# IRVLUTD/handnet-pipeline

Measured on AMD Instinct MI355X. Metric: end-to-end frames/sec (FCOS+A2J, 640x480), higher is better.
Workload: dtype f16x3 (fp32 values split into fp16 hi+lo, 3 MFMAs, fp32 accumulate; fp32 I/O); 1 GPU; Full HandNet pipeline (FCOS -> crop -> A2J), 640x480 RGB-D (BASELINE config 4); batch_per_gpu=32, global_batch=32, frame=640x480 RGB-D, parallelism=frames sharded over 1 GPU(s), one all-gather of per-frame records per step, rccl_ranks=1, ipc_mode=HSA_ENABLE_IPC_MODE_LEGACY=0, hipgraph=False

## Files before the change

### handnet-pipeline_amd/csrc/conv_igemm_f16x3.hip

```cpp
#define HN_IGEMM_MAIN_TU 1
#include "conv_igemm_f16x3_plan.h"

namespace {

constexpr const char* kCarryRefused =
    "the carried apply pass rides on the plain row-shared 128x128 grouped launch only (this shape takes another form): run the "
    "separate pass";

template <int BM, int BN, int WM, int WN, int NBUF, bool BUF, int TERMS = 3>
int launch16_impl(const ConvParams16& p0, hipStream_t st, const hn::CarryHook* carry = nullptr) {
  ConvParams16 p = p0;
  p.tiles_m = hn::cdiv(p.M, BM);
  p.tiles_n = hn::cdiv(p.Cout, BN);
  p.nblocks = p.tiles_m * p.tiles_n;
  plan_splits(p, BM, BN);
  int taken = 0;
  assign_tickets(p, BM, BN, WM * WN, p.split_ws, taken);
  int grid_x = p.nblocks;
  if (p.groups > 1) {
    grid_x = 0;
    for (int g = 0; g < p.groups; ++g) {
      p.gnblocks[g] = hn::cdiv(p.gM[g], BM) * p.tiles_n;
      grid_x = grid_x > p.gnblocks[g] ? grid_x : p.gnblocks[g];
    }
  }
  bool rs = false;
  constexpr int RS_LDS_BYTES = NBUF * (BM + WM * WN * 8 + BN) * ROWH * 2;
  if constexpr (BUF && NBUF == 2 && (WM * WN == 4 || WM * WN == 8) && RS_LDS_BYTES <= (WM * WN == 4 ? 80 : 160) * 1024 - 2048) {
    rs = rs_will_run(p, BM, BN, WM * WN, NBUF, BUF);
    if constexpr (BM == 128 && BN == 128 && WM == 2 && WN == 2 && TERMS == 3) {
      const int mask = rs ? mixed_small_mask(p, p.tiles_n) : 0;
      if (mask && carry) return hn::fail(HN_ERR_ARG, "%s", kCarryRefused);
      if (mask) {
        p.small_mask = mask;
        grid_x = 0;
        for (int g = 0; g < p.groups; ++g) {
          p.gnblocks[g] = hn::cdiv(p.gM[g], (mask >> g) & 1 ? 64 : 128) * p.tiles_n;
          grid_x = grid_x > p.gnblocks[g] ? grid_x : p.gnblocks[g];
        }
        constexpr int LDS_MIXED = RS_LDS_BYTES > 3 * (64 + 128) * ROWH * 2 ? RS_LDS_BYTES : 3 * (64 + 128) * ROWH * 2;
        static bool mixed_attr[64] = {};
        int dev = 0;
        HN_CHECK_HIP(hipGetDevice(&dev));
        if (dev < 0 || dev >= 64 || !mixed_attr[dev]) {
          HN_CHECK_HIP(hipFuncSetAttribute((const void*)conv_igemm_f16x3_mixed_kernel, hipFuncAttributeMaxDynamicSharedMemorySize,
                                           LDS_MIXED));
          if (dev >= 0 && dev < 64) mixed_attr[dev] = true;
        }
        hipLaunchKernelGGL(conv_igemm_f16x3_mixed_kernel, dim3(grid_x, 1, p.groups), dim3(256), LDS_MIXED, st, p);
        HN_CHECK_LAUNCH("conv_igemm_f16x3_mixed_kernel");
        return HN_OK;
      }
    }
    if (carry) {
      if constexpr (BM == 128 && BN == 128 && WM == 2 && WN == 2) {
        if (!rs || p.groups <= 1 || p.splits != 1) return hn::fail(HN_ERR_ARG, "%s", kCarryRefused);
        if (carry->dry) return HN_OK;
        return hn::launch_conv_carry(&p, sizeof(p), grid_x, p.groups, TERMS, RS_LDS_BYTES, carry->job, st);
      } else {
        return hn::fail(HN_ERR_ARG, "%s", kCarryRefused);
      }
    }
    if (rs) {
      constexpr int LDS_BYTES = RS_LDS_BYTES;
      static bool attr_set[64] = {};
      int dev = 0;
      HN_CHECK_HIP(hipGetDevice(&dev));
      if (dev < 0 || dev >= 64 || !attr_set[dev]) {
        HN_CHECK_HIP(hipFuncSetAttribute((const void*)conv_igemm_f16x3_kernel<BM, BN, WM, WN, NBUF, true, true, TERMS>,
                                         hipFuncAttributeMaxDynamicSharedMemorySize, LDS_BYTES));
        if (dev >= 0 && dev < 64) attr_set[dev] = true;
      }
      hipLaunchKernelGGL((conv_igemm_f16x3_kernel<BM, BN, WM, WN, NBUF, true, true, TERMS>),
                         dim3(grid_x, 1, p.groups > 1 ? p.groups : 1), dim3(WM * WN * 64), LDS_BYTES, st, p);
    }
  }
  if (carry) return hn::fail(HN_ERR_ARG, "%s", kCarryRefused);
  if (!rs)
    hipLaunchKernelGGL((conv_igemm_f16x3_kernel<BM, BN, WM, WN, NBUF, BUF, false, TERMS>),
                       dim3(grid_x, p.splits, p.groups > 1 ? p.groups : 1), dim3(WM * WN * 64), 0, st, p);
  HN_CHECK_LAUNCH("conv_igemm_f16x3_kernel");
  if (p.splits > 1 && p.ticket_base < 0) {
    const long total = (long)p.M * (p.Cout >> 3);
    const int grid = (int)((total + 255) / 256 < 4096 ? (total + 255) / 256 : 4096);
    hipLaunchKernelGGL(splitk_reduce_kernel, dim3(grid), dim3(256), 0, st, p);
    HN_CHECK_LAUNCH("splitk_reduce_kernel");
  }
  return HN_OK;
}

template <int BM, int BN, int WM, int WN, int NST, int KK>
int launch16_deepk(const ConvParams16& p0, hipStream_t st) {
  ConvParams16 p = p0;
  p.tiles_m = hn::cdiv(p.M, BM);
  p.tiles_n = hn::cdiv(p.Cout, BN);
  p.nblocks = p.tiles_m * p.tiles_n;
  plan_splits(p, BM, BN, KK);
  int taken = 0;
  assign_tickets(p, BM, BN, WM * WN, p.split_ws, taken);
  int grid_x = p.nblocks;
  if (p.groups > 1) {
    grid_x = 0;
    for (int g = 0; g < p.groups; ++g) {
      p.gnblocks[g] = hn::cdiv(p.gM[g], BM) * p.tiles_n;
      grid_x = grid_x > p.gnblocks[g] ? grid_x : p.gnblocks[g];
    }
  }
  constexpr int LDS_BYTES = NST * KK * (BM + BN) * ROWH * 2;
  static_assert(LDS_BYTES <= 160 * 1024, "deep-k ring exceeds the LDS");
  static bool attr_set[64] = {};
  int dev = 0;
  HN_CHECK_HIP(hipGetDevice(&dev));
  if (dev < 0 || dev >= 64 || !attr_set[dev]) {
    HN_CHECK_HIP(hipFuncSetAttribute((const void*)conv_igemm_f16x3_deepk_kernel<BM, BN, WM, WN, NST, KK>,
                                     hipFuncAttributeMaxDynamicSharedMemorySize, LDS_BYTES));
    if (dev >= 0 && dev < 64) attr_set[dev] = true;
  }
  hipLaunchKernelGGL((conv_igemm_f16x3_deepk_kernel<BM, BN, WM, WN, NST, KK>), dim3(grid_x, p.splits, p.groups > 1 ? p.groups : 1),
                     dim3(WM * WN * 64), LDS_BYTES, st, p);
  HN_CHECK_LAUNCH("conv_igemm_f16x3_deepk_kernel");
  if (p.splits > 1 && p.ticket_base < 0) {
    const long total = (long)p.M * (p.Cout >> 3);
    const int grid = (int)((total + 255) / 256 < 4096 ? (total + 255) / 256 : 4096);
    hipLaunchKernelGGL(splitk_reduce_kernel, dim3(grid), dim3(256), 0, st, p);
    HN_CHECK_LAUNCH("splitk_reduce_kernel");
  }
  return HN_OK;
}

template <int BM, int BN, int WM, int WN, int NBUF, bool ALLOW_F16X1 = true>
int launch16(const ConvParams16& p0, hipStream_t st, const hn::CarryHook* carry = nullptr) {
  ConvParams16 p = p0;
  const bool ok = finish_params16(p);
  if (p.terms == 1) {
    if constexpr (ALLOW_F16X1) {
      if (ok) return launch16_impl<BM, BN, WM, WN, NBUF, true, 1>(p, st, carry);
    }
    return hn::fail(HN_ERR_ARG, "the f16x1 mode exists for the descriptor-form kernels of the engine tiles only");
  }
  if (ok) return launch16_impl<BM, BN, WM, WN, NBUF, true>(p, st, carry);
  return launch16_impl<128, 128, 2, 2, 2, false>(p, st, carry);
}

}

static int deepk_of(const hn_conv_desc* d, int tile);
static int pick_tile_base(const hn_conv_desc* d);
extern "C" int hn_conv2d_f16x3_pick_tile(const hn_conv_desc* d) {
  if (!d) return HN_TILE_64x64;
  if (d->tile != HN_TILE_AUTO) return d->tile;
  return deepk_of(d, pick_tile_base(d));
}

static int pick_tile_base(const hn_conv_desc* d) {
  if (d->cout <= 32) return nblocks16(d, 128, 32) < 64 ? HN_TILE_32x64 : HN_TILE_128x32;
  const int64_t want = 256;
  if (d->cout > 64 && nblocks16(d, 128, 128) >= want) return HN_TILE_128x128;
  if (d->cout > 64 && d->r * d->s * d->cin / 32 >= 288 && nblocks16(d, 128, 128) >= 224) return HN_TILE_128x128;
  if (d->cout <= 64 && nblocks16(d, 256, 64) >= 2 * want) return HN_TILE_256x64;
  if (d->cout >= 128 && nblocks16(d, 64, 128) >= 192) return HN_TILE_64x128;
  if (nblocks16(d, 128, 64) >= want) return HN_TILE_128x64;
  if (nblocks16(d, 64, 64) < 128) return HN_TILE_32x64;
  return HN_TILE_64x64;
}

static int deepk_of(const hn_conv_desc* d, int tile) {
  if (hn::env_flags().no_deepk || d->terms == 1) return tile;
  const int ktiles = d->r * d->s * d->cin / 32;
  if (ktiles < 8) return tile;
  if (tile == HN_TILE_64x64 && nblocks16(d, 64, 64) <= 256) return HN_TILE_64x64_K2;
  return tile;
}

extern "C" int hn_conv2d_f16x3_uses_halo(const hn_conv_desc* d, int has_residual) {
  return d && hn::conv3x3_halo_applies(d, false, false, has_residual ? (const void*)d : nullptr) ? 1 : 0;
}

extern "C" int hn_conv2d_f16x3_uses_stream(const hn_conv_desc* d) {
  return d && hn::conv1x1_stream_applies(d, false, false) ? 1 : 0;
}

extern "C" int hn_conv2d_f16x3_uses_rs(const hn_conv_desc* d) {
  if (!d || d->w <= 0 || d->cin <= 0) return 0;
  if (hn::conv3x3_halo_applies(d, false, false, d->res_mode ? (const void*)d : nullptr)) return 0;
  const int tile = hn_conv2d_f16x3_pick_tile(d);
  ConvParams16 p;
  p.R = d->r; p.S = d->s; p.stride = d->stride; p.dil = d->dil; p.pad = d->pad;
  p.H = d->h; p.W = d->w; p.pitch = d->w;
  p.OH = (d->h + 2 * d->pad - d->dil * (d->r - 1) - 1) / d->stride + 1;
  p.OW = (d->w + 2 * d->pad - d->dil * (d->s - 1) - 1) / d->stride + 1;
  p.Cout = d->cout;
  p.M = d->n * d->oh * d->ow;
  p.ktiles = d->r * d->s * d->cin / BK;
  p.groups = 1;
  p.rs_ok = 1;
  p.gn_partial = nullptr;
  p.vec_epi = d->cout % 8 == 0;
  p.splitk_mode = d->splitk;
  p.split_ws = d->splitk >= 0 ? reinterpret_cast<float*>(16) : nullptr;
  p.split_ws_bytes = (int64_t)32 << 20;
  TileForm f = tile_form(tile, tile == HN_TILE_128x32 && rs32_preferred(d));
  if (f.bm == 0) return 0;
  p.nblocks = hn::cdiv(p.M, f.bm) * hn::cdiv(p.Cout, f.bn);
  plan_splits(p, f.bm, f.bn, f.kk);
  if (tile == HN_TILE_128x32 && f.nbuf == 2 && !rs_will_run(p, f.bm, f.bn, f.waves, 2, true)) return 0;
  return rs_will_run(p, f.bm, f.bn, f.waves, f.nbuf, true) ? 1 : 0;
}


extern "C" int hn_conv2d_nhwc_f16x3(const hn_conv_desc* d, const void* x16, const void* w16, const float* bias,
                                    const void* residual, void* y, void* stream) {
  return hn_igemm_conv16_run(d, x16, w16, bias, residual, y, nullptr, nullptr, 0, stream);
}

extern "C" int hn_conv2d_nhwc_f16x3_ws(const hn_conv_desc* d, const void* x16, const void* w16, const float* bias,
                                       const void* residual, void* y, void* workspace, int64_t workspace_bytes,
                                       void* stream) {
  HN_CHECK_ARG(workspace == nullptr || ((uintptr_t)workspace % 16 == 0 && workspace_bytes >= 0), "bad workspace");
  return hn_igemm_conv16_run(d, x16, w16, bias, residual, y, nullptr, workspace, workspace_bytes, stream);
}

extern "C" int hn_conv2d_nhwc_f16x3_gn(const hn_conv_desc* d, const void* x16, const void* w16, const float* bias,
                                       void* y, float* gn_partial, void* stream) {
  HN_CHECK_ARG(gn_partial, "hn_conv2d_nhwc_f16x3_gn: null gn_partial");
  HN_CHECK_ARG(d && d->cout % 8 == 0, "GroupNorm statistics need cout %% 8 == 0");
  return hn_igemm_conv16_run(d, x16, w16, bias, nullptr, y, gn_partial, nullptr, 0, stream);
}

extern "C" int hn_conv2d_nhwc_f16x3_grouped(const hn_conv_desc* d, const hn_conv_group* group, void* stream) {
  return hn::conv_grouped_run(d, group, stream, nullptr);
}

int hn::conv_grouped_run(const hn_conv_desc* d, const hn_conv_group* group, void* stream, const hn::CarryHook* carry) {
  HN_CHECK_ARG(d && group, "hn_conv2d_nhwc_f16x3_grouped: null pointer");
  HN_CHECK_ARG(group->count >= 1 && group->count <= HN_CONV_MAX_GROUP, "group count must be 1..%d", HN_CONV_MAX_GROUP);
  HN_CHECK_ARG(d->res_mode == 0, "grouped convolutions take no residual");
  bool any_gn = false, all_gn = true;
  for (int g = 0; g < group->count; ++g) {
    HN_CHECK_ARG(group->x16[g] && group->w16[g] && group->y[g], "group member %d has a null tensor", g);
    any_gn = any_gn || group->gn_partial[g];
    all_gn = all_gn && group->gn_partial[g];
  }
  HN_CHECK_ARG(any_gn == all_gn, "gn_partial must be given for every group member or for none");
  HN_CHECK_ARG(group->gn_units == 0 || group->gn_units >= d->cout / 8, "gn_units smaller than cout/8");
  return hn_igemm_conv16_run(d, group->x16[0], group->w16[0], group->bias[0], nullptr, group->y[0], nullptr, nullptr, 0, stream,
                    group, carry);
}

int hn_igemm_conv16_run(const hn_conv_desc* d, const void* x16, const void* w16, const float* bias, const void* residual, void* y,
                        float* gn_partial, void* workspace, int64_t workspace_bytes, void* stream, const hn_conv_group* group,
                        const hn::CarryHook* carry) {
  ConvParams16 p;
  HN_TRY16(fill_params16(d, x16, w16, bias, residual, y, gn_partial, workspace, workspace_bytes, p));
  if (d->terms != 1 && hn::conv3x3_halo_applies(d, gn_partial != nullptr, group != nullptr, residual) &&
      hn::conv3x3_halo_operands_ok(d, x16, w16, bias, residual, y))
    return hn::conv3x3_halo(d, x16, w16, bias, residual, y, (hipStream_t)stream);
  if (hn::conv1x1_stream_applies(d, gn_partial != nullptr, group != nullptr) &&
      hn::conv1x1_stream_operands_ok(d, x16, w16, bias, residual, y))
    return hn::conv1x1_stream(d, x16, w16, bias, residual, y, (hipStream_t)stream);

  hn_conv_desc tile_desc = *d;
  if (group) {
    p.groups = group->count;
    if (group->gn_units > 0) p.gn_units = group->gn_units;
    int64_t total_m = 0;
    for (int g = 0; g < group->count; ++g) {
      const int gh = group->h[g] > 0 ? group->h[g] : d->h, gw = group->w[g] > 0 ? group->w[g] : d->w;
      p.gH[g] = gh; p.gW[g] = gw;
      p.gOH[g] = (gh + 2 * d->pad - d->dil * (d->r - 1) - 1) / d->stride + 1;
      p.gOW[g] = (gw + 2 * d->pad - d->dil * (d->s - 1) - 1) / d->stride + 1;
      HN_CHECK_ARG(p.gOH[g] > 0 && p.gOW[g] > 0, "group member %d has an empty output", g);
      HN_CHECK_ARG((int64_t)d->n * p.gOH[g] * p.gOW[g] < (int64_t)1 << 31, "too many output pixels");
      p.gM[g] = d->n * p.gOH[g] * p.gOW[g];
      total_m += p.gM[g];
      if (gn_of_group_needs_32(group, g)) HN_CHECK_ARG(p.gOH[g] * p.gOW[g] >= 32, "GroupNorm statistics need OH*OW >= 32");
      p.gx[g] = (const _Float16*)group->x16[g]; p.gw[g] = (const _Float16*)group->w16[g];
      p.gbias[g] = group->bias[g]; p.gy[g] = group->y[g]; p.ggn[g] = group->gn_partial[g];
      p.vec_epi = p.vec_epi && ((uintptr_t)group->y[g] % 16 == 0) &&
                  (group->bias[g] == nullptr || (uintptr_t)group->bias[g] % 16 == 0);
    }
    p.gn_partial = group->gn_partial[0];
    p.split_ws = nullptr;
    if (group->gn_partial[0])
      HN_CHECK_ARG(p.vec_epi && !d->out_split && d->relu_cols == 0,
                   "GroupNorm statistics need the vector epilogue, fp32 output and no ReLU");
    tile_desc.n = 1;
    tile_desc.oh = (int)(total_m < ((int64_t)1 << 30) ? total_m : ((int64_t)1 << 30));
    tile_desc.ow = 1;
  }
  p.splits = 1;
  p.kt_per = p.ktiles;
  if (gn_partial) {
    HN_CHECK_ARG(p.vec_epi && !d->out_split && d->res_mode == 0 && d->relu_cols == 0,
                 "GroupNorm statistics need the vector epilogue, fp32 output, no residual and no ReLU");
    HN_CHECK_ARG(d->oh * d->ow >= 32, "GroupNorm statistics in the epilogue need OH*OW >= 32");
  }
  hipStream_t st = (hipStream_t)stream;
  int picked = hn_conv2d_f16x3_pick_tile(&tile_desc);
  if (carry && (picked != HN_TILE_128x128 || !group)) return hn::fail(HN_ERR_ARG, "%s", kCarryRefused);
  switch (picked) {
    case HN_TILE_128x128: return launch16<128, 128, 2, 2, 2>(p, st, carry);
    case HN_TILE_128x64: return launch16<128, 64, 2, 2, 2>(p, st);
    case HN_TILE_64x64: return launch16<64, 64, 2, 2, 3>(p, st);
    case HN_TILE_128x32: {
      bool rs2 = rs32_preferred(d);
      if (rs2) {
        ConvParams16 q = p;
        q.nblocks = hn::cdiv(q.M, 128) * hn::cdiv(q.Cout, 32);
        if (group) {
          q.nblocks = 0;
          for (int g = 0; g < q.groups; ++g) q.nblocks += hn::cdiv(q.gM[g], 128) * hn::cdiv(q.Cout, 32);
        }
        plan_splits(q, 128, 32);
        rs2 = rs_will_run(q, 128, 32, 4, 2, true);
      }
      if (rs2) return launch16<128, 32, 4, 1, 2>(p, st);
      return launch16<128, 32, 4, 1, 3>(p, st);
    }
    case HN_TILE_64x128: return launch16<64, 128, 2, 2, 3>(p, st);
    case HN_TILE_32x64: return launch16<32, 64, 1, 2, 4>(p, st);
    case HN_TILE_64x64_K2: {
      ConvParams16 q = p;
      if (p.terms == 3 && finish_params16(q)) return launch16_deepk<64, 64, 2, 2, 3, 2>(q, st);
      return launch16<64, 64, 2, 2, 3>(p, st);
    }
    case HN_TILE_256x64: return launch16<256, 64, 4, 1, 2>(p, st);
    default: return hn::fail(HN_ERR_ARG, "unknown or retired tile id %d", d->tile);
  }
}

static int stem16_run(const void* x16, int n, int ph, int pw, int pad, int r, int stride, int cout, const void* w16,
                      const float* bias, int relu, void* y, int out_split, bool pool, void* stream, int terms = 3) {
  HN_CHECK_ARG(x16 && w16 && y, "hn_conv_stem_f16x3: null pointer");
  HN_CHECK_ARG(n > 0 && ph > 0 && pw > 0 && cout > 0 && stride > 0, "bad dims");
  HN_CHECK_ARG(r >= 1 && r <= 8 && pad == r / 2, "stem filter must be R x R with R <= 8 and pad = R/2");
  HN_CHECK_ARG(!out_split || cout % 32 == 0, "S32 output needs cout %% 32 == 0 (got %d)", cout);
  const int hb = ph + 2 * pad, wb = pw + 2 * pad;
  const int oh = (hb - r) / stride + 1, ow = (wb - r) / stride + 1;
  HN_CHECK_ARG((ow - 1) * stride + 8 <= wb, "the 8-pixel k run of the last output column leaves the bordered row");
  HN_CHECK_ARG((int64_t)n * oh * ow < (int64_t)1 << 31, "too many output pixels");
  HN_CHECK_ARG((uintptr_t)x16 % 16 == 0 && (stride * 4 * 2) % 16 == 0 && (wb * 4 * 2) % 16 == 0,
               "LDS-DMA needs 16-byte aligned rows (stride and bordered width must be even)");
  ConvParams16 p;
  p.x = (const _Float16*)x16; p.w = (const _Float16*)w16; p.bias = bias; p.res = nullptr; p.y = y;
  p.N = n; p.H = hb; p.W = wb; p.Cin = 32; p.Cout = cout; p.R = r; p.S = 1;
  p.stride = stride; p.pad = 0; p.dil = 1; p.OH = oh; p.OW = ow;
  p.M = n * oh * ow;
  p.Ktot = r * 32;
  p.ktiles = r;
  p.relu_cols = relu ? cout : 0; p.res_mode = 0; p.res_h = p.res_w = 0;
  p.out_split = out_split; p.res_split = 0;
  p.xs = 4; p.pitch = wb; p.lo_off = (long)n * hb * wb * 4;
  p.gn_partial = nullptr;
  p.split_ws = nullptr; p.split_ws_bytes = 0; p.splits = 1; p.kt_per = p.ktiles; p.splitk_mode = -1; p.groups = 1; p.gn_units = cout >> 3;
  p.ys = (out_split ? 2 : 1) * cout;
  p.rs = 0;
  p.vec_epi = (cout % 8 == 0) && ((uintptr_t)y % 16 == 0) && (bias == nullptr || (uintptr_t)bias % 16 == 0);
  p.tiles_m = p.tiles_n = p.nblocks = 0;
  p.small_mask = 0;
  p.rs_ok = 0;
  p.terms = terms == 1 ? 1 : 3;
  p.range_flag = hn::range_flag_ptr();
  hipStream_t st = (hipStream_t)stream;
  if (pool) {
    HN_CHECK_ARG(cout == 64 && relu && out_split && bias, "the fused stem + max-pool kernel needs cout = 64, bias, ReLU and an S32 output");
    HN_CHECK_ARG((uintptr_t)y % 16 == 0 && (uintptr_t)bias % 16 == 0, "unaligned output / bias");
    HN_CHECK_ARG(r == 7 && stride == 2 && pad == 3 && (uintptr_t)w16 % 16 == 0,
                 "the fused stem + max-pool kernel is written for the 7x7 / stride-2 / pad-3 ResNet stem");
    return hn::stem_pool_direct(x16, n, ph, pw, w16, bias, y, terms == 1 ? 1 : 3, st);
  }
  if (cout <= 32) return launch16<128, 32, 4, 1, 3>(p, st);
  if (cout <= 64) return launch16<128, 64, 2, 2, 2>(p, st);
  return launch16<128, 128, 2, 2, 2>(p, st);
}

extern "C" int hn_conv_stem_f16x3(const void* x16, int n, int ph, int pw, int pad, int r, int stride, int cout,
                                  const void* w16, const float* bias, int relu, void* y, int out_split, void* stream) {
  return stem16_run(x16, n, ph, pw, pad, r, stride, cout, w16, bias, relu, y, out_split, false, stream);
}

extern "C" int hn_conv_stem_pool_f16x3(const void* x16, int n, int ph, int pw, int pad, int r, int stride, int cout,
                                       const void* w16, const float* bias, void* y, void* stream) {
  return stem16_run(x16, n, ph, pw, pad, r, stride, cout, w16, bias, 1, y, 1, true, stream);
}

extern "C" int hn_conv_stem_pool_f16x3_terms(const void* x16, int n, int ph, int pw, int pad, int r, int stride, int cout,
                                             const void* w16, const float* bias, void* y, int terms, void* stream) {
  HN_CHECK_ARG(terms == 0 || terms == 1 || terms == 3, "terms must be 0 / 3 or 1");
  return stem16_run(x16, n, ph, pw, pad, r, stride, cout, w16, bias, 1, y, 1, true, stream, terms);
}

int hn::tickets_nonzero_main(int64_t* count) { return tickets_nonzero_here(count); }
```

### handnet-pipeline_amd/csrc/conv_igemm_f16x3_kernel.h

```cpp
#pragma once
#include "hn_common.h"

#include <type_traits>

namespace {

typedef float f32x4 __attribute__((ext_vector_type(4)));
typedef _Float16 f16x8 __attribute__((ext_vector_type(8)));
typedef unsigned int u32x4 __attribute__((ext_vector_type(4)));
typedef __attribute__((address_space(3))) void lds_void;
typedef __attribute__((address_space(1))) const void gbl_void;

__device__ __attribute__((aligned(256))) _Float16 g_zero_page16[128];

constexpr int kTicketSlots = 128, kTicketsPerSlot = 4096;
constexpr bool fused_reduce_form(int bm, int bn) { return bm <= 64 && bn <= 128; }
__device__ int g_split_tickets[kTicketSlots * kTicketsPerSlot];

struct ConvParams16 {
  const _Float16* x;
  const _Float16* w;
  const float* bias;
  const void* res;
  void* y;
  int N, H, W, Cin, Cout, R, S, stride, pad, dil, OH, OW;
  int M, Ktot, ktiles;
  int relu_cols, res_mode, res_h, res_w;
  int xs;
  int pitch;
  long lo_off;
  int ys;
  int rs;
  int out_split, res_split;
  int vec_epi;
  float* gn_partial;
  int groups;
  const _Float16* gx[HN_CONV_MAX_GROUP];
  const _Float16* gw[HN_CONV_MAX_GROUP];
  const float* gbias[HN_CONV_MAX_GROUP];
  void* gy[HN_CONV_MAX_GROUP];
  float* ggn[HN_CONV_MAX_GROUP];
  int gH[HN_CONV_MAX_GROUP], gW[HN_CONV_MAX_GROUP], gOH[HN_CONV_MAX_GROUP], gOW[HN_CONV_MAX_GROUP];
  int gM[HN_CONV_MAX_GROUP], gnblocks[HN_CONV_MAX_GROUP];
  int gn_units;
  int splits, kt_per, splitk_mode;
  int ticket_base;
  float* split_ws;
  int64_t split_ws_bytes;
  int tiles_m, tiles_n, nblocks;
  int small_mask;
  int* range_flag;
  unsigned mg_ohow, sh_ohow, mg_ow, sh_ow;
  unsigned gmg_ohow[HN_CONV_MAX_GROUP], gsh_ohow[HN_CONV_MAX_GROUP], gmg_ow[HN_CONV_MAX_GROUP], gsh_ow[HN_CONV_MAX_GROUP];
  unsigned mg_w1, sh_w1, mg_h, sh_h;
  unsigned gmg_w1[HN_CONV_MAX_GROUP], gsh_w1[HN_CONV_MAX_GROUP], gmg_h[HN_CONV_MAX_GROUP], gsh_h[HN_CONV_MAX_GROUP];
  int terms;
  int rs_ok;
  unsigned a_records;
  unsigned b_records;
  unsigned ga_records[HN_CONV_MAX_GROUP];
};

#define HN_TRY16(expr)          \
  do {                          \
    const int st_ = (expr);     \
    if (st_ != HN_OK) return st_; \
  } while (0)

constexpr int BK = 32;
constexpr int ROWH = 64;

__device__ __forceinline__ int swz(int row) { return (row >> 1) & 7; }

__device__ __forceinline__ int fastdiv(int n, unsigned mg, unsigned sh) {
  return mg ? (int)(__umulhi((unsigned)n, mg) >> sh) : n;
}

__device__ __forceinline__ void mfma_pinned(f32x4& c, const f16x8& a, const f16x8& b) {
  asm volatile("v_mfma_f32_16x16x32_f16 %0, %2, %1, %0" : "+a"(c) : "v"(a), "v"(b) : "memory");
}

template <int OFF>
__device__ __forceinline__ void lds_read_pinned(f16x8& dst, unsigned addr) {
  static_assert(OFF >= 0 && OFF < 65536, "ds_read offset field is 16 bits");
  asm volatile("ds_read_b128 %0, %1 offset:%2" : "=v"(dst) : "v"(addr), "n"(OFF) : "memory");
}
template <int N>
__device__ __forceinline__ void lgkm_wait() {
  static_assert(N >= 0 && N <= 15, "lgkmcnt is a 4-bit counter");
  asm volatile("s_waitcnt lgkmcnt(%0)" ::"n"(N) : "memory");
}
__device__ __forceinline__ unsigned lds_addr(const _Float16* p) { return (unsigned)(size_t)(lds_void*)p; }

template <int B, int E, class F>
__device__ __forceinline__ void static_for(F&& f) {
  if constexpr (B < E) {
    f(std::integral_constant<int, B>{});
    static_for<B + 1, E>(f);
  }
}

__device__ __forceinline__ void epi_finish8(const ConvParams16& p, int m, int n, float (&v)[8], int ohow,
                                            const f16x8* pre_hi = nullptr, const f16x8* pre_lo = nullptr) {
  if (pre_hi) {
#pragma unroll
    for (int e = 0; e < 8; ++e) v[e] += (float)(*pre_hi)[e] + (float)(*pre_lo)[e];
  } else if (p.res_mode) {
    long rpix = m;
    if (p.res_mode == 2) {
      const int img = m / ohow;
      const int rem = m - img * ohow;
      const int oh = rem / p.OW, ow = rem - oh * p.OW;
      const int sh_ = (int)(((long)oh * p.res_h) / p.OH), sw_ = (int)(((long)ow * p.res_w) / p.OW);
      rpix = ((long)img * p.res_h + sh_) * p.res_w + sw_;
    }
    if (p.res_split) {
      const _Float16* q16 = reinterpret_cast<const _Float16*>(p.res) + rpix * p.rs + (n >> 5) * 64 + (n & 31);
      const f16x8 rh = *reinterpret_cast<const f16x8*>(q16), rl = *reinterpret_cast<const f16x8*>(q16 + 32);
#pragma unroll
      for (int e = 0; e < 8; ++e) v[e] += (float)rh[e] + (float)rl[e];
    } else {
      const float* q32 = reinterpret_cast<const float*>(p.res) + rpix * p.rs + n;
      const f32x4 r0 = *reinterpret_cast<const f32x4*>(q32), r1 = *reinterpret_cast<const f32x4*>(q32 + 4);
#pragma unroll
      for (int e = 0; e < 4; ++e) {
        v[e] += r0[e];
        v[4 + e] += r1[e];
      }
    }
  }
  if (p.relu_cols >= p.Cout) {
#pragma unroll
    for (int e = 0; e < 8; ++e) v[e] = hn::relu(v[e]);
  } else if (p.relu_cols > 0) {
#pragma unroll
    for (int e = 0; e < 8; ++e)
      if (n + e < p.relu_cols) v[e] = hn::relu(v[e]);
  }
  if (p.out_split) {
    if (p.range_flag) hn::range_note_n<8>(p.range_flag, v);
    f16x8 hi, lo;
#pragma unroll
    for (int e = 0; e < 8; ++e) {
      const _Float16 h = (_Float16)v[e];
      hi[e] = h;
      lo[e] = (_Float16)(v[e] - (float)h);
    }
    _Float16* q16 = reinterpret_cast<_Float16*>(p.y) + (long)m * p.ys + (n >> 5) * 64 + (n & 31);
    *reinterpret_cast<f16x8*>(q16) = hi;
    *reinterpret_cast<f16x8*>(q16 + 32) = lo;
  } else {
    float* q32 = reinterpret_cast<float*>(p.y) + (long)m * p.ys + n;
    f32x4 o0, o1;
#pragma unroll
    for (int e = 0; e < 4; ++e) {
      o0[e] = v[e];
      o1[e] = v[4 + e];
    }
    *reinterpret_cast<f32x4*>(q32) = o0;
    *reinterpret_cast<f32x4*>(q32 + 4) = o1;
  }
}

__device__ __forceinline__ void splitk_reduce_body(const ConvParams16& p) {
  const int units = p.Cout >> 3;
  const long total = (long)p.M * units;
  const int ohow = p.OH * p.OW;
  const long plane = (long)p.M * p.Cout;
  for (long i = (long)blockIdx.x * blockDim.x + threadIdx.x; i < total; i += (long)gridDim.x * blockDim.x) {
    const int m = (int)(i / units), n = (int)(i - (long)m * units) * 8;
    float v[8] = {0.f, 0.f, 0.f, 0.f, 0.f, 0.f, 0.f, 0.f};
    const float* src = p.split_ws + (long)m * p.Cout + n;
    for (int z = 0; z < p.splits; ++z) {
      const f32x4 a = *reinterpret_cast<const f32x4*>(src + z * plane), b = *reinterpret_cast<const f32x4*>(src + z * plane + 4);
#pragma unroll
      for (int e = 0; e < 4; ++e) {
        v[e] += a[e];
        v[4 + e] += b[e];
      }
    }
    if (p.bias) {
      const f32x4 b0 = *reinterpret_cast<const f32x4*>(p.bias + n), b1 = *reinterpret_cast<const f32x4*>(p.bias + n + 4);
#pragma unroll
      for (int e = 0; e < 4; ++e) {
        v[e] += b0[e];
        v[4 + e] += b1[e];
      }
    }
    epi_finish8(p, m, n, v, ohow);
  }
}

#ifdef HN_IGEMM_MAIN_TU
__global__ __launch_bounds__(256) void splitk_reduce_kernel(const ConvParams16 p) { splitk_reduce_body(p); }
#endif

template <int TM, int TH, int DPT, int TERMS = 3>
struct HalfSched {
  static constexpr int NM = 3 * TM * TH;
  static constexpr int NB = (TERMS == 3 ? 2 : 1) * TH;
  static constexpr int NAL = TERMS == 3 ? TM : 0;
  static constexpr int NMEM = DPT + NB + NAL + TM;
  static constexpr int earliest(int q) {
    return q < DPT + NB ? 0
           : q < DPT + NB + NAL ? (q - DPT - NB + 1) * TH
                                : 2 * TM * TH + (q - DPT - NB - NAL + 1) * TH;
  }
  static constexpr int slot(int q) {
    const int spread = (q * NM) / NMEM;
    return earliest(q) > spread ? earliest(q) : spread;
  }
};

template <int BM, int BN, int WM, int WN, int NBUF, bool BUF, bool RS = false, int TERMS = 3, bool DYN = false, int KK = 1>
__device__ __forceinline__ void conv_igemm_f16x3_body(const ConvParams16& p, const int blk_x, const int blk_y, const int blk_z,
                                                      const unsigned karg_off = 0 ) {
  static_assert(TERMS == 3 || TERMS == 1, "three terms (fp32-grade) or the hi*hi term alone");
  static_assert(NBUF >= 2 && NBUF <= 6, "2..6 LDS stages");
  static_assert(!RS || (BUF && NBUF == 2), "row-shared A needs the descriptor form and the 2-stage pipeline");
  static_assert(KK == 1 || (BUF && !RS && DYN && TERMS == 3), "the deep-k loop: descriptor form, per-tap, dynamic LDS, three terms");
  constexpr int NSLOT = NBUF * KK;
  struct {
    const _Float16 *x, *w;
    const float* bias;
    void* y;
    float* gn_partial;
    int H, W, pitch, OH, OW, M, nblocks;
    unsigned a_records, mg_ohow, sh_ohow, mg_ow, sh_ow, mg_w1, sh_w1, mg_h, sh_h;
  } o = {p.x, p.w, p.bias, p.y, p.gn_partial, p.H, p.W, p.pitch, p.OH, p.OW, p.M, p.nblocks, p.a_records,
         p.mg_ohow, p.sh_ohow, p.mg_ow, p.sh_ow, p.mg_w1, p.sh_w1, p.mg_h, p.sh_h};
  if (p.groups > 1) {
    typedef __attribute__((address_space(4))) const ConvParams16 KArgs;
    KArgs* kp = (KArgs*)__builtin_amdgcn_kernarg_segment_ptr();
    const int gz = blk_z;
    static_assert(HN_CONV_MAX_GROUP == 6, "member tables hold six entries");
    o.nblocks = kp->gnblocks[gz];
    if (blk_x >= o.nblocks) return;
    o.x = kp->gx[gz];
    o.w = kp->gw[gz];
    o.bias = kp->gbias[gz];
    o.y = kp->gy[gz];
    o.gn_partial = kp->ggn[gz];
    o.H = kp->gH[gz];
    o.W = kp->gW[gz];
    o.pitch = o.W;
    o.OH = kp->gOH[gz];
    o.OW = kp->gOW[gz];
    o.M = kp->gM[gz];
    o.a_records = kp->ga_records[gz];
    o.mg_ohow = kp->gmg_ohow[gz];
    o.sh_ohow = kp->gsh_ohow[gz];
    o.mg_ow = kp->gmg_ow[gz];
    o.sh_ow = kp->gsh_ow[gz];
    if constexpr (RS) {
      o.mg_w1 = kp->gmg_w1[gz];
      o.sh_w1 = kp->gsh_w1[gz];
      o.mg_h = kp->gmg_h[gz];
      o.sh_h = kp->gsh_h[gz];
    }
  }
  constexpr int NT = WM * WN * 64;
  constexpr int TM = BM / WM / 16, TN = BN / WN / 16;
  static_assert(TM >= 2 && TM % 2 == 0 && TN >= 2 && TN % 2 == 0, "wave tile must be a multiple of 32x32");
  constexpr int TH = TN / 2;
  constexpr int ROWS_PASS = NT / 8;
  static_assert(BM % ROWS_PASS == 0 && BN % ROWS_PASS == 0, "tile rows must be a multiple of NT/8");
  constexpr int A_ROWS = RS ? BM + ROWS_PASS : BM;
  constexpr int A_IT = A_ROWS / ROWS_PASS, B_IT = BN / ROWS_PASS;
  constexpr int A_BUF = A_ROWS * ROWH, B_BUF = BN * ROWH;
  extern __shared__ __attribute__((aligned(1024))) _Float16 smem_dyn[];
  __shared__ __attribute__((aligned(1024))) _Float16 smem_static[(RS || DYN) ? 8 : NSLOT * (A_BUF + B_BUF)];
  _Float16* smem = (RS || DYN) ? smem_dyn : smem_static;
  _Float16* As = smem;
  _Float16* Bs = smem + NSLOT * A_BUF;

  int lid;
  {
    const int bid = blk_x, nb = o.nblocks;
    const int q = nb >> 3, rr = nb & 7, xcd = bid & 7, loc = bid >> 3;
    lid = (xcd < rr ? xcd * (q + 1) : rr * (q + 1) + (xcd - rr) * q) + loc;
  }
  const int tile_m = lid / p.tiles_n, tile_n = lid - tile_m * p.tiles_n;
  const int m0 = tile_m * BM, n0 = tile_n * BN;
  const int tid = threadIdx.x, lane = tid & 63, wave = tid >> 6;
  const int wm = wave / WN, wn = wave - wm * WN;
  const int ohow = o.OH * o.OW;


  const int drow = tid >> 3, dpos = tid & 7;
  int a_ih0[A_IT], a_iw0[A_IT], a_cc[A_IT];
  const _Float16* a_row[A_IT];
  const _Float16* b_ptr[B_IT];
  unsigned a_off[A_IT], a_inv[A_IT], b_off[B_IT];
  int rs_u0 = 0;
  if constexpr (RS) {
    const int mw = fastdiv(m0, o.mg_ow, o.sh_ow);
    rs_u0 = mw * (o.W + 1) + (m0 - mw * o.W) - 1;
  }
#pragma unroll
  for (int it = 0; it < A_IT; ++it) {
    const int row = drow + it * ROWS_PASS;
    if constexpr (RS) {
      const int u = rs_u0 + row;
      const int uc = u < 0 ? 0 : u;
      const int rowi = fastdiv(uc, o.mg_w1, o.sh_w1);
      const int owp = uc - rowi * (o.W + 1);
      const int img = fastdiv(rowi, o.mg_h, o.sh_h);
      const int oh = rowi - img * o.H;
      const bool pix_ok = u >= 0 && owp < o.W && rowi < p.N * o.H;
      const int chunk = dpos ^ swz(row);
      a_off[it] = pix_ok ? (((unsigned)rowi * (unsigned)o.pitch + (unsigned)owp) * (unsigned)p.xs + (unsigned)((chunk & 3) * 8) +
                            (unsigned)(chunk >> 2) * (unsigned)p.lo_off) * 2u
                         : 0u;
      a_inv[it] = !pix_ok ? 7u : (oh == 0 ? 1u : 0u) | (oh == o.H - 1 ? 4u : 0u);
      continue;
    }
    int m = m0 + row;
    m = m < o.M ? m : o.M - 1;
    const int img = fastdiv(m, o.mg_ohow, o.sh_ohow);
    const int rem = m - img * ohow;
    const int oh = fastdiv(rem, o.mg_ow, o.sh_ow), ow = rem - oh * o.OW;
    const int ih0 = oh * p.stride - p.pad, iw0 = ow * p.stride - p.pad;
    const int chunk = dpos ^ swz(row);
    if constexpr (BUF) {
      a_off[it] = (((unsigned)(img * o.H + oh * p.stride) * (unsigned)o.pitch + (unsigned)(ow * p.stride)) * (unsigned)p.xs +
                   (unsigned)((chunk & 3) * 8) + (unsigned)(chunk >> 2) * (unsigned)p.lo_off) * 2u;
      unsigned inv = 0;
      if (p.pad > 0) {
        if (p.R == 3 && p.S == 3) {
          const unsigned uw = (unsigned)o.W, uh = (unsigned)o.H;
          const unsigned col_bits = ((unsigned)iw0 >= uw ? 1u : 0u) | ((unsigned)(iw0 + p.dil) >= uw ? 2u : 0u) |
                                    ((unsigned)(iw0 + 2 * p.dil) >= uw ? 4u : 0u);
          inv = ((unsigned)ih0 >= uh ? 7u : col_bits) | (((unsigned)(ih0 + p.dil) >= uh ? 7u : col_bits) << 3) |
                (((unsigned)(ih0 + 2 * p.dil) >= uh ? 7u : col_bits) << 6);
        } else {
          unsigned col_bits = 0;
          for (int sx = 0; sx < p.S; ++sx) col_bits |= ((unsigned)(iw0 + sx * p.dil) >= (unsigned)o.W ? 1u : 0u) << sx;
          const unsigned row_full = (1u << p.S) - 1u;
          for (int r = 0; r < p.R; ++r) {
            const unsigned bits = (unsigned)(ih0 + r * p.dil) >= (unsigned)o.H ? row_full : col_bits;
            inv |= bits << (r * p.S);
          }
        }
      }
      a_inv[it] = inv;
    } else {
      a_ih0[it] = ih0;
      a_iw0[it] = iw0;
      a_cc[it] = chunk * 8;
      a_row[it] = o.x + (((long)img * o.H + ih0) * o.pitch + iw0) * p.xs + (chunk & 3) * 8 + (chunk >> 2) * p.lo_off;
    }
  }
#pragma unroll
  for (int it = 0; it < B_IT; ++it) {
    const int row = drow + it * ROWS_PASS;
    int n = n0 + row;
    n = n < p.Cout ? n : p.Cout - 1;
    if constexpr (BUF)
      b_off[it] = ((unsigned)n * (unsigned)p.Ktot * 2u + (unsigned)((dpos ^ swz(row)) * 8)) * 2u;
    else
      b_ptr[it] = o.w + (long)n * p.Ktot * 2 + (dpos ^ swz(row)) * 8;
  }
  const long a_shift = RS ? (long)o.pitch * p.xs * 2 : BUF ? ((long)p.pad * o.pitch + p.pad) * p.xs * 2 : 0;
  const __amdgpu_buffer_rsrc_t rsrc_a = __builtin_amdgcn_make_buffer_rsrc(
      (void*)(reinterpret_cast<const char*>(o.x) - a_shift), 0, (int)o.a_records, 0x00020000);
  const __amdgpu_buffer_rsrc_t rsrc_b = __builtin_amdgcn_make_buffer_rsrc((void*)o.w, 0, (int)p.b_records, 0x00020000);
  const int grp_row = __builtin_amdgcn_readfirstlane(wave) * 8;
// ... 238 lines not shown
    if constexpr (PH == 2) rs_a_offsets(uoff_a, sh_a);
    _Float16* Ad = As + aq * A_BUF;
    _Float16* Bd = Bs + cs * B_BUF;
    const int an = PH == 2 ? aq ^ 1 : aq;
    unsigned anx[TM][2];
#pragma unroll
    for (int i = 0; i < TM; ++i)
#pragma unroll
      for (int pl = 0; pl < 2; ++pl) anx[i][pl] = rs_addr(i, NPH - 1, pl, an);
    const unsigned bnx_hi = b_rd_hi + ns * (B_BUF * 2), bnx_lo = b_rd_lo + ns * (B_BUF * 2);
    static_for<0, S3::NM + 1>([&](auto K) {
      constexpr int k = decltype(K)::value;
      static_for<0, S3::NMEM>([&](auto Q) {
        constexpr int q = decltype(Q)::value;
        if constexpr (S3::slot(q) == k) {
          if constexpr (q < B_IT) {
            dma_b_piece(q, Bd, boff);
          } else if constexpr (q < DPT_PH) {
            dma_a_piece(q - B_IT, Ad, 0, 0, uoff_a, sh_a);
          } else if constexpr (q < DPT_PH + S3::NB) {
            if constexpr (TERMS == 3) {
              constexpr int jj = (q - DPT_PH) >> 1;
              if constexpr ((q - DPT_PH) & 1)
                lds_read_pinned<jj * TILE_OFF>(b0.l[jj], bnx_lo);
              else
                lds_read_pinned<jj * TILE_OFF>(b0.h[jj], bnx_hi);
            } else {
              lds_read_pinned<(q - DPT_PH) * TILE_OFF>(b0.h[q - DPT_PH], bnx_hi);
            }
          } else if constexpr (q < DPT_PH + S3::NB + S3::NAL) {
            constexpr int i = q - DPT_PH - S3::NB;
            lds_read_pinned<0>(af.l[i], anx[i][1]);
          } else {
            constexpr int i = q - DPT_PH - S3::NB - S3::NAL;
            lds_read_pinned<0>(af.h[i], anx[i][0]);
          }
        }
      });
      if constexpr (k < S3::NM) {
        constexpr int term = k / (TM * TH), i = (k / TH) % TM, jj = k % TH;
        if constexpr (TERMS == 3 || term == 2) mfma_pinned(acc[i][TH + jj], term == 0 ? af.l[i] : af.h[i], term == 1 ? b1.l[jj] : b1.h[jj]);
      }
    });
    advance_tile();
    if constexpr (PH == 2) rs_a_advance();
  };
  if constexpr (RS) {
    rs_dma_a_tile(0);
    dma_tile(0);
    drain_and_barrier();
    dma_tile(1);
    rs_dma_a_tile(1);
    static_for<0, TH>([&](auto JJ) {
      constexpr int jj = decltype(JJ)::value;
      lds_read_pinned<jj * TILE_OFF>(b0.h[jj], b_rd_hi);
      if constexpr (TERMS == 3) lds_read_pinned<jj * TILE_OFF>(b0.l[jj], b_rd_lo);
    });
    if constexpr (TERMS == 3)
      static_for<0, TM>([&](auto I) { lds_read_pinned<0>(af.l[decltype(I)::value], rs_addr(decltype(I)::value, -1, 1, 0)); });
    static_for<0, TM>([&](auto I) { lds_read_pinned<0>(af.h[decltype(I)::value], rs_addr(decltype(I)::value, -1, 0, 0)); });
    __builtin_amdgcn_s_waitcnt(0xC07F);
    int aq = 0, cs = 0;
    for (int q3 = 0; q3 < a_qn; ++q3) {
      step_rs(std::integral_constant<int, 0>{}, cs, cs ^ 1, aq);
      step_rs(std::integral_constant<int, 1>{}, cs ^ 1, cs, aq);
      step_rs(std::integral_constant<int, 2>{}, cs, cs ^ 1, aq);
      cs ^= 1;
      aq ^= 1;
    }
  } else if constexpr (KK > 1) {
    static_assert((NBUF - 2) * KK * (A_IT + B_IT) <= 63, "vmcnt is a 6-bit counter");
    for (int s0 = 0; s0 < (NBUF - 1) * KK; ++s0) dma_tile(s0);
    const int nstages = (T + KK - 1) / KK;
    int grp = 0;
    static_assert(KK == 2, "the stage schedule below is written for two tiles per stage");
    auto read_frags = [&](int slot, f16x8 (&fah)[TM], f16x8 (&fal)[TM], f16x8 (&fbh)[TN], f16x8 (&fbl)[TN]) {
      const _Float16* Ab = As + slot * A_BUF;
      const _Float16* Bb = Bs + slot * B_BUF;
#pragma unroll
      for (int i = 0; i < TM; ++i) {
        fah[i] = *reinterpret_cast<const f16x8*>(Ab + a_rd[i][0]);
        fal[i] = *reinterpret_cast<const f16x8*>(Ab + a_rd[i][1]);
      }
#pragma unroll
      for (int j = 0; j < TN; ++j) {
        fbh[j] = *reinterpret_cast<const f16x8*>(Bb + b_rd[j][0]);
        fbl[j] = *reinterpret_cast<const f16x8*>(Bb + b_rd[j][1]);
      }
    };
    auto mfma_tile = [&](const f16x8 (&fah)[TM], const f16x8 (&fal)[TM], const f16x8 (&fbh)[TN], const f16x8 (&fbl)[TN]) {
#pragma unroll
      for (int i = 0; i < TM; ++i)
#pragma unroll
        for (int j = 0; j < TN; ++j) acc[i][j] = __builtin_amdgcn_mfma_f32_16x16x32_f16(fbh[j], fal[i], acc[i][j], 0, 0, 0);
#pragma unroll
      for (int i = 0; i < TM; ++i)
#pragma unroll
        for (int j = 0; j < TN; ++j) acc[i][j] = __builtin_amdgcn_mfma_f32_16x16x32_f16(fbl[j], fah[i], acc[i][j], 0, 0, 0);
#pragma unroll
      for (int i = 0; i < TM; ++i)
#pragma unroll
        for (int j = 0; j < TN; ++j) acc[i][j] = __builtin_amdgcn_mfma_f32_16x16x32_f16(fbh[j], fah[i], acc[i][j], 0, 0, 0);
    };
    (void)nstages;
    const int full = T / KK;
    for (int st = 0; st < full; ++st) {
      asm volatile("s_waitcnt vmcnt(%0) lgkmcnt(0)" ::"n"((NBUF - 2) * KK * DPT) : "memory");
      __builtin_amdgcn_s_barrier();
      asm volatile("" ::: "memory");
      f16x8 a0h[TM], a0l[TM], b0h[TN], b0l[TN], a1h[TM], a1l[TM], b1h[TN], b1l[TN];
      read_frags(grp * KK, a0h, a0l, b0h, b0l);
      const int refill = grp == 0 ? NBUF - 1 : grp - 1;
#pragma unroll
      for (int kk = 0; kk < KK; ++kk) dma_tile(refill * KK + kk);
      read_frags(grp * KK + 1, a1h, a1l, b1h, b1l);
      mfma_tile(a0h, a0l, b0h, b0l);
      mfma_tile(a1h, a1l, b1h, b1l);
      grp = grp + 1 == NBUF ? 0 : grp + 1;
    }
    if (T & 1) {
      asm volatile("s_waitcnt vmcnt(%0)" ::"n"((NBUF - 2) * KK * DPT) : "memory");
      __builtin_amdgcn_s_barrier();
      asm volatile("" ::: "memory");
      f16x8 a0h[TM], a0l[TM], b0h[TN], b0l[TN];
      read_frags(grp * KK, a0h, a0l, b0h, b0l);
      mfma_tile(a0h, a0l, b0h, b0l);
    }
  } else {
  dma_tile(0);
  drain_and_barrier();
  for (int i = 1; i < NBUF; ++i) dma_tile(i);
  static_for<0, TH>([&](auto JJ) {
    constexpr int jj = decltype(JJ)::value;
    lds_read_pinned<jj * TILE_OFF>(b0.h[jj], b_rd_hi);
    if constexpr (TERMS == 3) lds_read_pinned<jj * TILE_OFF>(b0.l[jj], b_rd_lo);
  });
  if constexpr (TERMS == 3)
    static_for<0, TM>([&](auto I) { lds_read_pinned<decltype(I)::value * TILE_OFF>(af.l[decltype(I)::value], a_rd_lo); });
  static_for<0, TM>([&](auto I) { lds_read_pinned<decltype(I)::value * TILE_OFF>(af.h[decltype(I)::value], a_rd_hi); });
  __builtin_amdgcn_s_waitcnt(0xC07F);
  int cs = 0, ns = 1;
  for (int t = 0; t < T; ++t) {
    step_main(cs, ns);
    cs = ns;
    ns = ns + 1 == NBUF ? 0 : ns + 1;
  }
  }
  asm volatile("s_waitcnt lgkmcnt(0)\n\ts_nop 15\n\ts_nop 15" ::: "memory");
  asm volatile("s_waitcnt vmcnt(0)" ::: "memory");

  ConvParams16 q = p;
  q.x = o.x; q.w = o.w; q.bias = o.bias; q.y = o.y; q.gn_partial = o.gn_partial;
  q.H = o.H; q.W = o.W; q.pitch = o.pitch; q.OH = o.OH; q.OW = o.OW; q.M = o.M;
  if (p.splits > 1) {
    q.y = p.split_ws + (long)blk_y * o.M * p.Cout;
    q.ys = p.Cout;
    q.bias = nullptr;
    q.res_mode = 0;
    q.relu_cols = 0;
    q.out_split = 0;
    q.gn_partial = nullptr;
  }
  const float* res32 = reinterpret_cast<const float*>(q.res);
  const _Float16* res16 = reinterpret_cast<const _Float16*>(q.res);
  float* y32 = reinterpret_cast<float*>(q.y);
  _Float16* y16 = reinterpret_cast<_Float16*>(q.y);
  const int px = lane & 15;
  const int nsub = (lg & 1) * 16 + (lg >> 1) * 8;
  const int n_wave = n0 + wn * (BN / WN);
  auto swap8 = [&](f32x4& x, f32x4& y) {
#pragma unroll
    for (int r = 0; r < 4; ++r) {
      const auto s = __builtin_amdgcn_permlane16_swap(__float_as_uint(x[r]), __float_as_uint(y[r]), false, false);
      x[r] = __uint_as_float(s[0]);
      y[r] = __uint_as_float(s[1]);
    }
  };
  constexpr bool FUSED_REDUCE = !RS && TERMS == 3 && fused_reduce_form(BM, BN);
  const bool tickets = FUSED_REDUCE && p.splits > 1 && p.ticket_base >= 0;
  __amdgpu_buffer_rsrc_t rsrc_ws = __builtin_amdgcn_make_buffer_rsrc((void*)p.split_ws, 0, 0, 0x00020000);
  int plane_off = 0;
  if constexpr (FUSED_REDUCE) {
    if (tickets) {
      const int plane_bytes = o.M * p.Cout * 4;
      rsrc_ws = __builtin_amdgcn_make_buffer_rsrc((void*)p.split_ws, 0, plane_bytes * p.splits, 0x00020000);
      plane_off = blk_y * plane_bytes;
    }
  }
  if (p.vec_epi) {
    constexpr int NP = TN / 2;
    f32x4 bias0[NP], bias1[NP];
#pragma unroll
    for (int jp = 0; jp < NP; ++jp) {
      const int n = n_wave + jp * 32 + nsub;
      bias0[jp] = f32x4{0.f, 0.f, 0.f, 0.f};
      bias1[jp] = bias0[jp];
      if (q.bias && n < p.Cout) {
        bias0[jp] = *reinterpret_cast<const f32x4*>(q.bias + n);
        bias1[jp] = *reinterpret_cast<const f32x4*>(q.bias + n + 4);
      }
    }
    constexpr bool PREF = TM * NP <= 8;
    f16x8 rpre_h[PREF ? TM * NP : 1], rpre_l[PREF ? TM * NP : 1];
    const bool use_pre = PREF && q.res_mode == 1 && q.res_split;
    if constexpr (PREF) {
      if (use_pre) {
#pragma unroll
        for (int i = 0; i < TM; ++i)
#pragma unroll
          for (int jp = 0; jp < NP; ++jp) {
            int m = m0 + wm * (BM / WM) + i * 16 + px;
            m = m < o.M ? m : o.M - 1;
            int n = n_wave + jp * 32 + nsub;
            n = n < p.Cout ? n : 0;
            const _Float16* q16 = res16 + (long)m * q.rs + (n >> 5) * 64 + (n & 31);
            rpre_h[i * NP + jp] = *reinterpret_cast<const f16x8*>(q16);
            rpre_l[i * NP + jp] = *reinterpret_cast<const f16x8*>(q16 + 32);
          }
      }
    }
    __builtin_amdgcn_s_waitcnt(0x0F70);
#pragma unroll
    for (int i = 0; i < TM; i += 2) {
      float gsum[NP][4];
#pragma unroll
      for (int jp = 0; jp < NP; ++jp)
#pragma unroll
        for (int e = 0; e < 4; ++e) gsum[jp][e] = 0.f;
      const int m_grp = m0 + wm * (BM / WM) + i * 16;
      const int m_split = (fastdiv(m_grp < o.M ? m_grp : o.M - 1, o.mg_ohow, o.sh_ohow) + 1) * ohow;
#pragma unroll
      for (int ii = 0; ii < 2; ++ii) {
        const int m = m_grp + ii * 16 + px;
#pragma unroll
        for (int jp = 0; jp < NP; ++jp) {
          f32x4 x = acc[i + ii][2 * jp], y = acc[i + ii][2 * jp + 1];
          swap8(x, y);
          const int n = n_wave + jp * 32 + nsub;
          if (m >= o.M || n >= p.Cout) continue;
          float v[8];
#pragma unroll
          for (int e = 0; e < 4; ++e) {
            v[e] = x[e] + bias0[jp][e];
            v[4 + e] = y[e] + bias1[jp][e];
          }
          if (q.gn_partial) {
            float s1 = 0.f, s2 = 0.f;
#pragma unroll
            for (int e = 0; e < 8; ++e) {
              s1 += v[e];
              s2 += v[e] * v[e];
            }
            const bool second = m >= m_split;
            gsum[jp][0] += second ? 0.f : s1;
            gsum[jp][1] += second ? 0.f : s2;
            gsum[jp][2] += second ? s1 : 0.f;
            gsum[jp][3] += second ? s2 : 0.f;
          }
          if constexpr (FUSED_REDUCE) {
            if (tickets) {
              const u32x4 d0 = {__float_as_uint(v[0]), __float_as_uint(v[1]), __float_as_uint(v[2]), __float_as_uint(v[3])};
              const u32x4 d1 = {__float_as_uint(v[4]), __float_as_uint(v[5]), __float_as_uint(v[6]), __float_as_uint(v[7])};
              const int voff = (m * p.Cout + n) * 4;
              __builtin_amdgcn_raw_buffer_store_b128(d0, rsrc_ws, voff, plane_off, 16 );
              __builtin_amdgcn_raw_buffer_store_b128(d1, rsrc_ws, voff + 16, plane_off, 16);
              continue;
            }
          }
          if constexpr (PREF) {
            if (use_pre) epi_finish8(q, m, n, v, ohow, &rpre_h[(i + ii) * NP + jp], &rpre_l[(i + ii) * NP + jp]);
            else epi_finish8(q, m, n, v, ohow);
          } else {
            epi_finish8(q, m, n, v, ohow);
          }
        }
      }
      if (q.gn_partial) {
#pragma unroll
        for (int jp = 0; jp < NP; ++jp) {
#pragma unroll
          for (int ofs = 1; ofs < 16; ofs <<= 1)
#pragma unroll
            for (int e = 0; e < 4; ++e) gsum[jp][e] += __shfl_xor(gsum[jp][e], ofs);
          const int n = n_wave + jp * 32 + nsub;
          if (px == 0 && n < p.Cout && m_grp < o.M) {
            f32x4 o4 = {gsum[jp][0], gsum[jp][1], gsum[jp][2], gsum[jp][3]};
            *reinterpret_cast<f32x4*>(q.gn_partial + ((long)(m_grp >> 5) * p.gn_units + (n >> 3)) * 4) = o4;
          }
        }
      }
    }
    if constexpr (FUSED_REDUCE) {
      if (tickets) {
        typedef __attribute__((address_space(4))) const unsigned KW;
        KW* kw = (KW*)((__attribute__((address_space(4))) const char*)__builtin_amdgcn_kernarg_segment_ptr() + karg_off);
        asm volatile("" : "+s"(kw));
        ConvParams16 f;
        {
          unsigned* dst = reinterpret_cast<unsigned*>(&f);
#pragma unroll
          for (int w = 0; w < (int)(sizeof(ConvParams16) / 4); ++w) dst[w] = kw[w];
        }
        int* ticket = g_split_tickets + p.ticket_base + lid * (WM * WN) + __builtin_amdgcn_readfirstlane(wave);
        __builtin_amdgcn_s_waitcnt(0x0F70);
        int drawn = 0;
        if (lane == 0) drawn = __hip_atomic_fetch_add(ticket, 1, __ATOMIC_RELAXED, __HIP_MEMORY_SCOPE_AGENT);
        drawn = __builtin_amdgcn_readfirstlane(drawn);
        if (drawn != f.splits - 1) return;
        if (lane == 0) __hip_atomic_store(ticket, 0, __ATOMIC_RELAXED, __HIP_MEMORY_SCOPE_AGENT);
        const int plane_bytes = f.M * f.Cout * 4;
        const int f_ohow = f.OH * f.OW;
        constexpr int NU = TM * NP, ZC = NU <= 2 ? 4 : 2;
        float v[NU][8];
        int voff[NU];
        bool live[NU];
#pragma unroll
        for (int u = 0; u < NU; ++u) {
          const int m = m0 + wm * (BM / WM) + (u / NP) * 16 + px, n = n_wave + (u % NP) * 32 + nsub;
          live[u] = m < f.M && n < f.Cout;
          voff[u] = live[u] ? (m * f.Cout + n) * 4 : 0;
#pragma unroll
          for (int e = 0; e < 8; ++e) v[u][e] = 0.f;
        }
        for (int z0 = 0; z0 < f.splits; z0 += ZC) {
          u32x4 ld[ZC][NU][2];
#pragma unroll
          for (int zz = 0; zz < ZC; ++zz) {
            const int z = z0 + zz < f.splits ? z0 + zz : f.splits - 1;
#pragma unroll
            for (int u = 0; u < NU; ++u) {
              ld[zz][u][0] = __builtin_amdgcn_raw_buffer_load_b128(rsrc_ws, voff[u], z * plane_bytes, 16 );
              ld[zz][u][1] = __builtin_amdgcn_raw_buffer_load_b128(rsrc_ws, voff[u] + 16, z * plane_bytes, 16);
            }
          }
#pragma unroll
          for (int zz = 0; zz < ZC; ++zz) {
            if (z0 + zz < f.splits) {
#pragma unroll
              for (int u = 0; u < NU; ++u)
#pragma unroll
                for (int e = 0; e < 4; ++e) {
                  v[u][e] += __uint_as_float(ld[zz][u][0][e]);
                  v[u][4 + e] += __uint_as_float(ld[zz][u][1][e]);
                }
            }
          }
        }
#pragma unroll
        for (int u = 0; u < NU; ++u) {
          if (!live[u]) continue;
          const int m = m0 + wm * (BM / WM) + (u / NP) * 16 + px, n = n_wave + (u % NP) * 32 + nsub;
          if (f.bias) {
            const f32x4 b0 = *reinterpret_cast<const f32x4*>(f.bias + n), b1 = *reinterpret_cast<const f32x4*>(f.bias + n + 4);
#pragma unroll
            for (int e = 0; e < 4; ++e) {
              v[u][e] += b0[e];
              v[u][4 + e] += b1[e];
            }
          }
          epi_finish8(f, m, n, v[u], f_ohow);
        }
      }
    }
    return;
  }
#pragma unroll
  for (int i = 0; i < TM; ++i) {
    const int m = m0 + wm * (BM / WM) + i * 16 + px;
    if (m >= o.M) continue;
    long rpix = 0;
    if (p.res_mode == 1) {
      rpix = (long)m;
    } else if (p.res_mode == 2) {
      const int img = m / ohow;
      const int rem = m - img * ohow;
      const int oh = rem / o.OW, ow = rem - oh * o.OW;
      const int sh_ = (int)(((long)oh * p.res_h) / o.OH), sw_ = (int)(((long)ow * p.res_w) / o.OW);
      rpix = ((long)img * p.res_h + sh_) * p.res_w + sw_;
    }
#pragma unroll
    for (int j = 0; j < TN; ++j) {
#pragma unroll
      for (int r = 0; r < 4; ++r) {
        const int n = n_wave + j * 16 + lg * 4 + r;
        if (n >= p.Cout) continue;
        float v = acc[i][j][r];
        if (q.bias) v += q.bias[n];
        if (p.res_mode) {
          if (p.res_split) {
            const _Float16* q = res16 + rpix * p.rs + (n >> 5) * 64 + (n & 31);
            v += (float)q[0] + (float)q[32];
          } else {
            v += res32[rpix * p.rs + n];
          }
        }
        if (n < p.relu_cols) v = hn::relu(v);
        if (p.out_split) {
          if (p.range_flag) hn::range_note(p.range_flag, v);
          _Float16* q = y16 + (long)m * p.ys + (n >> 5) * 64 + (n & 31);
          const _Float16 h = (_Float16)v;
          q[0] = h;
          q[32] = (_Float16)(v - (float)h);
        } else {
          y32[(long)m * p.ys + n] = v;
        }
      }
    }
  }
}

template <int BM, int BN, int WM, int WN, int NBUF, bool BUF, bool RS = false, int TERMS = 3>
__global__ __launch_bounds__(WM* WN * 64, (BM * BN / (WM * WN) > 64 * 64 ? 1 : 2))
void conv_igemm_f16x3_kernel(const ConvParams16 p) {
  conv_igemm_f16x3_body<BM, BN, WM, WN, NBUF, BUF, RS, TERMS>(p, (int)blockIdx.x, (int)blockIdx.y, (int)blockIdx.z);
}

template <int BM, int BN, int WM, int WN, int NST, int KK>
__global__ __launch_bounds__(WM* WN * 64, 2)
void conv_igemm_f16x3_deepk_kernel(const ConvParams16 p) {
  conv_igemm_f16x3_body<BM, BN, WM, WN, NST, true, false, 3, true, KK>(p, (int)blockIdx.x, (int)blockIdx.y, (int)blockIdx.z);
}

#ifdef HN_IGEMM_MAIN_TU
__global__ __launch_bounds__(256, 2) void conv_igemm_f16x3_mixed_kernel(const ConvParams16 p) {
  typedef __attribute__((address_space(4))) const ConvParams16 KArgs;
  KArgs* kp = (KArgs*)__builtin_amdgcn_kernarg_segment_ptr();
  if ((kp->small_mask >> blockIdx.z) & 1)
    conv_igemm_f16x3_body<64, 128, 2, 2, 3, true, false, 3, true>(p, (int)blockIdx.x, (int)blockIdx.y, (int)blockIdx.z);
  else
    conv_igemm_f16x3_body<128, 128, 2, 2, 2, true, true, 3>(p, (int)blockIdx.x, (int)blockIdx.y, (int)blockIdx.z);
}

#endif

constexpr int kMultiMax = HN_CONV_MULTI_MAX;
struct MultiParams16 {
  int count;
  int start[kMultiMax + 1];
  ConvParams16 m[kMultiMax];
};

__device__ __forceinline__ void load_member16(const MultiParams16& unused_by_value_copy, int g, ConvParams16& p) {
  (void)unused_by_value_copy;
  typedef __attribute__((address_space(4))) const unsigned KW;
  typedef __attribute__((address_space(4))) const char KB;
  KB* base = (KB*)__builtin_amdgcn_kernarg_segment_ptr();
  KW* src = (KW*)(base + offsetof(MultiParams16, m) + (size_t)g * sizeof(ConvParams16));
  unsigned* dst = reinterpret_cast<unsigned*>(&p);
  static_assert(sizeof(ConvParams16) % 4 == 0, "parameter block is copied word by word");
#pragma unroll
  for (int i = 0; i < (int)(sizeof(ConvParams16) / 4); ++i) dst[i] = src[i];
}

#ifdef HN_IGEMM_MULTI_TU
template <int BM, int BN, int WM, int WN, int NBUF, int KK = 1>
__global__ __launch_bounds__(WM* WN * 64, (BM * BN / (WM * WN) > 64 * 64 ? 1 : 2))
void conv_igemm_f16x3_multi_kernel(const MultiParams16 mp) {
  typedef __attribute__((address_space(4))) const MultiParams16 KM;
  KM* km = (KM*)__builtin_amdgcn_kernarg_segment_ptr();
  const int bid = (int)blockIdx.x;
  int g = 0;
#pragma unroll
  for (int i = 1; i < kMultiMax; ++i) g = (i < km->count && bid >= km->start[i]) ? i : g;
  int local = bid - km->start[g];
  ConvParams16 p;
  load_member16(mp, g, p);
  int by = 0;
  while (local >= p.nblocks) {
    local -= p.nblocks;
    ++by;
  }
  conv_igemm_f16x3_body<BM, BN, WM, WN, NBUF, true, false, 3, (KK > 1), KK>(
      p, local, by, 0, (unsigned)(offsetof(MultiParams16, m) + (size_t)g * sizeof(ConvParams16)));
}

__global__ __launch_bounds__(256) void splitk_reduce_multi_kernel(const MultiParams16 mp) {
  ConvParams16 p;
  load_member16(mp, (int)blockIdx.y, p);
  if (p.splits <= 1 || p.ticket_base >= 0) return;
  splitk_reduce_body(p);
}
#endif

}
```

### handnet-pipeline_amd/csrc/conv_igemm_f16x3_plan.h

```cpp
#pragma once
#include <mutex>
#include "conv_igemm_f16x3_kernel.h"

namespace {

struct SplitModel { int slots; double t_fix, t_k; };
static SplitModel split_model(int bm, int bn, int kk = 1) {
  const int cus = 256;
  if (kk > 1) return {1 * cus, 12.0, 0.10};
  if (bm == 32 && bn == 64) return {3 * cus, 3.0, 0.27};
  if (bm == 64 && bn == 64) return {3 * cus, 12.0, 0.12};
  if (bm == 64 && bn == 128) return {2 * cus, 16.0, 0.12};
  if (bm == 128 && bn == 64) return {2 * cus, 16.0, 0.20};
  if (bm == 128 && bn == 32) return {2 * cus, 12.0, 0.15};
  return {2 * cus, 20.0, 0.40};
}
static void plan_splits(ConvParams16& p, int bm, int bn, int kk = 1) {
  p.splits = 1;
  p.kt_per = p.ktiles;
  p.ticket_base = -1;
  if (p.groups > 1) return;
  if (!(p.split_ws && p.splitk_mode >= 0 && p.vec_epi && !p.gn_partial)) return;
  const int64_t plane_bytes = (int64_t)p.M * p.Cout * 4;
  int want = 1;
// ... 12 lines not shown
    SplitModel sm = split_model(bm, bn, kk);
    const hn::Tuning& tn = hn::tuning();
    sm.t_fix *= tn.splitk_fix;
    sm.t_k *= tn.splitk_tk;
    const double t_red0 = 4.5 * tn.splitk_red0, t_plane_min = 0.3 * tn.splitk_plane, bw = 3.0e6;
    double best = (double)hn::cdiv(p.nblocks, sm.slots) * (sm.t_fix + p.ktiles * sm.t_k);
    for (int s = 2; s <= 16 && p.ktiles / s >= min_per; ++s) {
      const int kt = hn::cdiv(p.ktiles, s), se = hn::cdiv(p.ktiles, kt);
      if (se != s) continue;
      const double per_plane = (double)plane_bytes / bw;
      const double t = (double)hn::cdiv((int64_t)p.nblocks * s, sm.slots) * (sm.t_fix + kt * sm.t_k) + t_red0 +
                       s * (per_plane > t_plane_min ? per_plane : t_plane_min);
      if (t < best) {
        best = t;
        want = s;
      }
    }
  }
  if ((int64_t)want * plane_bytes > p.split_ws_bytes) want = (int)(p.split_ws_bytes / plane_bytes);
  if (want > 1) {
    p.kt_per = hn::cdiv(p.ktiles, want);
    p.splits = hn::cdiv(p.ktiles, p.kt_per);
  }
}

static int split_ticket_slot(const void* workspace) {
  static std::mutex mu;
  static const void* keys[kTicketSlots];
  static int used = 0;
  std::lock_guard<std::mutex> lock(mu);
  for (int i = 0; i < used; ++i)
    if (keys[i] == workspace) return i;
  if (used == kTicketSlots) return -1;
  keys[used] = workspace;
  return used++;
}
static int tickets_nonzero_here(int64_t* count) {
  static int host[kTicketSlots * kTicketsPerSlot];
  HN_CHECK_HIP(hipDeviceSynchronize());
  HN_CHECK_HIP(hipMemcpyFromSymbol(host, HIP_SYMBOL(g_split_tickets), sizeof(host)));
  int64_t c = 0;
  for (int i = 0; i < kTicketSlots * kTicketsPerSlot; ++i) c += host[i] != 0;
  *count += c;
  return HN_OK;
}

static void assign_tickets(ConvParams16& p, int bm, int bn, int waves, const void* workspace, int& taken) {
  p.ticket_base = -1;
  if (p.splits <= 1 || !fused_reduce_form(bm, bn) || p.terms != 3 || !workspace || hn::env_flags().no_fused_reduce || taken + p.nblocks * waves > kTicketsPerSlot ||
      (int64_t)p.splits * p.M * p.Cout * 4 >= ((int64_t)1 << 31)) return;
  const int slot = split_ticket_slot(workspace);
  if (slot < 0) return;
  p.ticket_base = slot * kTicketsPerSlot + taken;
  taken += p.nblocks * waves;
}

static bool rs_tile_form(int bm, int bn, int waves, int nbuf, bool buf) {
  const int lds = nbuf * (bm + waves * 8 + bn) * ROWH * 2;
  return buf && nbuf == 2 && (waves == 4 || waves == 8) && lds <= (waves == 4 ? 80 : 160) * 1024 - 2048;
}
static bool rs_geometry(const ConvParams16& p) {
  return p.R == 3 && p.S == 3 && p.stride == 1 && p.dil == 1 && p.pad == 1 && p.pitch == p.W && p.OH == p.H && p.OW == p.W &&
         !hn::env_flags().no_rs;
}
static bool rs_will_run(const ConvParams16& p, int bm, int bn, int waves, int nbuf, bool buf) {
  if (!(p.rs_ok && rs_geometry(p) && rs_tile_form(bm, bn, waves, nbuf, buf)) || p.splits != 1) return false;
  const int spare = waves * 8 - 2;
  if ((bm + 1) / p.W + 1 > spare) return false;
  for (int g = 0; p.groups > 1 && g < p.groups; ++g)
    if ((bm + 1) / p.gW[g] + 1 > spare) return false;
  return true;
}

static int mixed_small_mask(const ConvParams16& p, int tiles_n) {
  if (p.groups <= 1 || p.terms != 3 || hn::env_flags().no_mixed) return 0;
  const int slots = 512;
  int64_t total = 0;
  int max_m = 0;
  for (int g = 0; g < p.groups; ++g) {
    total += (int64_t)hn::cdiv(p.gM[g], 128) * tiles_n;
    max_m = max_m > p.gM[g] ? max_m : p.gM[g];
  }
  const int64_t tail = total % slots;
  if (total <= slots || total > 3 * slots || tail == 0 || tail > slots / 4) return 0;
  int mask = 0;
  for (int g = 0; g < p.groups; ++g)
    if ((int64_t)p.gM[g] * 2 <= max_m) mask |= 1 << g;
  return mask;
}

static void magic_u31(unsigned d, unsigned& mg, unsigned& sh) {
  if (d <= 1) { mg = 0; sh = 0; return; }
  unsigned k = 0;
  while ((1ull << k) < d) ++k;
  const unsigned long long pw = 1ull << (31 + k);
  mg = (unsigned)((pw + d - 1) / d);
  sh = k - 1;
}

static bool finish_params16(ConvParams16& p) {
  magic_u31((unsigned)(p.OH * p.OW), p.mg_ohow, p.sh_ohow);
  magic_u31((unsigned)p.OW, p.mg_ow, p.sh_ow);
  magic_u31((unsigned)p.W + 1u, p.mg_w1, p.sh_w1);
  magic_u31((unsigned)p.H, p.mg_h, p.sh_h);
  for (int g = 0; g < HN_CONV_MAX_GROUP; ++g) {
    const bool on = p.groups > 1 && g < p.groups;
    magic_u31(on ? (unsigned)(p.gOH[g] * p.gOW[g]) : 1u, p.gmg_ohow[g], p.gsh_ohow[g]);
    magic_u31(on ? (unsigned)p.gOW[g] : 1u, p.gmg_ow[g], p.gsh_ow[g]);
    magic_u31(on ? (unsigned)p.gW[g] + 1u : 1u, p.gmg_w1[g], p.gsh_w1[g]);
    magic_u31(on ? (unsigned)p.gH[g] : 1u, p.gmg_h[g], p.gsh_h[g]);
  }
  p.rs_ok = p.rs_ok && rs_geometry(p);
  const int64_t lim = (int64_t)1 << 31;
  auto extent = [&](int h, int pitch) {
    return ((int64_t)p.N * h * pitch * p.xs + (p.lo_off > 32 ? p.lo_off : 0)) * 2 +
           ((int64_t)p.pad * pitch + p.pad) * p.xs * 2;
  };
  bool ok = p.R * p.S <= 32 && (int64_t)p.Cout * p.Ktot * 4 < lim;
  int64_t ea = extent(p.H, p.pitch);
  ok = ok && ea < lim;
  p.a_records = (unsigned)(ok ? ea : 0);
  p.b_records = (unsigned)(ok ? (int64_t)p.Cout * p.Ktot * 4 : 0);
  for (int g = 0; g < HN_CONV_MAX_GROUP; ++g) p.ga_records[g] = 0;
  if (p.groups > 1)
    for (int g = 0; g < p.groups; ++g) {
      ea = extent(p.gH[g], p.gW[g]);
      ok = ok && ea < lim;
      p.ga_records[g] = (unsigned)(ea < lim ? ea : 0);
    }
  return ok;
}

int64_t nblocks16(const hn_conv_desc* d, int bm, int bn) {
  const int64_t M = (int64_t)d->n * d->oh * d->ow;
  return (int64_t)hn::cdiv(M, bm) * hn::cdiv(d->cout, bn);
}

struct TileForm { int bm, bn, waves, nbuf, kk; };
static bool rs32_preferred(const hn_conv_desc* d) {
  return d->r == 3 && d->s == 3 && d->stride == 1 && d->dil == 1 && d->pad == 1 && !hn::env_flags().no_rs && !hn::env_flags().no_rs32;
}
static TileForm tile_form(int tile, bool rs32) {
  switch (tile) {
    case HN_TILE_128x128: return {128, 128, 4, 2, 1};
    case HN_TILE_128x64: return {128, 64, 4, 2, 1};
    case HN_TILE_64x64: return {64, 64, 4, 3, 1};
    case HN_TILE_128x32: return {128, 32, 4, rs32 ? 2 : 3, 1};
    case HN_TILE_64x128: return {64, 128, 4, 3, 1};
    case HN_TILE_32x64: return {32, 64, 2, 4, 1};
    case HN_TILE_256x64: return {256, 64, 4, 2, 1};
    case HN_TILE_64x64_K2: return {64, 64, 4, 3, 2};
    default: return {0, 0, 0, 0, 1};
  }
}

static inline bool gn_of_group_needs_32(const hn_conv_group* group, int g) { return group->gn_partial[g] != nullptr; }

static int fill_params16(const hn_conv_desc* d, const void* x16, const void* w16, const float* bias, const void* residual,
                         void* y, float* gn_partial, void* workspace, int64_t workspace_bytes, ConvParams16& p) {
  HN_CHECK_ARG(d && x16 && w16 && y, "hn_conv2d_nhwc_f16x3: null pointer");
  HN_CHECK_ARG(d->n > 0 && d->h > 0 && d->w > 0 && d->cin > 0 && d->cout > 0, "bad tensor dims");
  HN_CHECK_ARG(d->cin % 32 == 0, "f16x3 conv needs cin %% 32 == 0 (got %d); use hn_conv2d_nhwc_f32", d->cin);
  HN_CHECK_ARG(d->r > 0 && d->s > 0 && d->stride > 0 && d->dil > 0 && d->pad >= 0, "bad filter geometry");
  const int oh = (d->h + 2 * d->pad - d->dil * (d->r - 1) - 1) / d->stride + 1;
  const int ow = (d->w + 2 * d->pad - d->dil * (d->s - 1) - 1) / d->stride + 1;
  HN_CHECK_ARG(oh == d->oh && ow == d->ow, "output size mismatch: desc %dx%d, computed %dx%d", d->oh, d->ow, oh, ow);
  HN_CHECK_ARG(d->res_mode >= 0 && d->res_mode <= 2, "bad res_mode %d", d->res_mode);
  HN_CHECK_ARG(d->terms == 0 || d->terms == 1 || d->terms == 3, "terms must be 0 / 3 (f16x3) or 1 (f16x1), got %d", d->terms);
  HN_CHECK_ARG(d->res_mode == 0 || residual, "res_mode set but residual is null");
  HN_CHECK_ARG(d->res_mode != 2 || (d->res_h > 0 && d->res_w > 0), "res_mode 2 needs res_h/res_w");
  HN_CHECK_ARG(!d->in_affine, "f16x3 conv takes pre-split input; apply GroupNorm with hn_affine_split_f32 first");
  HN_CHECK_ARG(!d->out_split || d->cout % 32 == 0, "S32 output needs cout %% 32 == 0 (got %d)", d->cout);
  HN_CHECK_ARG(d->in_pix_stride == 0 || (d->in_pix_stride >= 2 * d->cin && d->in_pix_stride % 64 == 0), "bad in_pix_stride");
  HN_CHECK_ARG(d->out_pix_stride == 0 || d->out_pix_stride >= (d->out_split ? 2 : 1) * d->cout, "bad out_pix_stride");
  HN_CHECK_ARG((int64_t)d->n * d->oh * d->ow < (int64_t)1 << 31, "too many output pixels");
  p.x = (const _Float16*)x16; p.w = (const _Float16*)w16; p.bias = bias; p.res = residual; p.y = y;
  p.N = d->n; p.H = d->h; p.W = d->w; p.Cin = d->cin; p.Cout = d->cout; p.R = d->r; p.S = d->s;
  p.stride = d->stride; p.pad = d->pad; p.dil = d->dil; p.OH = d->oh; p.OW = d->ow;
  p.M = d->n * d->oh * d->ow;
  p.Ktot = d->r * d->s * d->cin;
  p.ktiles = p.Ktot / BK;
  p.relu_cols = d->relu_cols; p.res_mode = d->res_mode; p.res_h = d->res_h; p.res_w = d->res_w;
  p.out_split = d->out_split; p.res_split = d->res_split;
  p.xs = d->in_pix_stride ? d->in_pix_stride : 2 * d->cin;
  p.pitch = d->w;
  p.lo_off = 32;
  p.ys = d->out_pix_stride ? d->out_pix_stride : (d->out_split ? 2 : 1) * d->cout;
  p.rs = d->res_pix_stride ? d->res_pix_stride : (d->res_split ? 2 : 1) * d->cout;
  p.vec_epi = (d->cout % 8 == 0) && (p.out_split || p.ys % 4 == 0) &&
              (p.res_mode == 0 || p.res_split || p.rs % 4 == 0) &&
              ((uintptr_t)y % 16 == 0) && (bias == nullptr || (uintptr_t)bias % 16 == 0) &&
              (residual == nullptr || (uintptr_t)residual % 16 == 0);
  p.tiles_m = p.tiles_n = p.nblocks = 0;
  p.small_mask = 0;
  p.range_flag = hn::range_flag_ptr();
  p.gn_partial = gn_partial;
  p.split_ws = (float*)workspace;
  p.split_ws_bytes = workspace ? workspace_bytes : 0;
  p.splitk_mode = d->splitk;
  p.groups = 1;
  p.rs_ok = 1;
  p.terms = d->terms == 1 ? 1 : 3;
  p.gn_units = d->cout >> 3;
  return HN_OK;
}

}

int hn_igemm_conv16_run(const hn_conv_desc* d, const void* x16, const void* w16, const float* bias, const void* residual, void* y,
                        float* gn_partial, void* workspace, int64_t workspace_bytes, void* stream,
                        const hn_conv_group* group = nullptr, const hn::CarryHook* carry = nullptr);
```

### handnet-pipeline_amd/csrc/hn_common.h

```cpp
#pragma once
#include <hip/hip_runtime.h>
#include <stdarg.h>
#include <stdint.h>
#include <stdio.h>

#include "../../include/handnet_hip.h"

namespace hn {

char* err_buf();
int fail(int code, const char* fmt, ...);
int* range_flag_ptr();
struct EnvFlags {
  bool no_rs, no_rs32, split_generic, no_halo, no_thin, thin_tap, thin_flat, no_fuse_last_gn, pre_generic, no_multi,
      halo_stamps, splitk_fill512, no_stream, no_mixed, no_deepk, no_fused_reduce, thin_nogroup;
};
const EnvFlags& env_flags();
struct Tuning {
  double splitk_fix = 1.0, splitk_tk = 1.0, splitk_red0 = 1.0, splitk_plane = 1.0;
};
const Tuning& tuning();
bool conv3x3_halo_applies(const hn_conv_desc* d, bool has_gn, bool has_group, const void* residual);
bool conv3x3_halo_operands_ok(const hn_conv_desc* d, const void* x16, const void* w16, const float* bias, const void* residual,
                              const void* y);
int conv3x3_halo(const hn_conv_desc* d, const void* x16, const void* w16, const float* bias, const void* residual, void* y,
                 hipStream_t st);
int stem_pool_direct(const void* x16, int n, int ph, int pw, const void* w16, const float* bias, void* y, int terms, hipStream_t st);
bool conv1x1_stream_applies(const hn_conv_desc* d, bool has_gn, bool has_group);
bool conv1x1_stream_operands_ok(const hn_conv_desc* d, const void* x16, const void* w16, const float* bias, const void* residual,
                                const void* y);
int conv1x1_stream(const hn_conv_desc* d, const void* x16, const void* w16, const float* bias, const void* residual, void* y,
                   hipStream_t st);

struct CarryHook {
  const void* job;
  bool dry;
};
int launch_conv_carry(const void* conv_params, size_t conv_params_bytes, int grid_x, int groups, int terms, int lds_bytes,
                      const void* job, hipStream_t st);
int conv_grouped_run(const hn_conv_desc* d, const hn_conv_group* group, void* stream, const CarryHook* carry);

int tickets_nonzero_main(int64_t* count);
int tickets_nonzero_multi(int64_t* count);

#define HN_CHECK_ARG(cond, ...)                          \
  do {                                                   \
    if (!(cond)) return hn::fail(HN_ERR_ARG, __VA_ARGS__); \
  } while (0)

#define HN_CHECK_HIP(expr)                                                         \
  do {                                                                             \
    hipError_t e_ = (expr);                                                        \
    if (e_ != hipSuccess)                                                          \
      return hn::fail(HN_ERR_HIP, "%s failed: %s", #expr, hipGetErrorString(e_)); \
  } while (0)

#define HN_CHECK_LAUNCH(name)                                                          \
  do {                                                                                 \
    hipError_t e_ = hipGetLastError();                                                 \
    if (e_ != hipSuccess)                                                              \
      return hn::fail(HN_ERR_HIP, "launch of %s failed: %s", name, hipGetErrorString(e_)); \
  } while (0)

static inline int cdiv(int64_t a, int64_t b) { return (int)((a + b - 1) / b); }

__device__ __forceinline__ void range_note(int* flag, float v) {
  if (!(fabsf(v) <= 65504.f)) *flag = 1;
}
__device__ __forceinline__ float max_nan(float a, float b) { return __builtin_elementwise_maximum(a, b); }
__device__ __forceinline__ float relu(float v) { return max_nan(v, 0.f); }
__device__ __forceinline__ float range_mag(float a, float b) { return max_nan(fabsf(a), fabsf(b)); }
__device__ __forceinline__ bool range_bad(float v) { return !(fabsf(v) <= 65504.f); }
template <int N>
__device__ __forceinline__ void range_note_n(int* flag, const float (&v)[N]) {
  float m = fabsf(v[0]);
#pragma unroll
  for (int e = 1; e < N; ++e) m = max_nan(m, fabsf(v[e]));
  if (!(m <= 65504.f)) *flag = 1;
}
__device__ __forceinline__ void range_note_input(int* flag, float v) {
  if (!(fabsf(v) <= 65504.f)) flag[fabsf(v) <= 3.402823466e38f ? 1 : 2] = 1;
}

}
```

### handnet-pipeline_amd/csrc/hn_common.hip

```cpp
#include "hn_common.h"

#include <stdlib.h>

#include <string.h>

__device__ int g_range_flag[4];
static thread_local int g_range_check_on = 0;
static thread_local int* g_range_bound = nullptr;
struct RangeScope { int on; int* bound; };
static thread_local RangeScope g_range_stack[8];
static thread_local int g_range_depth = 0;

namespace hn {

int* range_flag_ptr() {
  if (!g_range_check_on) return nullptr;
  if (g_range_bound) return g_range_bound;
  static int* ptrs[64] = {nullptr};
  int dev = 0;
  if (hipGetDevice(&dev) != hipSuccess || dev < 0 || dev >= 64) return nullptr;
  if (!ptrs[dev]) {
    void* p = nullptr;
    if (hipGetSymbolAddress(&p, HIP_SYMBOL(g_range_flag)) != hipSuccess) return nullptr;
    ptrs[dev] = (int*)p;
  }
  return ptrs[dev];
}

char* err_buf() {
  static thread_local char buf[512] = {0};
  return buf;
}

int fail(int code, const char* fmt, ...) {
  va_list ap;
  va_start(ap, fmt);
  vsnprintf(err_buf(), 512, fmt, ap);
  va_end(ap);
  return code;
}

}

extern "C" int hn_abi_version(void) { return HN_ABI_VERSION; }

extern "C" int hn_debug_tickets_nonzero(int64_t* count) {
  HN_CHECK_ARG(count, "hn_debug_tickets_nonzero: null pointer");
  *count = 0;
  if (int rc = hn::tickets_nonzero_main(count)) return rc;
  return hn::tickets_nonzero_multi(count);
}

namespace hn {
static EnvFlags g_env = {};
const EnvFlags& env_flags() { return g_env; }
static Tuning g_tuning;
const Tuning& tuning() { return g_tuning; }
}

extern "C" int hn_set_tuning(const char* name, double value) {
  HN_CHECK_ARG(name && value > 0.0, "hn_set_tuning: null name or non-positive value");
  struct Entry { const char* name; double hn::Tuning::*field; };
  static const Entry table[] = {{"splitk_fix", &hn::Tuning::splitk_fix}, {"splitk_tk", &hn::Tuning::splitk_tk},
                                {"splitk_red0", &hn::Tuning::splitk_red0}, {"splitk_plane", &hn::Tuning::splitk_plane}};
  for (const Entry& e : table)
    if (strcmp(e.name, name) == 0) {
      hn::g_tuning.*(e.field) = value;
      return HN_OK;
    }
  return hn::fail(HN_ERR_ARG, "hn_set_tuning: unknown constant '%s'", name);
}

extern "C" int hn_set_form(const char* name, int value) {
  HN_CHECK_ARG(name, "hn_set_form: null name");
  struct Entry { const char* name; bool hn::EnvFlags::*field; };
  static const Entry table[] = {
      {"conv_no_rs", &hn::EnvFlags::no_rs},
      {"conv_no_rs32", &hn::EnvFlags::no_rs32},
      {"split_generic", &hn::EnvFlags::split_generic},
      {"conv_no_halo", &hn::EnvFlags::no_halo},
      {"preprocess_generic", &hn::EnvFlags::pre_generic},
      {"conv_no_multi", &hn::EnvFlags::no_multi},
      {"no_fuse_last_gn", &hn::EnvFlags::no_fuse_last_gn},
      {"no_thin_outputs", &hn::EnvFlags::no_thin},
      {"thin_form_tap", &hn::EnvFlags::thin_tap},
      {"thin_form_flat", &hn::EnvFlags::thin_flat},
      {"thin_no_group", &hn::EnvFlags::thin_nogroup},
      {"halo_stamps", &hn::EnvFlags::halo_stamps},
      {"splitk_fill512", &hn::EnvFlags::splitk_fill512},
      {"conv_no_stream", &hn::EnvFlags::no_stream},
      {"conv_no_mixed", &hn::EnvFlags::no_mixed},
      {"conv_no_deepk", &hn::EnvFlags::no_deepk},
      {"conv_no_fused_reduce", &hn::EnvFlags::no_fused_reduce},
  };
  for (const Entry& e : table)
    if (strcmp(e.name, name) == 0) {
      hn::g_env.*(e.field) = value != 0;
      return HN_OK;
    }
  return hn::fail(HN_ERR_ARG, "hn_set_form: unknown form '%s'", name);
}

extern "C" const char* hn_last_error(void) { return hn::err_buf(); }

extern "C" int hn_device_info(int* cu_count, int* clock_khz, char* arch_name, int arch_name_len) {
  int dev = 0;
  HN_CHECK_HIP(hipGetDevice(&dev));
  hipDeviceProp_t prop;
  HN_CHECK_HIP(hipGetDeviceProperties(&prop, dev));
  if (cu_count) *cu_count = prop.multiProcessorCount;
  if (clock_khz) *clock_khz = prop.clockRate;
  if (arch_name && arch_name_len > 0) {
    strncpy(arch_name, prop.gcnArchName, arch_name_len - 1);
    arch_name[arch_name_len - 1] = 0;
  }
  return HN_OK;
}

extern "C" int hn_device_pci_bus_id(char* out, int out_len) {
  HN_CHECK_ARG(out && out_len >= 16, "hn_device_pci_bus_id: buffer of at least 16 bytes");
  int dev = 0;
  HN_CHECK_HIP(hipGetDevice(&dev));
  HN_CHECK_HIP(hipDeviceGetPCIBusId(out, out_len, dev));
  return HN_OK;
}

extern "C" int hn_event_create(void** ev) {
  HN_CHECK_ARG(ev, "hn_event_create: null");
  hipEvent_t e;
  HN_CHECK_HIP(hipEventCreate(&e));
  *ev = (void*)e;
  return HN_OK;
}

extern "C" int hn_event_destroy(void* ev) {
  HN_CHECK_HIP(hipEventDestroy((hipEvent_t)ev));
  return HN_OK;
}

extern "C" int hn_event_record(void* ev, void* stream) {
  HN_CHECK_HIP(hipEventRecord((hipEvent_t)ev, (hipStream_t)stream));
  return HN_OK;
}

extern "C" int hn_event_elapsed_ms(void* start, void* stop, float* ms) {
  HN_CHECK_ARG(ms, "hn_event_elapsed_ms: null");
  HN_CHECK_HIP(hipEventSynchronize((hipEvent_t)stop));
  HN_CHECK_HIP(hipEventElapsedTime(ms, (hipEvent_t)start, (hipEvent_t)stop));
  return HN_OK;
}

extern "C" int hn_range_check_enable(int on) {
  g_range_check_on = on ? 1 : 0;
  return HN_OK;
}

extern "C" int hn_range_check_enabled(void) { return g_range_check_on; }

extern "C" int hn_range_check_bind(int32_t* block) {
  g_range_bound = block;
  return HN_OK;
}

extern "C" int hn_range_scope_begin(int32_t* block, int on) {
  HN_CHECK_ARG(g_range_depth < 8, "hn_range_scope_begin: more than 8 nested scopes on this thread");
  g_range_stack[g_range_depth++] = RangeScope{g_range_check_on, g_range_bound};
  g_range_check_on = on ? 1 : 0;
  g_range_bound = on ? block : nullptr;
  return HN_OK;
}

extern "C" int hn_range_scope_end(void) {
  HN_CHECK_ARG(g_range_depth > 0, "hn_range_scope_end: no open scope on this thread");
  const RangeScope s = g_range_stack[--g_range_depth];
  g_range_check_on = s.on;
  g_range_bound = s.bound;
  return HN_OK;
}

extern "C" int hn_range_check_fetch(int* flag, int reset, void* stream) {
  HN_CHECK_ARG(flag, "hn_range_check_fetch: null");
  void* p = nullptr;
  int words[4] = {0, 0, 0, 0};
  HN_CHECK_HIP(hipGetSymbolAddress(&p, HIP_SYMBOL(g_range_flag)));
  HN_CHECK_HIP(hipMemcpyAsync(words, p, sizeof(words), hipMemcpyDeviceToHost, (hipStream_t)stream));
  HN_CHECK_HIP(hipStreamSynchronize((hipStream_t)stream));
  *flag = (words[0] ? HN_RANGE_ACTIVATION : 0) | (words[1] ? HN_RANGE_INPUT : 0) | (words[2] ? HN_RANGE_INPUT_NONFINITE : 0);
  if (reset) {
    HN_CHECK_HIP(hipMemsetAsync(p, 0, sizeof(words), (hipStream_t)stream));
    HN_CHECK_HIP(hipStreamSynchronize((hipStream_t)stream));
  }
  return HN_OK;
}

namespace {
__global__ void range_collect_kernel(int* __restrict__ flags, int* __restrict__ dst) {
  const int t = threadIdx.x;
  if (t < 4) {
    dst[t] = flags[t];
    flags[t] = 0;
  }
}
}

extern "C" int hn_range_check_collect(int32_t* block, int32_t* dst, void* stream) {
  HN_CHECK_ARG(dst, "hn_range_check_collect: null");
  void* p = block;
  if (!p) HN_CHECK_HIP(hipGetSymbolAddress(&p, HIP_SYMBOL(g_range_flag)));
  hipLaunchKernelGGL(range_collect_kernel, dim3(1), dim3(64), 0, (hipStream_t)stream, (int*)p, dst);
  HN_CHECK_LAUNCH("range_collect_kernel");
  return HN_OK;
}

namespace {
__global__ __launch_bounds__(64) void clock_sample_kernel(unsigned long long ticks, float* mhz) {
  const unsigned long long r0 = __builtin_amdgcn_s_memrealtime();
  const unsigned long long c0 = __builtin_amdgcn_s_memtime();
  unsigned long long r1 = r0;
  for (long guard = 0; guard < (1L << 26) && r1 - r0 < ticks; ++guard) {
    __builtin_amdgcn_s_sleep(64);
    r1 = __builtin_amdgcn_s_memrealtime();
  }
  const unsigned long long c1 = __builtin_amdgcn_s_memtime();
  if (threadIdx.x == 0) mhz[0] = (float)((double)(c1 - c0) / ((double)(r1 - r0) * 0.01));
}
}

extern "C" int hn_clock_sample(int micros, float* mhz, void* stream) {
  HN_CHECK_ARG(mhz, "hn_clock_sample: null");
  HN_CHECK_ARG(micros > 0 && micros <= 2000000, "hn_clock_sample: micros must be in 1..2e6");
  hipLaunchKernelGGL(clock_sample_kernel, dim3(1), dim3(64), 0, (hipStream_t)stream, (unsigned long long)micros * 100ull, mhz);
  HN_CHECK_LAUNCH("clock_sample_kernel");
  return HN_OK;
}
```

### handnet-pipeline_amd/hn_amd/_lib.py

```python
from __future__ import annotations

import ctypes as C
import os
import threading
from pathlib import Path

from . import build as _build

ABI_VERSION = 36

TILE_AUTO, TILE_128x128, TILE_128x64, TILE_64x64, TILE_128x32, _TILE_RETIRED_5, TILE_64x128 = range(7)
HN_FCOS_MAX_LEVELS = 5

c_f32p = C.POINTER(C.c_float)
c_i32p = C.POINTER(C.c_int32)
c_i64p = C.POINTER(C.c_int64)


class ConvDesc(C.Structure):
    _fields_ = [(k, C.c_int32) for k in (
        "n", "h", "w", "cin", "cout", "r", "s", "stride", "pad", "dil", "oh", "ow",
        "relu_cols", "res_mode", "res_h", "res_w", "in_affine", "tile", "out_split", "res_split",
        "res_pix_stride", "in_pix_stride", "out_pix_stride", "in_affine_stride", "splitk", "terms")]


CONV_MAX_GROUP = 6


class ConvGroup(C.Structure):
    _fields_ = [("count", C.c_int32), ("x16", C.c_void_p * CONV_MAX_GROUP), ("w16", C.c_void_p * CONV_MAX_GROUP),
                ("bias", C.c_void_p * CONV_MAX_GROUP), ("y", C.c_void_p * CONV_MAX_GROUP),
                ("gn_partial", C.c_void_p * CONV_MAX_GROUP), ("h", C.c_int32 * CONV_MAX_GROUP),
                ("w", C.c_int32 * CONV_MAX_GROUP), ("gn_units", C.c_int32)]


CONV_MULTI_MAX = 4


class ConvMulti(C.Structure):
    _fields_ = [("count", C.c_int32), ("desc", ConvDesc * CONV_MULTI_MAX), ("x16", C.c_void_p * CONV_MULTI_MAX),
                ("w16", C.c_void_p * CONV_MULTI_MAX), ("bias", C.c_void_p * CONV_MULTI_MAX),
                ("residual", C.c_void_p * CONV_MULTI_MAX), ("y", C.c_void_p * CONV_MULTI_MAX)]


class GraphCsr(C.Structure):
    _fields_ = [("indptr", C.c_void_p), ("indices", C.c_void_p), ("values", C.c_void_p), ("v", C.c_int32)]


class ConvertOpts(C.Structure):
    _fields_ = [("clamp_keypoints", C.c_int32), ("clamp_box_h", C.c_int32), ("clamp_box_w", C.c_int32), ("reserved", C.c_int32),
                ("sample_box", C.c_void_p), ("sample_paras", C.c_void_p)]


class ModelConfig(C.Structure):
    _fields_ = [(k, C.c_int32) for k in ("parts", "num_classes", "num_joints", "rgbd", "min_size", "max_size", "ext", "f16_terms",
                                          "precision")] + [("image_mean", C.c_float * 3), ("image_std", C.c_float * 3)]


MODEL_FCOS, MODEL_A2J = 1, 2
PRECISION_SPLIT, PRECISION_F32 = 0, 1
RANGE_ACTIVATION, RANGE_INPUT, RANGE_INPUT_NONFINITE = 1, 2, 4
FRAME_F32_CHW, FRAME_U8_BGR_HWC = 0, 1


class FcosLevels(C.Structure):
    _fields_ = [("num_levels", C.c_int32),
                ("h", C.c_int32 * HN_FCOS_MAX_LEVELS),
                ("w", C.c_int32 * HN_FCOS_MAX_LEVELS),
                ("stride", C.c_int32 * HN_FCOS_MAX_LEVELS),
                ("cls_lr", C.c_void_p * HN_FCOS_MAX_LEVELS),
                ("reg_ctr", C.c_void_p * HN_FCOS_MAX_LEVELS)]


class GnLevels(C.Structure):
    _fields_ = [("count", C.c_int32), ("hw", C.c_int32 * HN_FCOS_MAX_LEVELS),
                ("partial", C.c_void_p * HN_FCOS_MAX_LEVELS), ("scale", C.c_void_p * HN_FCOS_MAX_LEVELS),
                ("shift", C.c_void_p * HN_FCOS_MAX_LEVELS)]


class SplitLevels(C.Structure):
    _fields_ = [("count", C.c_int32), ("hw", C.c_int32 * HN_FCOS_MAX_LEVELS),
                ("x", C.c_void_p * HN_FCOS_MAX_LEVELS), ("scale", C.c_void_p * HN_FCOS_MAX_LEVELS),
                ("shift", C.c_void_p * HN_FCOS_MAX_LEVELS), ("y16", C.c_void_p * HN_FCOS_MAX_LEVELS)]


class ThinLevels(C.Structure):
    _fields_ = [("count", C.c_int32), ("x16", C.c_void_p * HN_FCOS_MAX_LEVELS), ("y", C.c_void_p * HN_FCOS_MAX_LEVELS),
                ("h", C.c_int32 * HN_FCOS_MAX_LEVELS), ("w", C.c_int32 * HN_FCOS_MAX_LEVELS)]


class ThinMember(C.Structure):
    _fields_ = [("lv", ThinLevels), ("cout", C.c_int32), ("relu_cols", C.c_int32), ("w16", C.c_void_p), ("bias", C.c_void_p)]


class ThinAffine(C.Structure):
    _fields_ = [("x", C.c_void_p * HN_FCOS_MAX_LEVELS), ("scale", C.c_void_p * HN_FCOS_MAX_LEVELS),
                ("shift", C.c_void_p * HN_FCOS_MAX_LEVELS), ("in_pix_stride", C.c_int32), ("affine_stride", C.c_int32)]


VP = C.c_void_p
SIGNATURES = {
    "hn_abi_version": (C.c_int, []),
    "hn_last_error": (C.c_char_p, []),
    "hn_device_info": (C.c_int, [c_i32p, c_i32p, C.c_char_p, C.c_int]),
    "hn_event_create": (C.c_int, [C.POINTER(VP)]),
    "hn_event_destroy": (C.c_int, [VP]),
    "hn_event_record": (C.c_int, [VP, VP]),
    "hn_event_elapsed_ms": (C.c_int, [VP, VP, c_f32p]),
    "hn_clock_sample": (C.c_int, [C.c_int, VP, VP]),
    "hn_conv2d_nhwc_f16x3_multi": (C.c_int, [C.POINTER(ConvMulti), VP, C.c_int64, VP]),
    "hn_conv2d_f16x3_multi_fuses": (C.c_int, [C.POINTER(ConvMulti), C.c_int64]),
    "hn_device_pci_bus_id": (C.c_int, [C.c_char_p, C.c_int]),
    "hn_ingest_u8bgr_u16mm": (C.c_int, [VP, VP, C.c_int, VP, VP, VP, C.c_int, C.c_int, C.c_int, VP]),
    "hn_range_check_enable": (C.c_int, [C.c_int]),
    "hn_range_check_fetch": (C.c_int, [c_i32p, C.c_int, VP]),
    "hn_range_check_enabled": (C.c_int, []),
    "hn_range_check_bind": (C.c_int, [VP]),
    "hn_range_scope_begin": (C.c_int, [VP, C.c_int]),
    "hn_range_scope_end": (C.c_int, []),
    "hn_range_check_collect": (C.c_int, [VP, VP, VP]),
    "hn_set_form": (C.c_int, [C.c_char_p, C.c_int]),
    "hn_set_tuning": (C.c_int, [C.c_char_p, C.c_double]),
    "hn_conv2d_nhwc_f32": (C.c_int, [C.POINTER(ConvDesc), VP, VP, VP, VP, VP, VP, VP, VP]),
    "hn_conv2d_pick_tile": (C.c_int, [C.POINTER(ConvDesc)]),
    "hn_conv2d_nhwc_f16x3": (C.c_int, [C.POINTER(ConvDesc), VP, VP, VP, VP, VP, VP]),
    "hn_affine_split_f32": (C.c_int, [VP, VP, VP] + [C.c_int] * 6 + [VP, C.c_int, VP]),
    "hn_unsplit_f32": (C.c_int, [VP] + [C.c_int] * 4 + [VP, C.c_int, VP]),
    "hn_maxpool3x3s2_s32": (C.c_int, [VP, VP] + [C.c_int] * 6 + [VP]),
    "hn_conv2d_f16x3_pick_tile": (C.c_int, [C.POINTER(ConvDesc)]),
    "hn_conv2d_f16x3_uses_stream": (C.c_int, [C.POINTER(ConvDesc)]),
    "hn_conv2d_f16x3_uses_rs": (C.c_int, [C.POINTER(ConvDesc)]),
    "hn_conv2d_f16x3_uses_halo": (C.c_int, [C.POINTER(ConvDesc), C.c_int]),
    "hn_maxpool3x3s2_nhwc_f32": (C.c_int, [VP, VP] + [C.c_int] * 6 + [VP]),
    "hn_groupnorm_scratch_floats": (C.c_int64, [C.c_int] * 4),
    "hn_groupnorm_affine_f32": (C.c_int, [VP, VP, VP] + [C.c_int] * 4 + [C.c_float, VP, VP, VP, VP]),
    "hn_fcos_preprocess_f32": (C.c_int, [VP, VP] + [C.c_int] * 7 + [c_f32p, c_f32p, VP]),
    "hn_conv2d_nhwc_f16x3_ws": (C.c_int, [C.POINTER(ConvDesc)] + [VP] * 6 + [C.c_int64, VP]),
    "hn_conv2d_nhwc_f16x3_grouped": (C.c_int, [C.POINTER(ConvDesc), C.POINTER(ConvGroup), VP]),
    "hn_conv2d_nhwc_f16x3_gn": (C.c_int, [C.POINTER(ConvDesc)] + [VP] * 6),
    "hn_groupnorm_rows32_scratch_floats": (C.c_int64, [C.c_int64, C.c_int]),
    "hn_groupnorm_finalize_rows32": (C.c_int, [VP, VP, VP] + [C.c_int] * 4 + [C.c_float, VP, VP, VP]),
    "hn_spmm_csr_f32": (C.c_int, [VP, VP, VP, C.c_int, VP, VP, C.c_int, C.c_int, VP]),
    "hn_graph_conv_cheby3_f16x3": (C.c_int, [C.POINTER(GraphCsr), C.POINTER(GraphCsr), VP, C.c_int, C.c_int, VP, C.c_int, VP,
                                             C.c_int, C.c_int, VP, C.c_int, C.c_int, VP, C.c_int, VP]),
    "hn_linear_rows_f16x3": (C.c_int, [VP, C.c_int, C.c_int, C.c_int, VP, VP, VP, C.c_int, C.c_int, VP, VP, C.c_int, C.c_int, VP,
                                       C.c_int, VP]),
    "hn_mesh_finish_f32": (C.c_int, [VP, VP, VP, VP, C.c_int, C.c_int, C.c_int, C.c_int, VP, VP]),
    "hn_mesh_render_scratch_bytes": (C.c_int64, [C.c_int, C.c_int]),
    "hn_draw_labels_u8": (C.c_int, [VP, VP, VP, C.c_int, C.c_int, VP] + [C.c_int] * 4 + [VP, VP, VP]),
    "hn_mesh_render_u8": (C.c_int, [VP, VP, VP, VP] + [C.c_int] * 4 + [c_f32p, VP, C.c_int, C.c_int, C.c_int, VP, C.c_int64, VP, VP,
                                    VP]),
    "hn_pad_split_rows_f32": (C.c_int, [VP, C.c_int64, C.c_int, C.c_int, VP, VP]),
    "hn_lifter_combine_f32": (C.c_int, [VP, VP, C.c_int, C.c_int, C.c_int, C.c_int, VP, VP]),
    "hn_cheby3_basis_split": (C.c_int, [VP, VP, VP, C.c_int, VP, VP, VP, C.c_int, C.c_int, C.c_int, VP]),
    "hn_feat_interp_add_f32": (C.c_int, [VP, VP, VP, C.c_int64, C.c_int, C.c_int, C.c_int, VP]),
    "hn_fcos_preprocess_split": (C.c_int, [VP, VP] + [C.c_int] * 8 + [c_f32p, c_f32p, VP]),
    "hn_fcos_preprocess_list": (C.c_int, [VP, VP, VP] + [C.c_int] * 5 + [c_f32p, c_f32p, VP]),
    "hn_conv_stem_f16x3": (C.c_int, [VP] + [C.c_int] * 7 + [VP, VP, C.c_int, VP, C.c_int, VP]),
    "hn_conv_stem_pool_f16x3": (C.c_int, [VP] + [C.c_int] * 7 + [VP, VP, VP, VP]),
    "hn_conv_stem_pool_f16x3_terms": (C.c_int, [VP] + [C.c_int] * 7 + [VP, VP, VP, C.c_int, VP]),
    "hn_fcos_candidates": (C.c_int, [C.POINTER(FcosLevels), C.c_int, C.c_int, C.c_float,
                                     VP, VP, VP, VP, VP, VP, VP, C.c_int, VP]),
    "hn_fcos_candidates_ws_bytes": (C.c_int64, [C.c_int, C.c_int]),
    "hn_fcos_candidates_ws": (C.c_int, [C.POINTER(FcosLevels), C.c_int, C.c_int, C.c_float,
                                     VP, VP, VP, VP, VP, VP, VP, C.c_int, VP, C.c_int64, VP]),
    "hn_fcos_ext_gather": (C.c_int, [C.POINTER(FcosLevels), C.POINTER(VP), VP, VP, VP, C.c_int, C.c_int, VP, VP, VP]),
    "hn_fcos_nms_scratch_bytes": (C.c_int64, [C.c_int, C.c_int]),
    "hn_fcos_nms": (C.c_int, [VP] * 6 + [C.c_int, C.c_int, C.c_double, C.c_float, C.c_float] + [VP] * 9),
    "hn_fcos_nms_ratios": (C.c_int, [VP] * 6 + [C.c_int, C.c_int, C.c_double, VP] + [VP] * 9),
    "hn_nms": (C.c_int, [VP, VP, C.c_int, C.c_double, VP, VP, VP, VP]),
    "hn_crop_resize": (C.c_int, [VP, VP, VP, C.c_int, C.c_int, VP] + [C.c_int] * 7 + [VP, VP, VP, VP]),
    "hn_crop_resize_hands": (C.c_int, [VP, VP, VP, VP] + [C.c_int] * 3 + [VP] + [C.c_int] * 7 + [VP] * 6),
    "hn_stem_image_nhwc4": (C.c_int, [VP, C.c_int, C.c_int, C.c_int, C.c_int, VP, VP]),
    "hn_stem_image_nhwc4_valid": (C.c_int, [VP, C.c_int, C.c_int, C.c_int, C.c_int, VP, VP, VP]),
    "hn_pack_depth_nhwc": (C.c_int, [VP, VP, C.c_int, C.c_int, C.c_int, VP]),
    "hn_a2j_aggregate_f32": (C.c_int, [VP, VP, VP, VP] + [C.c_int] * 5 + [VP, VP]),
    "hn_create": (C.c_int, [C.POINTER(ModelConfig), C.POINTER(VP)]),
    "hn_load_weight": (C.c_int, [VP, C.c_char_p, VP, c_i64p, C.c_int]),
    "hn_finalize": (C.c_int, [VP]),
    "hn_fcos_capacity": (C.c_int64, [VP, C.c_int, C.c_int]),
    "hn_fcos_forward": (C.c_int, [VP, VP, C.c_int, C.c_int, C.c_int] + [VP] * 6 + [C.c_int, VP]),
    "hn_fcos_forward_ext": (C.c_int, [VP, VP, C.c_int, C.c_int, C.c_int] + [VP] * 8 + [C.c_int, VP]),
    "hn_fcos_capacity_list": (C.c_int64, [VP, C.POINTER(C.c_int32), C.POINTER(C.c_int32), C.c_int]),
    "hn_fcos_forward_list": (C.c_int, [VP, C.POINTER(C.c_void_p), C.POINTER(C.c_int32), C.POINTER(C.c_int32), C.c_int,
                                       VP, VP, VP, VP, VP, VP, C.c_int, VP]),
    "hn_a2j_forward": (C.c_int, [VP, VP, C.c_int, C.c_int, C.c_int, VP, VP, VP]),
    "hn_handnet_forward": (C.c_int, [VP, VP, VP, C.c_int, C.c_int, C.c_int, VP, VP, VP, VP]),
    "hn_handnet_forward_hands": (C.c_int, [VP, VP, VP] + [C.c_int] * 4 + [VP] * 5),
    "hn_destroy": (C.c_int, [VP]),
    "hn_groupnorm_finalize_rows32_levels": (C.c_int, [C.POINTER(GnLevels), VP, VP, C.c_int, C.c_int, C.c_int, C.c_float, VP]),
    "hn_affine_split_f32_levels": (C.c_int, [C.POINTER(SplitLevels)] + [C.c_int] * 6 + [VP]),
    "hn_affine_split_f32_levels_streams": (C.c_int, [C.POINTER(C.c_int32), C.c_int, C.c_int, C.c_int]),
    "hn_conv2d_nhwc_f16x3_grouped_carry": (C.c_int, [C.POINTER(ConvDesc), C.POINTER(ConvGroup), C.POINTER(SplitLevels)]
                                           + [C.c_int] * 6 + [VP]),
    "hn_conv2d_f16x3_grouped_carry_applies": (C.c_int, [C.POINTER(ConvDesc), C.POINTER(ConvGroup)]),
    "hn_pack_records": (C.c_int, [VP, VP, VP, C.c_int, C.c_int, C.c_int, C.c_int, VP, VP]),
    "hn_debug_tickets_nonzero": (C.c_int, [c_i64p]),
    "hn_pack_records_ex": (C.c_int, [VP, VP, VP, C.c_int, C.c_int, C.c_int, C.c_int, VP, VP, VP, VP]),
    "hn_unpack_records": (C.c_int, [VP, C.c_int, C.c_int, C.c_int, VP, VP, VP, VP, VP]),
    "hn_nonfinite_count_f32": (C.c_int, [VP, C.c_int64, VP, VP]),
    "hn_conv3x3_thin_f16x3_levels": (C.c_int, [C.POINTER(ThinLevels), C.c_int, C.c_int, C.c_int, VP, VP, C.c_int, C.c_int, VP]),
    "hn_conv3x3_thin_f16x3_levels_group": (C.c_int, [C.POINTER(ThinMember), C.c_int, C.c_int, C.c_int, C.c_int, VP]),
    "hn_conv3x3_thin_affine_applies": (C.c_int, [C.POINTER(ThinLevels), C.c_int, C.c_int, C.c_int]),
    "hn_conv3x3_thin_affine_f16x3_levels": (C.c_int, [C.POINTER(ThinLevels), C.POINTER(ThinAffine), C.c_int, C.c_int, C.c_int,
                                                      VP, VP, C.c_int, VP]),
    "hn_conv3x3_thin_uses_flat": (C.c_int, [C.POINTER(ThinLevels), C.c_int, C.c_int, C.c_int]),
    "hn_convert_joints_f32": (C.c_int, [VP, VP, VP, C.c_int, C.c_int, C.c_float, C.c_float, c_f32p, VP, VP]),
    "hn_convert_joints_samples_f32": (C.c_int, [VP, VP, VP, VP, C.c_int, C.c_int, C.c_float, C.c_float, VP, VP, VP]),
    "hn_a2j_aggregate_convert_f32": (C.c_int, [VP, VP, VP, VP] + [C.c_int] * 5 + [VP, C.c_float, C.c_float, c_f32p,
                                               C.POINTER(ConvertOpts), VP, VP, VP, VP]),
    "hn_a2j_aggregate_loss_f32": (C.c_int, [VP] * 5 + [C.c_int] * 5 + [C.c_float, C.c_float, VP, C.c_float, C.c_float, c_f32p,
                                            C.POINTER(ConvertOpts)] + [VP] * 7),
    "hn_joints2d_standardize_f32": (C.c_int, [VP, VP, C.c_int, C.c_int, VP, VP]),
    "hn_lifter_input_gated_f32": (C.c_int, [VP, VP, C.c_int, C.c_int, VP, VP, VP]),
    "hn_handnet_forward_xyz": (C.c_int, [VP, VP, VP, C.c_int, C.c_int, C.c_int, c_f32p, C.POINTER(ConvertOpts),
                                         VP, VP, VP, VP, VP, VP]),
    "hn_ingest_u8bgr_u16mm_flip": (C.c_int, [VP, VP, C.c_int, VP, VP, VP, C.c_int, C.c_int, C.c_int, C.c_int, VP]),
    "hn_flip_w_f32": (C.c_int, [VP, VP, C.c_int64, VP, VP, C.c_int64, C.c_int, VP]),
    "hn_crop_resize_hands_sided": (C.c_int, [VP] * 5 + [C.c_int] * 4 + [VP] + [C.c_int] * 7 + [VP] * 8),
    "hn_a2j_aggregate_convert_mirror_f32": (C.c_int, [VP] * 5 + [C.c_int] * 5 + [VP, C.c_float, C.c_float, c_f32p,
                                                      C.POINTER(ConvertOpts), VP, VP, VP, VP]),
    "hn_lifter_input_gated_mirror_f32": (C.c_int, [VP, VP, VP, C.c_int, C.c_int, VP, VP, VP]),
    "hn_mesh_finish_mirror_f32": (C.c_int, [VP] * 5 + [C.c_int] * 4 + [VP, VP]),
    "hn_crop_resize_hands_tracked": (C.c_int, [VP] * 5 + [C.c_int] * 4 + [VP] + [C.c_int] * 7 + [VP] * 8
                                     + [C.c_int, C.c_int, VP, VP, VP]),
    "hn_track_state_bytes": (C.c_int64, [C.c_int, C.c_int]),
    "hn_mesh_finish_smooth_f32": (C.c_int, [VP] * 9 + [C.c_int] * 4 + [C.c_float] * 4 + [VP] * 4),
    "hn_smooth_state_bytes": (C.c_int64, [C.c_int, C.c_int, C.c_int]),
    "hn_mesh_render_occluded_u8": (C.c_int, [VP, VP, VP, VP] + [C.c_int] * 4 + [c_f32p, VP, C.c_int, C.c_int, C.c_int, VP, C.c_int64,
                                             C.c_float, VP, C.c_int64, VP, VP, VP, VP, VP]),
    "hn_mesh_render_cams_u8": (C.c_int, [VP, VP, VP, VP] + [C.c_int] * 4 + [VP, VP, C.c_int, C.c_int, C.c_int, VP, C.c_int64, VP,
                                         VP, VP]),
    "hn_mesh_render_cams_occluded_u8": (C.c_int, [VP, VP, VP, VP] + [C.c_int] * 4 + [VP, VP, C.c_int, C.c_int, C.c_int, VP,
                                                  C.c_int64, C.c_float, VP, C.c_int64, VP, VP, VP, VP, VP]),
    "hn_rig_fuse_f32": (C.c_int, [VP] * 7 + [C.c_int] * 4 + [C.c_float] + [VP] * 9),
    "hn_hand_cloud_scratch_bytes": (C.c_int64, [C.c_int] * 3),
    "hn_hand_cloud_f32": (C.c_int, [VP] * 3 + [C.c_int64] + [VP] * 3 + [C.c_int] * 6 + [C.c_float, VP, C.c_int64] + [VP] * 4),
    "hn_mesh_fit_scratch_bytes": (C.c_int64, [C.c_int] * 3),
    "hn_mesh_fit_f32": (C.c_int, [VP] * 3 + [C.c_int64] + [VP] * 4 + [C.c_int] * 7 + [C.c_float, C.c_int] + [C.c_double] * 3
                        + [VP, C.c_int64] + [VP] * 6),
    "hn_mesh_geometry_f32": (C.c_int, [VP] * 4 + [C.c_int] * 4 + [c_f32p, VP, C.c_int, C.c_int, VP, C.c_int64, VP, VP, VP]),
    "hn_mesh_fit_iters_scratch_bytes": (C.c_int64, [C.c_int] * 8),
    "hn_mesh_fit_iters_f32": (C.c_int, [VP] * 3 + [C.c_int64] + [VP] * 7 + [C.c_int] * 9 + [C.c_float, C.c_int] + [C.c_double] * 3
                              + [VP, C.c_int64, VP, C.c_int64] + [VP] * 7),
    "hn_hpe_accumulate_f32": (C.c_int, [VP] * 3 + [C.c_int, C.c_int, VP, C.c_int] + [VP] * 6),
    "hn_det_ap_accumulate_f32": (C.c_int, [VP] * 8 + [C.c_int, C.c_int] + [VP] * 4 + [C.c_int] + [VP] * 3 + [C.c_int] * 4
                                 + [C.c_float, C.c_double] + [VP] * 4 + [C.c_int, VP]),
}

_lock = threading.Lock()
_lib = None


def lib_path() -> Path:
    override = os.environ.get("HN_LIB_PATH")
    return Path(override) if override else _build.LIB_PATH


def load(build_if_missing: bool = True) -> C.CDLL:
    global _lib
    with _lock:
        if _lib is not None:
            return _lib
        path = lib_path()
        if not path.exists():
            if not build_if_missing or path != _build.LIB_PATH:
                raise RuntimeError(f"{path} is missing; run `python __graft_entry__.py build`")
            _build.build_library()
        lib = C.CDLL(str(path))
        for name, (res, args) in SIGNATURES.items():
            try:
                fn = getattr(lib, name)
            except AttributeError as e:
                raise RuntimeError(f"{path} does not export {name}; rebuild it") from e
            fn.restype, fn.argtypes = res, args
        if lib.hn_abi_version() != ABI_VERSION:
            raise RuntimeError(f"{path}: ABI {lib.hn_abi_version()} != expected {ABI_VERSION}; rebuild it")
        _lib = lib
        return lib


def check(status: int, what: str) -> None:
    if status != 0:
        msg = load().hn_last_error()
        raise RuntimeError(f"{what} failed (status {status}): {msg.decode() if msg else '?'}")


def ptr(t) -> int | None:
    return None if t is None else t.data_ptr()
```

### handnet-pipeline_amd/hn_amd/forms.py

```python
from __future__ import annotations

import os

ENGINE_DEFAULTS = dict(
    head_streams=1,
    group_convs=True,
    fuse_stem_pool=True,
    fuse_last_gn=True,
    thin_outputs=True,
    conv_multi=True,
    conv_multi_fcos=True,
    tower_carry=True,
)
ACTIVE = dict(ENGINE_DEFAULTS)

_LIB_ENV = {
    "HN_CONV_NO_RS": ("conv_no_rs", None), "HN_CONV_NO_RS32": ("conv_no_rs32", None),
    "HN_SPLIT_GENERIC": ("split_generic", None),
    "HN_CONV_NO_HALO": ("conv_no_halo", None), "HN_PREPROCESS_GENERIC": ("preprocess_generic", None),
    "HN_CONV_NO_MULTI": ("conv_no_multi", None), "HN_HALO_STAMPS": ("halo_stamps", None),
    "HN_SPLITK_FILL512": ("splitk_fill512", None), "HN_CONV_NO_STREAM": ("conv_no_stream", None),
    "HN_CONV_NO_MIXED": ("conv_no_mixed", None), "HN_CONV_NO_DEEPK": ("conv_no_deepk", None),
    "HN_CONV_NO_FUSED_REDUCE": ("conv_no_fused_reduce", None), "HN_THIN_NO_GROUP": ("thin_no_group", None),
}


def engine_forms(overrides=None) -> dict:
    f = dict(ACTIVE)
    if overrides:
        unknown = set(overrides) - set(ENGINE_DEFAULTS)
        if unknown:
            raise KeyError(f"unknown engine forms: {sorted(unknown)}")
        f.update(overrides)
    return f


def apply_env(environ=None) -> dict:
    from . import ops
    env = os.environ if environ is None else environ
    done = {}
    for var, (form, _) in _LIB_ENV.items():
        if var in env:
            ops.set_form(form, True)
            done[var] = form
    if env.get("HN_FUSE_LAST_GN") == "0":
        ops.set_form("no_fuse_last_gn", True)
        ACTIVE["fuse_last_gn"] = False
        done["HN_FUSE_LAST_GN"] = "0"
    if env.get("HN_THIN_OUTPUTS") == "0":
        ops.set_form("no_thin_outputs", True)
        ACTIVE["thin_outputs"] = False
        done["HN_THIN_OUTPUTS"] = "0"
    if env.get("HN_THIN_FORM", "")[:1] in ("t", "f"):
        ops.set_form("thin_form_tap" if env["HN_THIN_FORM"][0] == "t" else "thin_form_flat", True)
        done["HN_THIN_FORM"] = env["HN_THIN_FORM"]
    for var, key in (("HN_GROUP_CONVS", "group_convs"), ("HN_FUSE_STEM_POOL", "fuse_stem_pool"), ("HN_CONV_MULTI", "conv_multi"),
                     ("HN_CONV_MULTI_FCOS", "conv_multi_fcos"), ("HN_TOWER_CARRY", "tower_carry")):
        if var in env:
            ACTIVE[key] = env[var] != "0"
            done[var] = env[var]
    if "HN_CONV_MULTI" in env and "HN_CONV_MULTI_FCOS" not in env:
        ACTIVE["conv_multi_fcos"] = ACTIVE["conv_multi"]
    if "HN_HEAD_STREAMS" in env:
        ACTIVE["head_streams"] = int(env["HN_HEAD_STREAMS"])
        done["HN_HEAD_STREAMS"] = env["HN_HEAD_STREAMS"]
    if "HN_SPLITK" in env:
        ops.SPLITK = env["HN_SPLITK"] != "0"
        done["HN_SPLITK"] = env["HN_SPLITK"]
    if "HN_SPLITK_EAGER" in env:
        ops.SPLITK_EAGER = env["HN_SPLITK_EAGER"] == "1"
        done["HN_SPLITK_EAGER"] = env["HN_SPLITK_EAGER"]
    for var in env:
        if var.startswith("HN_TUNE_"):
            from . import _lib
            ops.check(_lib.load().hn_set_tuning(var[8:].lower().encode(), float(env[var])), "hn_set_tuning")
            done[var] = env[var]
    if "HN_CANDIDATES_CHUNKED" in env:
        ops.CANDIDATES_CHUNKED = env["HN_CANDIDATES_CHUNKED"] != "0"
        done["HN_CANDIDATES_CHUNKED"] = env["HN_CANDIDATES_CHUNKED"]
    return done
```

### handnet-pipeline_amd/hn_amd/ops.py

```python
from __future__ import annotations

import collections
import contextlib
import ctypes as C
import math
import os
from dataclasses import dataclass

import numpy as np
import torch

from . import _lib
from ._lib import ConvDesc, ConvGroup, FcosLevels, check, ptr


_raw_stream = getattr(torch._C, "_cuda_getCurrentRawStream", None)
_cur_device = getattr(torch._C, "_cuda_getDevice", None)


def _stream() -> int:
    if _raw_stream is not None and _cur_device is not None:
        return _raw_stream(_cur_device())
    return torch.cuda.current_stream().cuda_stream

# ... 47 lines not shown


def conv_out_size(h, w, r, s, stride, pad, dil):
    return ((h + 2 * pad - dil * (r - 1) - 1) // stride + 1,
            (w + 2 * pad - dil * (s - 1) - 1) // stride + 1)


def is_split(t) -> bool:
    return t is not None and t.dtype == torch.float16 and t.dim() == 6 and t.shape[4] == 2 and t.shape[5] == 32


def channels(t) -> int:
    return t.shape[3] * 32 if is_split(t) else t.shape[3]


def _pixel_stride(t: torch.Tensor, name: str) -> int:
    if not t.is_cuda:
        raise RuntimeError(f"{name} must live on the GPU (no CPU fallback in handnet-pipeline_amd)")
    _check_device(t, name)
    n, h, w = t.shape[:3]
    ps = t.stride(2)
    if is_split(t):
        inner_ok = t.stride(5) == 1 and t.stride(4) == 32 and t.stride(3) == 64 and ps >= 64 * t.shape[3]
    elif t.dtype == torch.float32 and t.dim() == 4:
        inner_ok = t.stride(3) == 1 and ps >= t.shape[3]
    else:
        raise TypeError(f"{name}: expected fp32 [N,H,W,C] or fp16 S32 [N,H,W,C/32,2,32], got {t.dtype} {tuple(t.shape)}")
    if not inner_ok or t.stride(1) != w * ps or t.stride(0) != h * w * ps:
        raise ValueError(f"{name} must be NHWC-dense or a channel slice of an NHWC-dense tensor")
    return ps


_DESC_TEMPLATES = {}
_PLANS = {}


def _plan_get(*parts):
    key = (SPLITK, SPLITK_EAGER, F16_TERMS, parts)
    return key, _PLANS.get(key)


def _plan_put(key, struct, out_specs, use_ws):
    _PLANS[key] = (type(struct).from_buffer_copy(struct), out_specs, bool(use_ws))


def make_conv_desc(n, h, w, cin, cout, r, s, stride=1, pad=0, dil=1, relu_cols=0, res_mode=0,
                   res_h=0, res_w=0, in_affine=0, tile=0, in_pix_stride=0, out_pix_stride=0) -> ConvDesc:
    key = (n, h, w, cin, cout, r, s, stride, pad, dil, relu_cols, res_mode, res_h, res_w, in_affine, tile,
           in_pix_stride, out_pix_stride)
    tpl = _DESC_TEMPLATES.get(key)
    if tpl is None:
        oh, ow = conv_out_size(h, w, r, s, stride, pad, dil)
        tpl = _DESC_TEMPLATES[key] = ConvDesc(
            n=n, h=h, w=w, cin=cin, cout=cout, r=r, s=s, stride=stride, pad=pad, dil=dil, oh=oh, ow=ow,
            relu_cols=relu_cols, res_mode=res_mode, res_h=res_h, res_w=res_w, in_affine=in_affine, tile=tile,
            out_split=0, res_split=0, res_pix_stride=0, in_pix_stride=in_pix_stride, out_pix_stride=out_pix_stride,
            in_affine_stride=0, splitk=0)
    return ConvDesc.from_buffer_copy(tpl)


def _table_stride(scale, shift, n, c, stride=None, names="scale / shift", width="C"):
    if stride is None:
        stride = scale.stride(0)
    for t in (scale, shift):
        if not t.is_cuda or t.dtype != torch.float32 or tuple(t.shape) != (n, c) or t.stride(1) != 1 or t.stride(0) != stride:
            raise ValueError(f"{names} must be fp32 GPU [N, {width}] tables with equal row stride")
    return stride


def _s32_levels(xs, cin, what="levels"):
    n, xstride = xs[0].shape[0], _pixel_stride(xs[0], "x")
    for x in xs:
        if not is_split(x) or x.shape[0] != n or channels(x) != cin or _pixel_stride(x, "x") != xstride:
            raise ValueError(f"{what} must be S32 tensors of one batch size, channel count and pixel stride")
    return n, xstride


def _f32_levels(ts, c):
    n, xstride = ts[0].shape[0], _pixel_stride(ts[0], "x")
    for t in ts:
        if t.dtype != torch.float32 or is_split(t) or t.shape[0] != n or t.shape[3] != c or _pixel_stride(t, "x") != xstride:
            raise ValueError("levels must be fp32 NHWC tensors of one batch size, channel count and pixel stride")
    return n, xstride


def _rows(xs) -> int:
    return sum(x.shape[0] * x.shape[1] * x.shape[2] for x in xs)


def _alloc_out(n, oh, ow, cout, split, device):
    if split:
        if cout % 32:
            raise ValueError("out_split needs Cout % 32 == 0")
        return torch.empty((n, oh, ow, cout // 32, 2, 32), device=device, dtype=torch.float16)
    return torch.empty((n, oh, ow, cout), device=device, dtype=torch.float32)


def _relu_cols(cout, relu, relu_cols):
    return (cout if relu else 0) if relu_cols is None else relu_cols


def _stamp_out(d, out, cout, f16=True, splitk=None):
    ys = _pixel_stride(out, "out")
    d.out_split = 1 if is_split(out) else 0
    d.out_pix_stride = 0 if ys == (2 * cout if d.out_split else cout) else ys
    d.terms = 1 if (f16 and F16_TERMS == 1) else 0
    if splitk is not None:
        d.splitk = (1 if SPLITK_EAGER else 0) if splitk else -1
    return ys


def _stamp_residual(d, residual):
    d.res_split = 1 if is_split(residual) else 0
    d.res_pix_stride = _pixel_stride(residual, "residual")


def to_split(x, scale=None, shift=None, relu=False, out=None):
    lib = _lib.load()
    xs = _pixel_stride(x, "x")
    if is_split(x):
        raise TypeError("x is already split")
    n, h, w, c = x.shape
    if c % 32:
        raise ValueError("the S32 format needs C % 32 == 0")
    if out is None:
        out = torch.empty((n, h, w, c // 32, 2, 32), device=x.device, dtype=torch.float16)
    ys = _pixel_stride(out, "out")
    a_stride = 0 if scale is None else _table_stride(scale, shift, n, c)
    check(lib.hn_affine_split_f32(ptr(x), ptr(scale), ptr(shift), 1 if relu else 0, n, h * w, c, xs, a_stride,
                                  ptr(out), ys, _stream()), "hn_affine_split_f32")
    return out


def from_split(xs16, out=None):
    lib = _lib.load()
    ps = _pixel_stride(xs16, "x")
    if not is_split(xs16):
        raise TypeError("x is not an S32 tensor")
    n, h, w, nb = xs16.shape[:4]
    if out is None:
        out = torch.empty((n, h, w, nb * 32), device=xs16.device, dtype=torch.float32)
    check(lib.hn_unsplit_f32(ptr(xs16), n, h * w, nb * 32, ps, ptr(out), _pixel_stride(out, "out"), _stream()),
          "hn_unsplit_f32")
    return out


CONV_PROFILE = None
PROFILE_STAGE = None
TILE_NAMES = {1: "128x128", 2: "128x64", 3: "64x64", 4: "128x32", 6: "64x128", 7: "32x64", 8: "256x64", 12: "64x64k2"}
TILE_RS = 0x100
TILE_HALO = 0x200
TILE_MULTI = 0x400
TILE_STREAM = 0x800


def tile_name(tile) -> str:
    if isinstance(tile, int) and tile & TILE_HALO:
        return "halo16x16"
    if isinstance(tile, int) and tile & TILE_STREAM:
        return "stream1x1"
    base = TILE_NAMES.get(tile & 0xFF, str(tile & 0xFF)) if isinstance(tile, int) else str(tile)
    return base + ("+rs" if isinstance(tile, int) and tile & TILE_RS else "") + \
        ("+multi" if isinstance(tile, int) and tile & TILE_MULTI else "")


def _profile_start():
    if CONV_PROFILE is None:
        return None
    timer = HipTimer()
    timer.start()
    return timer


def _profile_stop(timer, describe):
    timer.stop()
    kind, macs, shape = describe()
    CONV_PROFILE.append((kind, macs, timer, shape, PROFILE_STAGE))


F16_TERMS = 3


class f16_terms:

    def __init__(self, terms):
        self.terms = terms

    def __enter__(self):
        global F16_TERMS
        self._old, F16_TERMS = F16_TERMS, self.terms

    def __exit__(self, *a):
        global F16_TERMS
        F16_TERMS = self._old


def clear_plan_caches():
    _PLANS.clear()
    _DESC_TEMPLATES.clear()


CONV_WORKSPACE_BYTES = 32 << 20
SPLITK = True
SPLITK_EAGER = True


class launch_cost_hidden:

    def __enter__(self):
        global SPLITK_EAGER
        self._old, SPLITK_EAGER = SPLITK_EAGER, True

    def __exit__(self, *a):
        global SPLITK_EAGER
        SPLITK_EAGER = self._old


def warm_up_on_side_stream(step, steps: int = 2):
    side = torch.cuda.Stream()
    side.wait_stream(torch.cuda.current_stream())
    with launch_cost_hidden(), torch.cuda.stream(side):
        for _ in range(steps):
            step()
    torch.cuda.current_stream().wait_stream(side)


def capture(step):
    g = torch.cuda.CUDAGraph()
    with launch_cost_hidden(), torch.cuda.graph(g, capture_error_mode="thread_local"):
        out = step()
    return g, out


def capture_step(step):
    warm_up_on_side_stream(step)
    return capture(step)


_WORKSPACES = {}


def _conv_workspace(device):
    key = (device.index, _stream())
    ws = _WORKSPACES.get(key)
    if ws is None:
        ws = _WORKSPACES[key] = torch.empty((CONV_WORKSPACE_BYTES // 4,), device=device, dtype=torch.float32)
    return ws


def conv2d_nhwc(x, w, bias=None, *, stride=1, pad=0, dil=1, relu=False, relu_cols=None,
                residual=None, res_upsample=False, in_scale=None, in_shift=None, out=None, tile=0,
                algo_cin=None, w16=None, out_split=False, gn_partial=None, splitk=True, force_splits=None):
    lib = _lib.load()
    plan_key = None
    if (out is None and in_scale is None and w16 is not None and gn_partial is None and CONV_PROFILE is None
            and x.dtype == torch.float16 and x.is_cuda):
        _check_device(x, "x")
        dev = x.device
        plan_key, plan = _plan_get(
            ConvDesc, dev.index, x.shape, x.stride(), w.data_ptr(), tuple(w.shape), w16.data_ptr(),
            None if bias is None else bias.data_ptr(), stride, pad, dil, relu, relu_cols, tile, out_split, res_upsample, splitk,
            None if residual is None else (residual.shape, residual.stride(), residual.dtype))
        if plan is not None:
            tpl, (out_shape, out_dtype), use_ws = plan
            d = ConvDesc.from_buffer_copy(tpl)
            out = torch.empty(out_shape, device=dev, dtype=out_dtype)
            ws = _conv_workspace(dev) if use_ws else None
            check(lib.hn_conv2d_nhwc_f16x3_ws(C.byref(d), ptr(x), ptr(w16), ptr(bias), ptr(residual), ptr(out),
                                              ptr(ws), ws.numel() * 4 if use_ws else 0, _stream()),
                  "hn_conv2d_nhwc_f16x3_ws")
            return out
    _req(w, name="w")
    cout, r, s, cin = w.shape
    use16 = w16 is not None
    if use16:
        if is_split(x):
            if in_scale is not None:
                raise ValueError("apply the affine with to_split() before an S32-input convolution")
        else:
            x = to_split(x, in_scale, in_shift, relu=in_scale is not None)
            in_scale = in_shift = None
    elif is_split(x):
        raise TypeError("the f32 kernel needs an fp32 input (use from_split)")
    xs = _pixel_stride(x, "x")
    n, h, wd = x.shape[:3]
    if channels(x) != cin:
        raise ValueError(f"weight Cin {cin} != input channels {channels(x)}")
    rc = _relu_cols(cout, relu, relu_cols)
    res_mode, rh, rw = 0, 0, 0
    if residual is not None:
        if channels(residual) != cout or residual.shape[0] != n:
            raise ValueError("residual shape mismatch")
        if is_split(residual) and not use16:
            raise TypeError("the f32 kernel takes fp32 residuals only")
        if res_upsample:
            res_mode, rh, rw = 2, residual.shape[1], residual.shape[2]
        else:
            res_mode = 1
    dense_in = xs == (2 * cin if is_split(x) else cin)
    d = make_conv_desc(n, h, wd, cin, cout, r, s, stride, pad, dil, rc, res_mode, rh, rw,
                       1 if in_scale is not None else 0, tile, in_pix_stride=0 if dense_in else xs)
    if out is None:
        out = _alloc_out(n, d.oh, d.ow, cout, out_split, x.device)
    if tuple(out.shape[:3]) != (n, d.oh, d.ow) or channels(out) != cout:
        raise ValueError("out has the wrong shape")
    splitk = bool(splitk and SPLITK) if use16 and gn_partial is None else None
    _stamp_out(d, out, cout, use16, splitk)
    if residual is not None:
        if res_mode == 1 and tuple(residual.shape[:3]) != (n, d.oh, d.ow):
            raise ValueError("residual shape mismatch")
        if use16:
            _stamp_residual(d, residual)
        elif _pixel_stride(residual, "residual") != cout:
            raise ValueError("the f32 kernel needs a dense residual")
    if bias is not None:
        _req(bias, name="bias")
    if in_scale is not None:
        a_stride = _table_stride(in_scale, in_shift, n, cin, names="in_scale / in_shift", width="Cin")
        d.in_affine_stride = 0 if a_stride == cin else a_stride
    timer = _profile_start()
    if use16:
        if (not w16.is_cuda or w16.dtype != torch.float16 or not w16.is_contiguous()
                or w16.numel() != 2 * w.numel()):
            raise ValueError("w16 must be the contiguous fp16 GPU tensor produced by weights.split_f16x3(w)")
        if gn_partial is not None:
            if residual is not None or rc or d.out_split:
                raise ValueError("gn_partial needs an fp32 output without residual / ReLU")
            need = lib.hn_groupnorm_rows32_scratch_floats(n * d.oh * d.ow, cout)
            if not gn_partial.is_cuda or gn_partial.dtype != torch.float32 or gn_partial.numel() < need:
                raise ValueError(f"gn_partial must be an fp32 GPU buffer of >= {need} floats")
            check(lib.hn_conv2d_nhwc_f16x3_gn(C.byref(d), ptr(x), ptr(w16), ptr(bias), ptr(out), ptr(gn_partial),
                                              _stream()), "hn_conv2d_nhwc_f16x3_gn")
        else:
            if force_splits is not None:
                d.splitk = int(force_splits) if force_splits >= 2 else -1
                plan_key = None
            ws = _conv_workspace(x.device) if splitk else None
            if plan_key is not None and (bias is None or bias.is_contiguous()):
                _plan_put(plan_key, d, (tuple(out.shape), out.dtype), splitk)
            check(lib.hn_conv2d_nhwc_f16x3_ws(C.byref(d), ptr(x), ptr(w16), ptr(bias), ptr(residual), ptr(out),
                                              ptr(ws), ws.numel() * 4 if splitk else 0, _stream()),
                  "hn_conv2d_nhwc_f16x3_ws")
    else:
        if gn_partial is not None:
            raise ValueError("gn_partial is an f16x3-kernel feature")
        check(lib.hn_conv2d_nhwc_f32(C.byref(d), ptr(x), ptr(w), ptr(bias), ptr(residual), ptr(in_scale),
                                     ptr(in_shift), ptr(out), _stream()), "hn_conv2d_nhwc_f32")
    if timer is not None:
        def describe():
            if use16:
                flags = TILE_HALO if lib.hn_conv2d_f16x3_uses_halo(C.byref(d), 1 if residual is not None else 0) else \
                    (TILE_STREAM if lib.hn_conv2d_f16x3_uses_stream(C.byref(d)) else
                     TILE_RS if lib.hn_conv2d_f16x3_uses_rs(C.byref(d)) else 0)
                kind = ("f16x3", lib.hn_conv2d_f16x3_pick_tile(C.byref(d)) | flags)
            else:
                kind = ("f32", lib.hn_conv2d_pick_tile(C.byref(d)))
            return kind, n * d.oh * d.ow * cout * r * s * (algo_cin or cin), (n, h, wd, cin, cout, r, stride, dil)
        _profile_stop(timer, describe)
    return out


def conv2d_nhwc_multi(items, fused=None):
    lib = _lib.load()
    k = len(items)
    if k == 0 or k > _lib.CONV_MULTI_MAX:
        raise ValueError(f"need 1..{_lib.CONV_MULTI_MAX} members")
    splitk = SPLITK
    key = [_lib.ConvMulti]
    for x, cw, opts in items:
        res = opts.get("residual")
        key.append((x.device.index, x.shape, x.stride(), x.dtype, cw.w16.data_ptr() if cw.w16 is not None else None,
                    None if cw.bias is None else cw.bias.data_ptr(), cw.stride, cw.pad, cw.dil, opts.get("relu", False),
                    opts.get("relu_cols"), opts.get("out_split", True),
                    None if res is None else (res.shape, res.stride(), res.dtype)))
    key, plan = _plan_get(*key)
    if plan is not None and CONV_PROFILE is None and fused is None:
        tpl, out_specs, use_ws = plan
        mm = _lib.ConvMulti.from_buffer_copy(tpl)
        outs = []
        for i, ((x, _cw, opts), (shape, dtype)) in enumerate(zip(items, out_specs)):
            _check_device(x, "x")
            y = torch.empty(shape, device=x.device, dtype=dtype)
            mm.x16[i], mm.residual[i], mm.y[i] = x.data_ptr(), ptr(opts.get("residual")), y.data_ptr()
            outs.append(y)
        ws = _conv_workspace(items[0][0].device) if use_ws else None
        check(lib.hn_conv2d_nhwc_f16x3_multi(C.byref(mm), ptr(ws), ws.numel() * 4 if use_ws else 0, _stream()),
              "hn_conv2d_nhwc_f16x3_multi")
        return outs
    mm = _lib.ConvMulti()
    mm.count = k
    outs = []
    macs, shapes = 0, []
    for i, (x, cw, opts) in enumerate(items):
        if not is_split(x) or cw.w16 is None:
            raise TypeError("multi launches take S32 inputs and split filter banks")
        if not x.is_cuda:
            raise RuntimeError("x must live on the GPU (no CPU fallback in handnet-pipeline_amd)")
        _check_device(x, "x")
        relu, relu_cols = opts.get("relu", False), opts.get("relu_cols")
        residual, out_split = opts.get("residual"), opts.get("out_split", True)
        cout, r, s_, cin = cw.w.shape
        n, h, wd = x.shape[:3]
        if channels(x) != cin:
            raise ValueError(f"member {i}: weight Cin {cin} != input channels {channels(x)}")
        xs = _pixel_stride(x, "x")
        d = make_conv_desc(n, h, wd, cin, cout, r, s_, cw.stride, cw.pad, cw.dil, _relu_cols(cout, relu, relu_cols),
                           1 if residual is not None else 0, 0, 0, 0, 0, in_pix_stride=0 if xs == 2 * cin else xs)
        y = _alloc_out(n, d.oh, d.ow, cout, out_split, x.device)
        _stamp_out(d, y, cout, splitk=bool(splitk))
        if residual is not None:
            if tuple(residual.shape[:3]) != (n, d.oh, d.ow) or channels(residual) != cout:
                raise ValueError(f"member {i}: residual shape mismatch")
            _stamp_residual(d, residual)
        if cw.bias is not None:
            _req(cw.bias, name="bias")
        mm.desc[i] = d
        mm.x16[i], mm.w16[i], mm.bias[i] = ptr(x), ptr(cw.w16), ptr(cw.bias)
        mm.residual[i], mm.y[i] = ptr(residual), ptr(y)
        outs.append(y)
        macs += n * d.oh * d.ow * cout * r * s_ * cin
        shapes.append((n, h, wd, cin, cout, r, cw.stride, cw.dil))
    ws = _conv_workspace(items[0][0].device) if splitk else None
    if fused is not None:
        fused.append(bool(lib.hn_conv2d_f16x3_multi_fuses(C.byref(mm), ws.numel() * 4 if splitk else 0)))
    timer = _profile_start()
    check(lib.hn_conv2d_nhwc_f16x3_multi(C.byref(mm), ptr(ws), ws.numel() * 4 if splitk else 0, _stream()),
          "hn_conv2d_nhwc_f16x3_multi")
    if timer is not None:
        def describe():
            big = max(range(k), key=lambda i: shapes[i][0] * shapes[i][1] * shapes[i][2] * shapes[i][3] * shapes[i][4] * shapes[i][5] ** 2)
            return ("f16x3", lib.hn_conv2d_f16x3_pick_tile(C.byref(mm.desc[big])) | TILE_MULTI), macs, shapes[big]
        _profile_stop(timer, describe)
    else:
        _plan_put(key, mm, [(tuple(y.shape), y.dtype) for y in outs], splitk)
    return outs


def conv2d_nhwc_grouped(xs, ws, *, pad=0, relu=False, relu_cols=None, out_split=False, tile=0, gn_partials=None,
                        outs=None, out_channel_offsets=None, gn=None, gn_units=0, carry=None, carry_query=False):
    k = len(xs)
    if k != len(ws) or k == 0 or k > _lib.CONV_MAX_GROUP:
        raise ValueError(f"need 1..{_lib.CONV_MAX_GROUP} inputs and as many weight sets")
    if k == 1 and outs is None and gn is None and carry is None and not carry_query:
        return [conv2d_nhwc(xs[0], ws[0].w, ws[0].bias, pad=pad, relu=relu, relu_cols=relu_cols, w16=ws[0].w16,
                            out_split=out_split, tile=tile, gn_partial=None if gn_partials is None else gn_partials[0])]
    lib = _lib.load()
    cout, r, s, cin = ws[0].w.shape
    x0 = xs[0]
    n, xstride = _s32_levels(xs, cin, "grouped inputs")
    for cw in ws:
        if tuple(cw.w.shape) != (cout, r, s, cin) or cw.w16 is None or (cw.bias is None) != (ws[0].bias is None):
            raise ValueError("grouped weights must share one shape (and all or none have a bias)")
    rc = _relu_cols(cout, relu, relu_cols)
    h0, w0 = x0.shape[1:3]
    d = make_conv_desc(n, h0, w0, cin, cout, r, s, 1, pad, 1, rc, 0, 0, 0, 0, tile,
                       in_pix_stride=0 if xstride == 2 * cin else xstride)
    if gn_partials is not None:
        if gn is not None or len(gn_partials) != k:
            raise ValueError("give gn_partials (one per member) or gn, not both")
        gn, gn_units = [(g, 0) for g in gn_partials], 0
    if gn is not None and (rc or out_split):
        raise ValueError("GroupNorm sums need fp32 outputs without ReLU")
    sizes = [conv_out_size(x.shape[1], x.shape[2], r, s, 1, pad, 1) for x in xs]
    if outs is None:
        outs = [_alloc_out(n, oh, ow, cout, out_split, x0.device) for oh, ow in sizes]
    offs = [0] * k if out_channel_offsets is None else list(out_channel_offsets)
    ystride = _stamp_out(d, outs[0], cout, splitk=False)
    grp = ConvGroup()
    grp.count = k
    grp.gn_units = int(gn_units)
    units = gn_units if gn_units else cout // 8
    for i, (x, cw, y, (oh, ow)) in enumerate(zip(xs, ws, outs, sizes)):
        if (tuple(y.shape[:3]) != (n, oh, ow) or is_split(y) != bool(d.out_split) or _pixel_stride(y, "out") != ystride
                or offs[i] % 32 or offs[i] + cout > channels(y)):
            raise ValueError("grouped outputs must match their member's size and share type / pixel stride")
        elt = 2 if d.out_split else 4
        grp.x16[i], grp.w16[i], grp.bias[i] = ptr(x), ptr(cw.w16), ptr(cw.bias)
        grp.y[i] = y.data_ptr() + elt * (2 * offs[i] if d.out_split else offs[i])
        grp.h[i], grp.w[i] = x.shape[1], x.shape[2]
        grp.gn_partial[i] = None
        if gn is not None:
            buf, uoff = gn[i]
            need = lib.hn_groupnorm_rows32_scratch_floats(n * oh * ow, units * 8)
            if buf.numel() < need or buf.dtype != torch.float32 or not buf.is_cuda or uoff * 8 + cout > units * 8:
                raise ValueError(f"member {i}: GroupNorm slab must be an fp32 GPU buffer of >= {need} floats")
            grp.gn_partial[i] = buf.data_ptr() + 16 * uoff
    if carry_query:
        return bool(lib.hn_conv2d_f16x3_grouped_carry_applies(C.byref(d), C.byref(grp)))
    timer = _profile_start()
    if carry is not None:
        cxs, caff, couts, crelu = carry
        lv, cn, cc, cxstride, ca_stride, cystride, _ = _split_levels_arg(cxs, caff, couts)
        check(lib.hn_conv2d_nhwc_f16x3_grouped_carry(C.byref(d), C.byref(grp), C.byref(lv), 1 if crelu else 0, cn, cc, cxstride,
                                                     ca_stride, cystride, _stream()), "hn_conv2d_nhwc_f16x3_grouped_carry")
    else:
        check(lib.hn_conv2d_nhwc_f16x3_grouped(C.byref(d), C.byref(grp), _stream()), "hn_conv2d_nhwc_f16x3_grouped")
    if timer is not None:
        def describe():
            rows = sum(n * oh * ow for oh, ow in sizes)
            tot = make_conv_desc(1, rows, 1, cin, cout, 1, 1)
            picked = lib.hn_conv2d_f16x3_pick_tile(C.byref(tot))
            q = ConvDesc.from_buffer_copy(d)
            q.tile, q.w = picked, min(ow for _, ow in sizes)
            return (("f16x3", picked | (TILE_RS if lib.hn_conv2d_f16x3_uses_rs(C.byref(q)) else 0)), rows * cout * r * s * cin,
                    (1, rows, 1, cin, cout, r, 1, 1))
        _profile_stop(timer, describe)
    return outs


def conv3x3_thin_levels(xs, cw, relu_cols=0):
    lib = _lib.load()
    cout, r, s, cin = cw.w.shape
    if (r, s) != (3, 3) or cout > 16 or cw.w16 is None or len(xs) > _lib.HN_FCOS_MAX_LEVELS:
        raise ValueError("conv3x3_thin_levels needs a 3x3 filter bank with <= 16 output channels and a split bank")
    n, xstride = _s32_levels(xs, cin)
    lv = _thin_levels_of(xs, inputs=True)
    outs = _thin_outs(lv, xs, cout)
    timer = _profile_start()
    check(lib.hn_conv3x3_thin_f16x3_levels(C.byref(lv), n, cin, cout, ptr(cw.w16), ptr(cw.bias), int(relu_cols),
                                           0 if xstride == 2 * cin else xstride, _stream()), "hn_conv3x3_thin_f16x3_levels")
    if timer is not None:
        def describe():
            rows = _rows(xs)
            form = "thin-P" if lib.hn_conv3x3_thin_uses_flat(C.byref(lv), n, cin, cout) else "thin16x16"
            return ("f16x3", form), rows * cout * 9 * cin, (1, rows, 1, cin, cout, 3, 1, 1)
        _profile_stop(timer, describe)
    return outs


def conv3x3_thin_levels_group(members):
    lib = _lib.load()
    if not 1 <= len(members) <= 3:
        raise ValueError("1..3 members")
    cin = members[0][1].w.shape[3]
    n, xstride = _s32_levels([x for xs, _, _ in members for x in xs], cin)
    arr = (_lib.ThinMember * len(members))()
    results = []
    for m, (xs, cw, relu_cols) in enumerate(members):
        cout, r, s_, c = cw.w.shape
        if (r, s_) != (3, 3) or cout > 16 or cw.w16 is None or len(xs) > _lib.HN_FCOS_MAX_LEVELS or c != cin:
            raise ValueError("members need 3x3 filter banks with <= 16 output channels, a split bank and one input channel count")
        mm = arr[m]
        mm.lv = _thin_levels_of(xs, inputs=True)
        results.append(_thin_outs(mm.lv, xs, cout))
        mm.cout, mm.relu_cols, mm.w16, mm.bias = cout, int(relu_cols), ptr(cw.w16), ptr(cw.bias)
    timer = _profile_start()
    check(lib.hn_conv3x3_thin_f16x3_levels_group(arr, len(members), n, cin, 0 if xstride == 2 * cin else xstride, _stream()),
          "hn_conv3x3_thin_f16x3_levels_group")
    if timer is not None:
        def describe():
            flat = any(lib.hn_conv3x3_thin_uses_flat(C.byref(arr[m].lv), n, cin, arr[m].cout) for m in range(len(members)))
            macs = sum(_rows(xs) * cw.w.shape[0] for xs, cw, _ in members) * 9 * cin
            couts = sum(cw.w.shape[0] for _, cw, _ in members)
            return ("f16x3", "thin-P" if flat else f"thin16x16x{len(members)}"), macs, (1, _rows(members[0][0]), 1, cin, couts, 3, 1, 1)
        _profile_stop(timer, describe)
    return results


def _thin_levels_of(ts, inputs=False):
    lv = _lib.ThinLevels()
    lv.count = len(ts)
    for i, t in enumerate(ts):
        lv.h[i], lv.w[i] = t.shape[1], t.shape[2]
        if inputs:
            lv.x16[i] = t.data_ptr()
    return lv


def _thin_outs(lv, ts, cout):
    outs = [torch.empty((t.shape[0], t.shape[1], t.shape[2], cout), device=t.device, dtype=torch.float32) for t in ts]
    for i, y in enumerate(outs):
        lv.y[i] = y.data_ptr()
    return outs


def thin_affine_applies(ts, cw) -> bool:
    cout, _, _, cin = cw.w.shape
    lv = _thin_levels_of(ts)
    return len(ts) <= _lib.HN_FCOS_MAX_LEVELS and bool(_lib.load().hn_conv3x3_thin_affine_applies(C.byref(lv), ts[0].shape[0], cin, cout))


def conv3x3_thin_affine_levels(ts, affines, ch0, cw, relu_cols=0):
    lib = _lib.load()
    cout, r, s, cin = cw.w.shape
    c = ts[0].shape[3]
    if (r, s) != (3, 3) or cw.w16 is None or ch0 % 32 or ch0 + cin > c:
        raise ValueError("conv3x3_thin_affine_levels needs a split 3x3 filter bank and a 32-aligned channel range")
    n, xstride = _f32_levels(ts, c)
    a_stride = affines[0][0].stride(0)
    lv, aff = _thin_levels_of(ts), _lib.ThinAffine()
    aff.in_pix_stride, aff.affine_stride = xstride, a_stride
    for i, (t, (scale, shift)) in enumerate(zip(ts, affines)):
        _table_stride(scale, shift, n, c, a_stride)
        aff.x[i], aff.scale[i], aff.shift[i] = t.data_ptr() + 4 * ch0, scale.data_ptr() + 4 * ch0, shift.data_ptr() + 4 * ch0
    outs = _thin_outs(lv, ts, cout)
    timer = _profile_start()
    check(lib.hn_conv3x3_thin_affine_f16x3_levels(C.byref(lv), C.byref(aff), n, cin, cout, ptr(cw.w16), ptr(cw.bias),
                                                  int(relu_cols), _stream()), "hn_conv3x3_thin_affine_f16x3_levels")
    if timer is not None:
        def describe():
            rows = _rows(ts)
            return ("f16x3", "thin-P+gn"), rows * cout * 9 * cin, (1, rows, 1, cin, cout, 3, 1, 1)
        _profile_stop(timer, describe)
    return outs


def thin_uses_flat(xs, cw) -> bool:
    cout, _, _, cin = cw.w.shape
    return bool(_lib.load().hn_conv3x3_thin_uses_flat(C.byref(_thin_levels_of(xs)), xs[0].shape[0], cin, cout))


def maxpool3x3s2_nhwc(x, out=None):
    lib = _lib.load()
    if is_split(x):
        if not x.is_contiguous():
            raise ValueError("x must be contiguous")
        n, h, w, nb = x.shape[:4]
        oh, ow = (h + 2 - 3) // 2 + 1, (w + 2 - 3) // 2 + 1
        if out is None:
            out = torch.empty((n, oh, ow, nb, 2, 32), device=x.device, dtype=torch.float16)
        check(lib.hn_maxpool3x3s2_s32(ptr(x), ptr(out), n, h, w, nb * 32, oh, ow, _stream()), "hn_maxpool3x3s2_s32")
        return out
    _req(x, name="x")
    n, h, w, c = x.shape
    oh, ow = (h + 2 - 3) // 2 + 1, (w + 2 - 3) // 2 + 1
    if out is None:
        out = torch.empty((n, oh, ow, c), device=x.device, dtype=torch.float32)
    check(lib.hn_maxpool3x3s2_nhwc_f32(ptr(x), ptr(out), n, h, w, c, oh, ow, _stream()), "hn_maxpool3x3s2_nhwc_f32")
    return out


def groupnorm_affine(x, gamma, beta, groups=32, eps=1e-5, scratch=None, scale=None, shift=None):
    lib = _lib.load()
    _req(x, name="x"); _req(gamma, name="gamma"); _req(beta, name="beta")
    n, h, w, c = x.shape
    need = lib.hn_groupnorm_scratch_floats(n, h * w, c, groups)
    if scratch is None or scratch.numel() < need:
        scratch = torch.empty((need,), device=x.device, dtype=torch.float32)
    if scale is None:
        scale = torch.empty((n, c), device=x.device, dtype=torch.float32)
    if shift is None:
        shift = torch.empty((n, c), device=x.device, dtype=torch.float32)
    check(lib.hn_groupnorm_affine_f32(ptr(x), ptr(gamma), ptr(beta), n, h * w, c, groups, eps, ptr(scratch),
# ... 749 lines not shown
        if other is not None and other.device != pred.device:
            raise ValueError(f"{name} lives on {other.device}, pred on {pred.device}")
    dist = torch.empty((s, 3, j), device=pred.device, dtype=torch.float64) if want_dist else None
    aligned = torch.empty((s, j, 3), device=pred.device, dtype=torch.float64) if want_aligned else None
    check(_lib.load().hn_hpe_accumulate_f32(ptr(pred), ptr(gt), ptr(valid), s, j, ptr(thresholds), t, ptr(state.hist), ptr(state.sum),
                                            ptr(state.n), ptr(dist), ptr(aligned), _stream()), "hn_hpe_accumulate_f32")
    return HPEBatch(state, dist, aligned)


def procrustes_align(gt, pred):
    _req(pred, name="pred")
    return hpe_accumulate(pred, gt, torch.zeros((1,), device=pred.device, dtype=torch.float64), want_aligned=True).aligned


DET_AP_MAX_GT = 64
DET_AP_MAX_RECORDS = 1 << 27
DET_AP_SCORE_BITS, DET_AP_TP_SHIFT, DET_AP_FP_SHIFT, DET_AP_VALID = 10, 10, 15, 1 << 20

DetAPTable = collections.namedtuple("DetAPTable", "hand_off hand_box hand_meta hand_obj obj_off obj_box obj_diff num_images "
                                                  "npos_hand npos_obj")
DetAPState = collections.namedtuple("DetAPState", "hand obj fed overflow flat")


def det_ap_table(hand_off, hand_box, hand_meta, hand_obj, obj_off, obj_box, obj_diff, device) -> DetAPTable:
    hand_off, obj_off = (np.asarray(x, np.int64).reshape(-1) for x in (hand_off, obj_off))
    hand_box, hand_meta, obj_box = (np.asarray(x, np.int64).reshape(-1, 4) for x in (hand_box, hand_meta, obj_box))
    hand_obj, obj_diff = np.asarray(hand_obj, np.float64).reshape(-1, 4), np.asarray(obj_diff, np.int64).reshape(-1)
    num_images = hand_off.shape[0] - 1
    if num_images < 1 or obj_off.shape[0] != num_images + 1:
        raise ValueError(f"hand_off and obj_off must hold images + 1 >= 2 offsets, got {hand_off.shape[0]} and {obj_off.shape[0]}")
    for name, off, rows in (("hand", hand_off, hand_box.shape[0]), ("obj", obj_off, obj_box.shape[0])):
        per = np.diff(off)
        if off[0] != 0 or off[-1] != rows or (per < 0).any():
            raise ValueError(f"{name}_off must rise from 0 to the {rows} rows of {name}_box")
        if (per > DET_AP_MAX_GT).any():
            raise ValueError(f"image {int(np.argmax(per))} has {int(per.max())} {name} boxes: at most {DET_AP_MAX_GT} (one lane each)")
    if hand_meta.shape[0] != hand_box.shape[0] or hand_obj.shape[0] != hand_box.shape[0] or obj_diff.shape[0] != obj_box.shape[0]:
        raise ValueError("hand_meta, hand_obj and obj_diff must hold one row per box")
    if max(np.abs(hand_box).max(initial=0), np.abs(obj_box).max(initial=0), np.abs(hand_meta).max(initial=0)) >= 1 << 24:
        raise ValueError("box coordinates and hand fields must be integers below 2^24")
    dev = torch.device(device)
    up = lambda x, dt: torch.from_numpy(np.ascontiguousarray(x.astype(dt))).to(dev)
    return DetAPTable(up(hand_off, np.int32), up(hand_box, np.int32), up(hand_meta, np.int32), up(hand_obj, np.float64),
                      up(obj_off, np.int32), up(obj_box, np.int32), up(obj_diff, np.int32), num_images,
                      int((hand_meta[:, 0] == 0).sum()), int((obj_diff == 0).sum()))


def det_ap_state(num_images, max_dets, device) -> DetAPState:
    num_images, max_dets = int(num_images), int(max_dets)
    if num_images < 1 or max_dets < 1 or num_images * max_dets > DET_AP_MAX_RECORDS:
        raise ValueError(f"num_images >= 1, max_dets >= 1 and num_images * max_dets <= {DET_AP_MAX_RECORDS}, got {num_images} and {max_dets}")
    a = num_images * max_dets
    flat = torch.zeros((2 * a + num_images + 1,), device=device, dtype=torch.int32)
    return DetAPState(flat[:a].view(num_images, max_dets), flat[a:2 * a].view(num_images, max_dets), flat[2 * a:2 * a + num_images],
                      flat[2 * a + num_images:], flat)


def det_ap_accumulate(det, contacts, dxdymags, image_ids, table: DetAPTable, state: DetAPState | None = None, max_dets=100,
                      hand_label=2, object_label=1, score_min=0.1, ovthresh=0.5) -> DetAPState:
    _req(det.boxes, name="det.boxes"); _req(det.scores, name="det.scores")
    if det.scores.dim() != 2 or tuple(det.boxes.shape) != tuple(det.scores.shape) + (4,):
        raise ValueError(f"det.scores must be fp32 [N,cap] and det.boxes [N,cap,4], got {tuple(det.scores.shape)} and {tuple(det.boxes.shape)}")
    n, cap = det.scores.shape
    for name, t, shape in (("det.labels", det.labels, (n, cap)), ("det.sides", det.sides, (n, cap)), ("det.count", det.count, (n,)),
                           ("contacts", contacts, (n, cap)), ("image_ids", image_ids, (n,))):
        if tuple(_req(t, torch.int32, name).shape) != shape:
            raise ValueError(f"{name}: expected int32 {list(shape)}, got {tuple(t.shape)}")
    if tuple(_req(dxdymags, name="dxdymags").shape) != (n, cap, 3):
        raise ValueError(f"dxdymags: expected fp32 {[n, cap, 3]}, got {tuple(dxdymags.shape)}")
    if not isinstance(table, DetAPTable):
        raise TypeError("table must come from det_ap_table")
    if int(hand_label) == int(object_label):
        raise ValueError(f"hand_label and object_label are both {hand_label}")
    if not 0.0 <= float(score_min) < 1.0 or math.isnan(float(ovthresh)):
        raise ValueError(f"score_min in [0, 1) and a threshold that is a number, got {score_min} and {ovthresh}")
    if n * cap > 1 << 28:
        raise ValueError(f"{n} x {cap} detections: at most 2^28 a batch")
    images = table.num_images
    if state is None:
        state = det_ap_state(images, max_dets, det.scores.device)
    else:
        if state.hand.dim() != 2 or state.hand.shape[0] != images:
            raise ValueError(f"state.hand: expected int32 [{images}, max_dets], got {tuple(state.hand.shape)}")
        m = state.hand.shape[1]
        for name, part, shape in (("hand", state.hand, (images, m)), ("obj", state.obj, (images, m)), ("fed", state.fed, (images,)),
                                  ("overflow", state.overflow, (1,))):
            if tuple(_req(part, torch.int32, f"state.{name}").shape) != shape:
                raise ValueError(f"state.{name}: expected int32 {list(shape)}, got {tuple(part.shape)}")
    for name, other in (("det.boxes", det.boxes), ("det.labels", det.labels), ("det.sides", det.sides), ("det.count", det.count),
                        ("contacts", contacts), ("dxdymags", dxdymags), ("image_ids", image_ids), ("table", table.hand_off),
                        ("state", state.hand)):
        if other.device != det.scores.device:
            raise ValueError(f"{name} lives on {other.device}, det.scores on {det.scores.device}")
    check(_lib.load().hn_det_ap_accumulate_f32(
        ptr(det.boxes), ptr(det.scores), ptr(det.labels), ptr(det.sides), ptr(det.count), ptr(contacts), ptr(dxdymags), ptr(image_ids),
        n, cap, ptr(table.hand_off), ptr(table.hand_box), ptr(table.hand_meta), ptr(table.hand_obj), table.hand_box.shape[0],
        ptr(table.obj_off), ptr(table.obj_box), ptr(table.obj_diff), table.obj_box.shape[0], images, int(hand_label),
        int(object_label), float(score_min), float(ovthresh), ptr(state.hand), ptr(state.obj), ptr(state.fed), ptr(state.overflow),
        state.hand.shape[1], _stream()), "hn_det_ap_accumulate_f32")
    return state


def pack_records(kp, crop_box, has_hand, rows, rec_bytes, out=None, extras=()):
    _req(kp, name="keypoints"); _req(crop_box, torch.int64, "crop_box"); _req(has_hand, torch.int32, "has_hand")
    n, j = kp.shape[0], kp.shape[1]
    if out is None:
        out = torch.empty((rows, rec_bytes), device=kp.device, dtype=torch.uint8)
    extras = [e for e in extras if e is not None]
    if extras:
        for e in extras:
            _req(e, name="extra")
            if e.shape != kp.shape:
                raise ValueError("extra fields must have the keypoints' shape")
        e0, e1 = extras[0], (extras[1] if len(extras) > 1 else None)
        check(_lib.load().hn_pack_records_ex(ptr(kp), ptr(crop_box), ptr(has_hand), n, rows, j, rec_bytes, ptr(e0), ptr(e1),
                                             ptr(out), _stream()), "hn_pack_records_ex")
        return out
    check(_lib.load().hn_pack_records(ptr(kp), ptr(crop_box), ptr(has_hand), n, rows, j, rec_bytes, ptr(out), _stream()),
          "hn_pack_records")
    return out


def unpack_records(rec, joints):
    _req(rec, torch.uint8, "records")
    rows, rec_bytes = rec.shape
    dev = rec.device
    kp = torch.empty((rows, joints, 3), device=dev, dtype=torch.float32)
    box = torch.empty((rows, 4), device=dev, dtype=torch.int64)
    has = torch.empty((rows,), device=dev, dtype=torch.int32)
    valid = torch.empty((rows,), device=dev, dtype=torch.int32)
    check(_lib.load().hn_unpack_records(ptr(rec), rows, joints, rec_bytes, ptr(kp), ptr(box), ptr(has), ptr(valid), _stream()),
          "hn_unpack_records")
    return kp, box, has, valid


def nonfinite_count(x, flag=None):
    _req(x, name="x")
    if flag is None:
        flag = torch.zeros((1,), device=x.device, dtype=torch.int32)
    check(_lib.load().hn_nonfinite_count_f32(ptr(x), x.numel(), ptr(flag), _stream()), "hn_nonfinite_count_f32")
    return flag


def tickets_nonzero() -> int:
    c = C.c_int64(0)
    check(_lib.load().hn_debug_tickets_nonzero(C.byref(c)), "hn_debug_tickets_nonzero")
    return int(c.value)


def set_form(name: str, on=True):
    check(_lib.load().hn_set_form(name.encode(), 1 if on else 0), "hn_set_form")


def range_check_enable(on=True):
    check(_lib.load().hn_range_check_enable(1 if on else 0), "hn_range_check_enable")


def range_check_bits(reset=True) -> int:
    flag = C.c_int32(0)
    check(_lib.load().hn_range_check_fetch(C.byref(flag), 1 if reset else 0, _stream()), "hn_range_check_fetch")
    return int(flag.value)


def range_check_fetch(reset=True) -> bool:
    return range_check_bits(reset) != 0


def range_check_bind(block=None):
    check(_lib.load().hn_range_check_bind(ptr(block) if block is not None else None), "hn_range_check_bind")


@contextlib.contextmanager
def range_scope(block=None, on=True):
    lib = _lib.load()
    check(lib.hn_range_scope_begin(ptr(block) if (block is not None and on) else None, 1 if on else 0), "hn_range_scope_begin")
    try:
        yield
    finally:
        check(lib.hn_range_scope_end(), "hn_range_scope_end")


def range_check_collect(block=None, out=None):
    if out is None:
        dev = block.device if block is not None else torch.device("cuda", torch.cuda.current_device())
        out = torch.empty((4,), device=dev, dtype=torch.int32)
    check(_lib.load().hn_range_check_collect(ptr(block) if block is not None else None, ptr(out), _stream()),
          "hn_range_check_collect")
    return out


def range_bits(words) -> int:
    return ((_lib.RANGE_ACTIVATION if words[0] else 0) | (_lib.RANGE_INPUT if words[1] else 0)
            | (_lib.RANGE_INPUT_NONFINITE if words[2] else 0))


class RangeError(RuntimeError):
    """A value left the dynamic range the f16x3 split format supports."""


def clock_sample(micros, out=None, stream=None):
    if out is None:
        out = torch.zeros((1,), device=torch.device("cuda", _cur_device() if _cur_device else 0), dtype=torch.float32)
    st = _stream() if stream is None else stream.cuda_stream
    check(_lib.load().hn_clock_sample(int(micros), ptr(out), st), "hn_clock_sample")
    return out


class HipTimer:

    def __init__(self):
        lib = _lib.load()
        self._a, self._b = C.c_void_p(), C.c_void_p()
        check(lib.hn_event_create(C.byref(self._a)), "hn_event_create")
        check(lib.hn_event_create(C.byref(self._b)), "hn_event_create")

    def start(self):
        check(_lib.load().hn_event_record(self._a, _stream()), "hn_event_record")

    def stop(self):
        check(_lib.load().hn_event_record(self._b, _stream()), "hn_event_record")

    def elapsed_ms(self) -> float:
        ms = C.c_float()
        check(_lib.load().hn_event_elapsed_ms(self._a, self._b, C.byref(ms)), "hn_event_elapsed_ms")
        return float(ms.value)

    def __del__(self):
        try:
            lib = _lib.load()
            lib.hn_event_destroy(self._a)
            lib.hn_event_destroy(self._b)
        except Exception:
            pass


@dataclass
class CsrGraph:
    indptr: torch.Tensor
    indices: torch.Tensor
    values: torch.Tensor
    v: int


def csr_graph(L, device) -> CsrGraph:
    if torch.is_tensor(L):
        c = L.coalesce() if L.layout == torch.sparse_coo else L.to_sparse_coo().coalesce()
        import scipy.sparse as sp
        idx = c.indices().cpu().numpy()
        L = sp.csr_matrix((c.values().cpu().numpy(), (idx[0], idx[1])), shape=tuple(c.shape))
    m = L.tocsr().astype(np.float32)
    m.sort_indices()
    if m.shape[0] != m.shape[1]:
        raise ValueError("graph Laplacian must be square")
    return CsrGraph(torch.from_numpy(m.indptr.astype(np.int32)).to(device), torch.from_numpy(m.indices.astype(np.int32)).to(device),
                    torch.from_numpy(m.data.astype(np.float32)).to(device), m.shape[0])


def cheby2_graph(L, device) -> CsrGraph:
    import scipy.sparse as sp
    m = L.tocsr().astype(np.float64)
    q = (2.0 * (m @ m) - sp.identity(m.shape[0], dtype=np.float64, format="csr")).tocsr()
    q.sum_duplicates()
    return csr_graph(q, device)


def _csr_struct(g: CsrGraph):
    return _lib.GraphCsr(g.indptr.data_ptr(), g.indices.data_ptr(), g.values.data_ptr(), g.v)


def graph_conv_cheby3(g: CsrGraph, g2: CsrGraph, x, cw, relu=True, xin=None, up=1, out_split=False, out=None):
    _req(x, name="x")
    b, v, fin = x.shape
    fout, _, _, k = cw.w.shape
    if v != g.v or g2.v != g.v or k != (3 * fin + 31) // 32 * 32:
        raise ValueError("graph / filter bank do not match the input")
    if xin is not None:
        _req(xin, name="xin")
        if tuple(xin.shape[:2]) != (b, v):
            raise ValueError("xin must be [B,V,Fi]")
    if out is not None:
        y = _req(out, torch.float16 if out_split else torch.float32, "out")
        if y.numel() != b * v * up * fout * (2 if out_split else 1):
            raise ValueError("out has the wrong size")
    elif out_split:
        y = torch.empty((b, v * up, 1, fout // 32, 2, 32), device=x.device, dtype=torch.float16)
    else:
        y = torch.empty((b, v * up, fout), device=x.device, dtype=torch.float32)
    wf = getattr(cw, "w_frag", None)
    check(_lib.load().hn_graph_conv_cheby3_f16x3(C.byref(_csr_struct(g)), C.byref(_csr_struct(g2)), ptr(x), b, fin,
                                                 ptr(wf if wf is not None else cw.w16), 1 if wf is not None else 0,
                                                 ptr(cw.bias), fout, 1 if relu else 0, ptr(xin), xin.shape[2] if xin is not None else 0,
                                                 up, ptr(y), 1 if out_split else 0, _stream()), "hn_graph_conv_cheby3_f16x3")
    return y


def fragment_order(w16):
    fout, kt, _, _ = w16.shape
    nt = (fout + 15) // 16
    w = torch.zeros((nt * 16, kt, 2, 32), dtype=w16.dtype, device=w16.device)
    w[:fout] = w16
    return w.view(nt, 16, kt, 2, 4, 8).permute(0, 2, 3, 4, 1, 5).contiguous().view(nt, kt, 2, 64, 8)


def linear_rows(x, cw, scale=None, shift=None, residual=None, relu=False, n_out=None):
    _req(x, name="x")
    m, kx = x.shape
# ... 655 lines not shown
```

### include/handnet_hip.h

```cpp
#ifndef HANDNET_HIP_H
#define HANDNET_HIP_H

#include <stdint.h>

#ifdef __cplusplus
extern "C" {
#endif

#define HN_OK 0
#define HN_ERR_ARG 1
#define HN_ERR_HIP 2

#define HN_ABI_VERSION 36
int hn_abi_version(void);
const char* hn_last_error(void);

int hn_device_info(int* cu_count, int* clock_khz, char* arch_name, int arch_name_len);
int hn_device_pci_bus_id(char* out , int out_len );

int hn_event_create(void** ev);
int hn_event_destroy(void* ev);
int hn_event_record(void* ev, void* stream);
int hn_event_elapsed_ms(void* start, void* stop, float* ms);

int hn_clock_sample(int micros, float* mhz, void* stream);

#define HN_RANGE_ACTIVATION 1
#define HN_RANGE_INPUT 2
#define HN_RANGE_INPUT_NONFINITE 4
int hn_range_check_enable(int on);
int hn_range_check_enabled(void);
int hn_range_check_fetch(int* flag , int reset, void* stream);
int hn_range_check_bind(int32_t* block );
int hn_range_scope_begin(int32_t* block , int on);
int hn_range_scope_end(void);
int hn_range_check_collect(int32_t* block , int32_t* dst , void* stream);

int hn_set_form(const char* name, int value);
int hn_debug_tickets_nonzero(int64_t* count );
int hn_set_tuning(const char* name, double value);

typedef struct hn_conv_desc {
  int32_t n, h, w, cin;
  int32_t cout;
  int32_t r, s;
  int32_t stride, pad, dil;
  int32_t oh, ow;
  int32_t relu_cols;
  int32_t res_mode;
  int32_t res_h, res_w;
  int32_t in_affine;
  int32_t tile;
  int32_t out_split;
  int32_t res_split;
  int32_t res_pix_stride;
  int32_t in_pix_stride;
  int32_t out_pix_stride;
  int32_t in_affine_stride;
  int32_t splitk;
  int32_t terms;
} hn_conv_desc;

#define HN_TILE_AUTO 0
#define HN_TILE_128x128 1
#define HN_TILE_128x64 2
#define HN_TILE_64x64 3
#define HN_TILE_128x32 4
#define HN_TILE_64x128 6
#define HN_TILE_32x64 7
#define HN_TILE_256x64 8
#define HN_TILE_64x64_K2 12

int hn_conv2d_nhwc_f32(const hn_conv_desc* d, const float* x, const float* w,
                       const float* bias ,
                       const float* residual ,
                       const float* in_scale, const float* in_shift ,
                       float* y, void* stream);

int hn_conv2d_pick_tile(const hn_conv_desc* d);

int hn_conv2d_nhwc_f16x3(const hn_conv_desc* d, const void* x16 , const void* w16,
                         const float* bias, const void* residual ,
                         void* y , void* stream);
int hn_conv2d_f16x3_pick_tile(const hn_conv_desc* d);
int hn_conv2d_f16x3_uses_rs(const hn_conv_desc* d);
int hn_conv2d_f16x3_uses_halo(const hn_conv_desc* d, int has_residual);
int hn_conv2d_f16x3_uses_stream(const hn_conv_desc* d);

int hn_affine_split_f32(const float* x, const float* scale, const float* shift, int relu,
                        int n, int hw, int c, int in_pix_stride, int affine_stride,
                        void* y16, int out_pix_stride, void* stream);
int hn_unsplit_f32(const void* x16, int n, int hw, int c, int in_pix_stride,
                   float* y, int out_pix_stride, void* stream);
int hn_maxpool3x3s2_s32(const void* x16, void* y16, int n, int h, int w, int c,
                        int oh, int ow, void* stream);

int hn_maxpool3x3s2_nhwc_f32(const float* x, float* y, int n, int h, int w, int c,
                             int oh, int ow, void* stream);

int64_t hn_groupnorm_scratch_floats(int n, int hw, int c, int groups);
int hn_groupnorm_affine_f32(const float* x , const float* gamma,
                            const float* beta, int n, int hw, int c, int groups, float eps,
                            float* partial, float* scale, float* shift, void* stream);

int hn_conv2d_nhwc_f16x3_ws(const hn_conv_desc* desc, const void* x16, const void* w16,
                            const float* bias, const void* residual, void* y,
                            void* workspace, int64_t workspace_bytes, void* stream);

#define HN_CONV_MAX_GROUP 6
typedef struct hn_conv_group {
  int32_t count;
  const void* x16[HN_CONV_MAX_GROUP];
  const void* w16[HN_CONV_MAX_GROUP];
  const float* bias[HN_CONV_MAX_GROUP];
  void* y[HN_CONV_MAX_GROUP];
  float* gn_partial[HN_CONV_MAX_GROUP];
  int32_t h[HN_CONV_MAX_GROUP], w[HN_CONV_MAX_GROUP];
  int32_t gn_units;
} hn_conv_group;
int hn_conv2d_nhwc_f16x3_grouped(const hn_conv_desc* desc, const hn_conv_group* group, void* stream);

#define HN_CONV_MULTI_MAX 4
typedef struct hn_conv_multi {
  int32_t count;
  hn_conv_desc desc[HN_CONV_MULTI_MAX];
  const void* x16[HN_CONV_MULTI_MAX];
  const void* w16[HN_CONV_MULTI_MAX];
  const float* bias[HN_CONV_MULTI_MAX];
  const void* residual[HN_CONV_MULTI_MAX];
  void* y[HN_CONV_MULTI_MAX];
} hn_conv_multi;
int hn_conv2d_nhwc_f16x3_multi(const hn_conv_multi* mm, void* workspace, int64_t workspace_bytes, void* stream);
int hn_conv2d_f16x3_multi_fuses(const hn_conv_multi* mm, int64_t workspace_bytes);

int hn_conv2d_nhwc_f16x3_gn(const hn_conv_desc* desc, const void* x16, const void* w16,
                            const float* bias, void* y, float* gn_partial, void* stream);
int64_t hn_groupnorm_rows32_scratch_floats(int64_t rows, int c);
int hn_groupnorm_finalize_rows32(const float* partial, const float* gamma, const float* beta,
                                 int n, int hw, int c, int groups, float eps,
                                 float* scale, float* shift, void* stream);

#define HN_FCOS_MAX_LEVELS 5
typedef struct hn_gn_levels {
  int32_t count;
  int32_t hw[HN_FCOS_MAX_LEVELS];
  const float* partial[HN_FCOS_MAX_LEVELS];
  float* scale[HN_FCOS_MAX_LEVELS];
  float* shift[HN_FCOS_MAX_LEVELS];
} hn_gn_levels;
int hn_groupnorm_finalize_rows32_levels(const hn_gn_levels* lv, const float* gamma, const float* beta,
                                        int n, int c, int groups, float eps, void* stream);
typedef struct hn_split_levels {
  int32_t count;
  int32_t hw[HN_FCOS_MAX_LEVELS];
  const float* x[HN_FCOS_MAX_LEVELS];
  const float* scale[HN_FCOS_MAX_LEVELS];
  const float* shift[HN_FCOS_MAX_LEVELS];
  void* y16[HN_FCOS_MAX_LEVELS];
} hn_split_levels;
int hn_affine_split_f32_levels(const hn_split_levels* lv, int relu, int n, int c, int in_pix_stride,
                               int affine_stride, int out_pix_stride, void* stream);
int hn_affine_split_f32_levels_streams(const int32_t* hw, int count, int n, int c);

int hn_conv2d_nhwc_f16x3_grouped_carry(const hn_conv_desc* desc, const hn_conv_group* group, const hn_split_levels* lv,
                                       int relu, int n, int c, int in_pix_stride, int affine_stride, int out_pix_stride,
                                       void* stream);
int hn_conv2d_f16x3_grouped_carry_applies(const hn_conv_desc* desc, const hn_conv_group* group);

typedef struct hn_thin_levels {
  int32_t count;
  const void* x16[HN_FCOS_MAX_LEVELS];
  float* y[HN_FCOS_MAX_LEVELS];
  int32_t h[HN_FCOS_MAX_LEVELS], w[HN_FCOS_MAX_LEVELS];
} hn_thin_levels;
int hn_conv3x3_thin_f16x3_levels(const hn_thin_levels* lv, int n, int cin, int cout, const void* w16, const float* bias,
                                 int relu_cols, int in_pix_stride, void* stream);
int hn_conv3x3_thin_uses_flat(const hn_thin_levels* lv, int n, int cin, int cout);

typedef struct hn_thin_member {
  hn_thin_levels lv;
  int32_t cout, relu_cols;
  const void* w16;
  const float* bias;
} hn_thin_member;
int hn_conv3x3_thin_f16x3_levels_group(const hn_thin_member* members, int count , int n, int cin, int in_pix_stride,
                                       void* stream);

typedef struct hn_thin_affine {
  const float* x[HN_FCOS_MAX_LEVELS];
  const float* scale[HN_FCOS_MAX_LEVELS];
  const float* shift[HN_FCOS_MAX_LEVELS];
  int32_t in_pix_stride;
  int32_t affine_stride;
} hn_thin_affine;
int hn_conv3x3_thin_affine_applies(const hn_thin_levels* lv, int n, int cin, int cout);
int hn_conv3x3_thin_affine_f16x3_levels(const hn_thin_levels* lv, const hn_thin_affine* aff, int n, int cin, int cout,
                                        const void* w16, const float* bias, int relu_cols, void* stream);

int hn_ingest_u8bgr_u16mm(const uint8_t* bgr, const void* depth, int depth_kind, float* rgb, float* depth_m,
                          float* rgbd, int n, int h, int w, void* stream);
int hn_ingest_u8bgr_u16mm_flip(const uint8_t* bgr, const void* depth, int depth_kind, float* rgb, float* depth_m,
                               float* rgbd, int n, int h, int w, int flip_w, void* stream);
int hn_flip_w_f32(const float* a, float* a_out, int64_t rows_a, const float* b, float* b_out, int64_t rows_b, int w,
                  void* stream);

int hn_fcos_preprocess_f32(const float* src, float* dst, int n, int h, int w,
                           int oh, int ow, int ph, int pw,
                           const float mean[3], const float stdv[3], void* stream);

int hn_fcos_preprocess_split(const float* src, void* dst16, int n, int h, int w, int oh, int ow,
                             int ph, int pw, int border, const float mean[3], const float stdv[3],
                             void* stream);
int hn_fcos_preprocess_list(const float* const* srcs, const int32_t* geom, void* dst, int split, int n,
                            int ph, int pw, int border, const float mean[3], const float stdv[3],
                            void* stream);
int hn_conv_stem_f16x3(const void* x16, int n, int ph, int pw, int pad, int r, int stride, int cout,
                       const void* w16, const float* bias, int relu, void* y, int out_split,
                       void* stream);
int hn_conv_stem_pool_f16x3(const void* x16, int n, int ph, int pw, int pad, int r, int stride, int cout,
                            const void* w16, const float* bias, void* y, void* stream);
int hn_conv_stem_pool_f16x3_terms(const void* x16, int n, int ph, int pw, int pad, int r, int stride, int cout,
                                  const void* w16, const float* bias, void* y, int terms, void* stream);

typedef struct hn_fcos_levels {
  int32_t num_levels;
  int32_t h[HN_FCOS_MAX_LEVELS], w[HN_FCOS_MAX_LEVELS], stride[HN_FCOS_MAX_LEVELS];
  const float* cls_lr[HN_FCOS_MAX_LEVELS];
  const float* reg_ctr[HN_FCOS_MAX_LEVELS];
} hn_fcos_levels;

int hn_fcos_candidates(const hn_fcos_levels* lv, int n, int num_classes, float score_thresh,
                       float* cand_boxes , float* cand_scores ,
                       int32_t* cand_labels, int32_t* cand_sides, int32_t* cand_level ,
                       int32_t* cand_point ,
                       int32_t* cand_count , int cap, void* stream);
int64_t hn_fcos_candidates_ws_bytes(int n, int total_points);
int hn_fcos_candidates_ws(const hn_fcos_levels* lv, int n, int num_classes, float score_thresh, float* cand_boxes,
                          float* cand_scores, int32_t* cand_labels, int32_t* cand_sides, int32_t* cand_level,
                          int32_t* cand_point, int32_t* cand_count, int cap, void* workspace, int64_t workspace_bytes,
                          void* stream);

int hn_fcos_ext_gather(const hn_fcos_levels* lv, const float* const* ext, const int32_t* det_keep,
                       const int32_t* cand_point, const int32_t* det_count, int n, int cap,
                       int32_t* det_contacts , float* det_dxdymags ,
                       void* stream);

int64_t hn_fcos_nms_scratch_bytes(int n, int cap);
int hn_fcos_nms(const float* cand_boxes, const float* cand_scores, const int32_t* cand_labels,
                const int32_t* cand_sides, const int32_t* cand_level, const int32_t* cand_count,
                int n, int cap, double iou_thresh, float ratio_h, float ratio_w,
                void* scratch,
                float* det_boxes , float* det_scores, int32_t* det_labels,
                int32_t* det_sides, int32_t* det_level, int32_t* det_keep ,
                int32_t* det_count , void* stream);

int hn_fcos_nms_ratios(const float* cand_boxes, const float* cand_scores, const int32_t* cand_labels,
                       const int32_t* cand_sides, const int32_t* cand_level, const int32_t* cand_count,
                       int n, int cap, double iou_thresh, const float* ratios, void* scratch,
                       float* det_boxes, float* det_scores, int32_t* det_labels, int32_t* det_sides,
                       int32_t* det_level, int32_t* det_keep, int32_t* det_count, void* stream);

int hn_nms(const float* boxes, const float* scores, int k, double iou_thresh,
           void* scratch , int32_t* keep, int32_t* num_keep,
           void* stream);

int hn_crop_resize(const float* det_boxes, const int32_t* det_labels, const int32_t* det_count,
                   int cap, int hand_label, const float* depth, int n, int in_ch, int reorder_bgr,
                   int h, int w, int out, int cpad, int64_t* crop_box, int32_t* has_hand, float* crops,
                   void* stream);

int hn_crop_resize_hands(const float* det_boxes, const float* det_scores, const int32_t* det_labels,
                         const int32_t* det_count, int cap, int hand_label, int max_hands, const float* depth, int n,
                         int in_ch, int reorder_bgr, int h, int w, int out, int cpad, int64_t* crop_box, int32_t* has_hand,
// ... 216 lines not shown
```

Measured before the change: 1171 frames/s.

## Split 3x3 conv batches into 128x128 and 64x128 members to fill the tail wave

Adds a tail-split planner for stride-1 3x3 convolutions. It models workgroup waves over 512 slots and, when the last wave would be partly empty, splits the batch into two group members: one tiled 128x128 and the rest tiled 64x128, both issued as a single mixed launch. To make that possible the grouped launch now accepts per-member residuals through a gres table and a new gres kernel, and a new grouped_res API exposes this. The cost model relies on hand-set constants, so it may choose a worse split for some shapes, and a two-member launch adds planning work on the host.

```diff
diff --git a/handnet-pipeline_amd/csrc/conv_igemm_f16x3.hip b/handnet-pipeline_amd/csrc/conv_igemm_f16x3.hip
--- a/handnet-pipeline_amd/csrc/conv_igemm_f16x3.hip
+++ b/handnet-pipeline_amd/csrc/conv_igemm_f16x3.hip
@@ -29,7 +29,7 @@
   if constexpr (BUF && NBUF == 2 && (WM * WN == 4 || WM * WN == 8) && RS_LDS_BYTES <= (WM * WN == 4 ? 80 : 160) * 1024 - 2048) {
     rs = rs_will_run(p, BM, BN, WM * WN, NBUF, BUF);
     if constexpr (BM == 128 && BN == 128 && WM == 2 && WN == 2 && TERMS == 3) {
-      const int mask = rs ? mixed_small_mask(p, p.tiles_n) : 0;
+      const int mask = !rs ? 0 : p.small_mask ? p.small_mask : mixed_small_mask(p, p.tiles_n);
       if (mask && carry) return hn::fail(HN_ERR_ARG, "%s", kCarryRefused);
       if (mask) {
         p.small_mask = mask;
@@ -49,6 +49,25 @@
         }
         hipLaunchKernelGGL(conv_igemm_f16x3_mixed_kernel, dim3(grid_x, 1, p.groups), dim3(256), LDS_MIXED, st, p);
         HN_CHECK_LAUNCH("conv_igemm_f16x3_mixed_kernel");
+        return HN_OK;
+      }
+    }
+    if constexpr (BM == 128 && BN == 128 && WM == 2 && WN == 2 && TERMS == 3) {
+      if (p.groups > 1 && p.res_mode && !carry) {
+        if (rs) {
+          static bool gres_attr[64] = {};
+          int dev = 0;
+          HN_CHECK_HIP(hipGetDevice(&dev));
+          if (dev < 0 || dev >= 64 || !gres_attr[dev]) {
+            HN_CHECK_HIP(hipFuncSetAttribute((const void*)conv_igemm_f16x3_gres_kernel<true>, hipFuncAttributeMaxDynamicSharedMemorySize,
+                                             RS_LDS_BYTES));
+            if (dev >= 0 && dev < 64) gres_attr[dev] = true;
+          }
+          hipLaunchKernelGGL(conv_igemm_f16x3_gres_kernel<true>, dim3(grid_x, 1, p.groups), dim3(256), RS_LDS_BYTES, st, p);
+        } else {
+          hipLaunchKernelGGL(conv_igemm_f16x3_gres_kernel<false>, dim3(grid_x, 1, p.groups), dim3(256), 0, st, p);
+        }
+        HN_CHECK_LAUNCH("conv_igemm_f16x3_gres_kernel");
         return HN_OK;
       }
     }
@@ -231,10 +250,25 @@
   return hn::conv_grouped_run(d, group, stream, nullptr);
 }
 
-int hn::conv_grouped_run(const hn_conv_desc* d, const hn_conv_group* group, void* stream, const hn::CarryHook* carry) {
+extern "C" int hn_conv2d_nhwc_f16x3_grouped_res(const hn_conv_desc* d, const hn_conv_group* group, const void* const* residual,
+                                                void* stream) {
+  HN_CHECK_ARG(residual, "hn_conv2d_nhwc_f16x3_grouped_res: null residual table");
+  return hn::conv_grouped_run(d, group, stream, nullptr, residual);
+}
+
+int hn::conv_grouped_run(const hn_conv_desc* d, const hn_conv_group* group, void* stream, const hn::CarryHook* carry,
+                         const void* const* residual) {
   HN_CHECK_ARG(d && group, "hn_conv2d_nhwc_f16x3_grouped: null pointer");
   HN_CHECK_ARG(group->count >= 1 && group->count <= HN_CONV_MAX_GROUP, "group count must be 1..%d", HN_CONV_MAX_GROUP);
-  HN_CHECK_ARG(d->res_mode == 0, "grouped convolutions take no residual");
+  HN_CHECK_ARG(d->res_mode == 0 || !carry, "the carrying grouped launch takes no residual");
+  HN_CHECK_ARG(d->res_mode == 0 || residual, "grouped convolutions take a residual through hn_conv2d_nhwc_f16x3_grouped_res only");
+  HN_CHECK_ARG(d->res_mode != 2, "grouped convolutions do not take the upsampled residual (res_mode 2)");
+  HN_CHECK_ARG(d->res_mode == 0 || d->res_split, "grouped convolutions do not take an fp32 residual (S32 only)");
+  HN_CHECK_ARG(d->res_mode != 0 || !residual, "a residual table needs res_mode 1");
+  for (int g = 0; residual && g < group->count; ++g) {
+    HN_CHECK_ARG(residual[g] && (uintptr_t)residual[g] % 16 == 0, "group member %d has a null or unaligned residual", g);
+    HN_CHECK_ARG(!group->gn_partial[g], "a group member with GroupNorm sums takes no residual");
+  }
   bool any_gn = false, all_gn = true;
   for (int g = 0; g < group->count; ++g) {
     HN_CHECK_ARG(group->x16[g] && group->w16[g] && group->y[g], "group member %d has a null tensor", g);
@@ -243,13 +277,45 @@
   }
   HN_CHECK_ARG(any_gn == all_gn, "gn_partial must be given for every group member or for none");
   HN_CHECK_ARG(group->gn_units == 0 || group->gn_units >= d->cout / 8, "gn_units smaller than cout/8");
-  return hn_igemm_conv16_run(d, group->x16[0], group->w16[0], group->bias[0], nullptr, group->y[0], nullptr, nullptr, 0, stream,
-                    group, carry);
+  return hn_igemm_conv16_run(d, group->x16[0], group->w16[0], group->bias[0], residual ? residual[0] : nullptr, group->y[0], nullptr,
+                             nullptr, 0, stream, group, carry, residual);
+}
+
+static TailSplitPlan tail_split_of(const hn_conv_desc* d, bool has_workspace, int64_t workspace_bytes) {
+  const int picked = hn_conv2d_f16x3_pick_tile(d);
+  const TileForm f = tile_form(picked, false);
+  ConvParams16 q;
+  q.M = d->n * d->oh * d->ow; q.Cout = d->cout; q.ktiles = d->r * d->s * d->cin / BK;
+  q.groups = 1; q.gn_partial = nullptr; q.vec_epi = 1; q.splitk_mode = d->splitk; q.terms = 3;
+  q.split_ws = has_workspace ? reinterpret_cast<float*>(16) : nullptr;
+  q.split_ws_bytes = has_workspace ? workspace_bytes : 0;
+  bool single = f.bm != 0;
+  if (single) {
+    q.nblocks = hn::cdiv(q.M, f.bm) * hn::cdiv(q.Cout, f.bn);
+    plan_splits(q, f.bm, f.bn, f.kk);
+    single = q.splits == 1;
+  }
+  return tail_split_plan(d, single, picked == HN_TILE_128x128);
+}
+
+extern "C" int hn_conv2d_f16x3_tail_split(const hn_conv_desc* d) {
+  if (!d || d->n <= 0 || d->w <= 0 || d->cin <= 0 || d->cout <= 0) return 0;
+  if (hn::conv3x3_halo_applies(d, false, false, d->res_mode ? (const void*)d : nullptr)) return 0;
+  const TailSplitPlan t = tail_split_of(d, d->splitk >= 0, (int64_t)32 << 20);
+  return t.taken ? t.n0 : 0;
+}
+
+extern "C" int hn_conv2d_f16x3_tail_split_plan(const hn_conv_desc* d, double* out) {
+  HN_CHECK_ARG(d && out, "hn_conv2d_f16x3_tail_split_plan: null pointer");
+  const TailSplitPlan t = tail_split_of(d, d->splitk >= 0, (int64_t)32 << 20);
+  out[0] = t.n0; out[1] = t.taken; out[2] = (double)t.wg_plain; out[3] = (double)t.wg0; out[4] = (double)t.wg1;
+  out[5] = t.us_plain; out[6] = t.us_split;
+  return HN_OK;
 }
 
 int hn_igemm_conv16_run(const hn_conv_desc* d, const void* x16, const void* w16, const float* bias, const void* residual, void* y,
                         float* gn_partial, void* workspace, int64_t workspace_bytes, void* stream, const hn_conv_group* group,
-                        const hn::CarryHook* carry) {
+                        const hn::CarryHook* carry, const void* const* group_residual) {
   ConvParams16 p;
   HN_TRY16(fill_params16(d, x16, w16, bias, residual, y, gn_partial, workspace, workspace_bytes, p));
   if (d->terms != 1 && hn::conv3x3_halo_applies(d, gn_partial != nullptr, group != nullptr, residual) &&
@@ -258,6 +324,16 @@
   if (hn::conv1x1_stream_applies(d, gn_partial != nullptr, group != nullptr) &&
       hn::conv1x1_stream_operands_ok(d, x16, w16, bias, residual, y))
     return hn::conv1x1_stream(d, x16, w16, bias, residual, y, (hipStream_t)stream);
+
+  if (!group && !gn_partial && !carry && d->terms != 1 && p.vec_epi) {
+    const TailSplitPlan t = tail_split_of(d, workspace != nullptr, workspace_bytes);
+    if (t.taken) {
+      ConvParams16 q = p, probe;
+      tail_split_members(q, t.n0);
+      probe = q;
+      if (finish_params16(probe) && rs_will_run(probe, 128, 128, 4, 2, true)) return launch16<128, 128, 2, 2, 2>(q, (hipStream_t)stream);
+    }
+  }
 
   hn_conv_desc tile_desc = *d;
   if (group) {
@@ -276,6 +352,7 @@
       if (gn_of_group_needs_32(group, g)) HN_CHECK_ARG(p.gOH[g] * p.gOW[g] >= 32, "GroupNorm statistics need OH*OW >= 32");
       p.gx[g] = (const _Float16*)group->x16[g]; p.gw[g] = (const _Float16*)group->w16[g];
       p.gbias[g] = group->bias[g]; p.gy[g] = group->y[g]; p.ggn[g] = group->gn_partial[g];
+      p.gres[g] = group_residual ? group_residual[g] : nullptr;
       p.vec_epi = p.vec_epi && ((uintptr_t)group->y[g] % 16 == 0) &&
                   (group->bias[g] == nullptr || (uintptr_t)group->bias[g] % 16 == 0);
     }
@@ -297,6 +374,11 @@
   }
   hipStream_t st = (hipStream_t)stream;
   int picked = hn_conv2d_f16x3_pick_tile(&tile_desc);
+  if (group && d->res_mode) {
+    ConvParams16 probe = p;
+    HN_CHECK_ARG(p.terms == 3 && finish_params16(probe), "grouped convolutions with a residual need three terms and operands below 2 GB");
+    picked = HN_TILE_128x128;
+  }
   if (carry && (picked != HN_TILE_128x128 || !group)) return hn::fail(HN_ERR_ARG, "%s", kCarryRefused);
   switch (picked) {
     case HN_TILE_128x128: return launch16<128, 128, 2, 2, 2>(p, st, carry);
diff --git a/handnet-pipeline_amd/csrc/conv_igemm_f16x3_kernel.h b/handnet-pipeline_amd/csrc/conv_igemm_f16x3_kernel.h
--- a/handnet-pipeline_amd/csrc/conv_igemm_f16x3_kernel.h
+++ b/handnet-pipeline_amd/csrc/conv_igemm_f16x3_kernel.h
@@ -59,6 +59,7 @@
   unsigned a_records;
   unsigned b_records;
   unsigned ga_records[HN_CONV_MAX_GROUP];
+  const void* gres[HN_CONV_MAX_GROUP];
 };
 
 #define HN_TRY16(expr)          \
@@ -212,7 +213,7 @@
   }
 };
 
-template <int BM, int BN, int WM, int WN, int NBUF, bool BUF, bool RS = false, int TERMS = 3, bool DYN = false, int KK = 1>
+template <int BM, int BN, int WM, int WN, int NBUF, bool BUF, bool RS = false, int TERMS = 3, bool DYN = false, int KK = 1, bool GRES = false>
 __device__ __forceinline__ void conv_igemm_f16x3_body(const ConvParams16& p, const int blk_x, const int blk_y, const int blk_z,
                                                       const unsigned karg_off = 0 ) {
   static_assert(TERMS == 3 || TERMS == 1, "three terms (fp32-grade) or the hi*hi term alone");
@@ -757,6 +758,12 @@
   ConvParams16 q = p;
   q.x = o.x; q.w = o.w; q.bias = o.bias; q.y = o.y; q.gn_partial = o.gn_partial;
   q.H = o.H; q.W = o.W; q.pitch = o.pitch; q.OH = o.OH; q.OW = o.OW; q.M = o.M;
+  if constexpr (GRES) {
+    if (p.groups > 1) {
+      typedef __attribute__((address_space(4))) const ConvParams16 KArgs;
+      q.res = ((KArgs*)__builtin_amdgcn_kernarg_segment_ptr())->gres[blk_z];
+    }
+  }
   if (p.splits > 1) {
     q.y = p.split_ws + (long)blk_y * o.M * p.Cout;
     q.ys = p.Cout;
@@ -1031,9 +1038,14 @@
   typedef __attribute__((address_space(4))) const ConvParams16 KArgs;
   KArgs* kp = (KArgs*)__builtin_amdgcn_kernarg_segment_ptr();
   if ((kp->small_mask >> blockIdx.z) & 1)
-    conv_igemm_f16x3_body<64, 128, 2, 2, 3, true, false, 3, true>(p, (int)blockIdx.x, (int)blockIdx.y, (int)blockIdx.z);
+    conv_igemm_f16x3_body<64, 128, 2, 2, 3, true, false, 3, true, 1, true>(p, (int)blockIdx.x, (int)blockIdx.y, (int)blockIdx.z);
   else
-    conv_igemm_f16x3_body<128, 128, 2, 2, 2, true, true, 3>(p, (int)blockIdx.x, (int)blockIdx.y, (int)blockIdx.z);
+    conv_igemm_f16x3_body<128, 128, 2, 2, 2, true, true, 3, false, 1, true>(p, (int)blockIdx.x, (int)blockIdx.y, (int)blockIdx.z);
+}
+
+template <bool RS>
+__global__ __launch_bounds__(256, 2) void conv_igemm_f16x3_gres_kernel(const ConvParams16 p) {
+  conv_igemm_f16x3_body<128, 128, 2, 2, 2, true, RS, 3, false, 1, true>(p, (int)blockIdx.x, (int)blockIdx.y, (int)blockIdx.z);
 }
 
 #endif
diff --git a/handnet-pipeline_amd/csrc/conv_igemm_f16x3_plan.h b/handnet-pipeline_amd/csrc/conv_igemm_f16x3_plan.h
--- a/handnet-pipeline_amd/csrc/conv_igemm_f16x3_plan.h
+++ b/handnet-pipeline_amd/csrc/conv_igemm_f16x3_plan.h
@@ -188,6 +188,93 @@
     case HN_TILE_64x64_K2: return {64, 64, 4, 3, 2};
     default: return {0, 0, 0, 0, 1};
   }
+}
+
+constexpr double kTailLone = 0.50;
+constexpr double kTailPair = 0.93;
+constexpr double kTailHalf = 0.60;
+constexpr double kTailFill = 480.0;
+constexpr double kTailFloor = 0.33;
+constexpr double kTailRoundUs0 = 16.0, kTailRoundUsK = 1.0;
+constexpr double kTailMinGain = 0.02;
+constexpr int kTailSlots = 512, kTailCus = 256, kTailNear = 8;
+constexpr bool kTailTakeLone = false;
+constexpr int kTailKtMin = 36, kTailKtMax = 144;
+struct TailSplitPlan {
+  int n0;
+  int taken;
+  int64_t wg_plain, wg0, wg1;
+  double us_plain, us_split;
+};
+static int64_t tail_wgs(int imgs, int ohow, int tiles_n, int bm) { return (int64_t)hn::cdiv((int64_t)imgs * ohow, bm) * tiles_n; }
+static bool tail_split_geometry(const hn_conv_desc* d) {
+  const hn::EnvFlags& ef = hn::env_flags();
+  if (ef.no_tail_split || ef.no_mixed || ef.no_rs || d->n < 2 || d->terms == 1 || d->in_affine) return false;
+  if (!(d->r == 3 && d->s == 3 && d->stride == 1 && d->dil == 1 && d->pad == 1 && d->oh == d->h && d->ow == d->w)) return false;
+  if (d->cin % 32 || d->cout % 8 || !(d->res_mode == 0 || (d->res_mode == 1 && d->res_split))) return false;
+  if ((128 + 1) / d->w + 1 > 4 * 8 - 2) return false;
+  const int64_t xs = d->in_pix_stride ? d->in_pix_stride : 2 * d->cin, lim = (int64_t)1 << 31;
+  return ((int64_t)d->n * d->h * d->w * xs + ((int64_t)d->w + 1) * xs) * 2 < lim && (int64_t)d->cout * 9 * d->cin * 4 < lim;
+}
+static TailSplitPlan tail_split_plan(const hn_conv_desc* d, bool single_pass, bool picked_128) {
+  TailSplitPlan t = {0, 0, 0, 0, 0, 0.0, 0.0};
+  if (!tail_split_geometry(d) || !single_pass) return t;
+  const int ohow = d->oh * d->ow, tiles_n = hn::cdiv(d->cout, 128), ktiles = d->r * d->s * d->cin / 32;
+  t.wg_plain = tail_wgs(d->n, ohow, tiles_n, 128);
+  const int forced = (int)hn::tuning().tail_split_n0;
+  bool lone = false;
+  if (forced > 0) {
+    if (forced >= d->n) return t;
+    t.n0 = forced;
+  } else {
+    if (d->tile != HN_TILE_AUTO || !picked_128 || t.wg_plain <= kTailSlots || t.wg_plain > 8 * kTailSlots) return t;
+    lone = t.wg_plain % kTailSlots <= kTailCus;
+    if (lone) {
+      int64_t best = kTailNear + 1;
+      for (int n0 = 1; n0 < d->n; ++n0) {
+        const int64_t w0 = tail_wgs(n0, ohow, tiles_n, 128), r = w0 % kTailSlots, dist = r < kTailSlots - r ? r : kTailSlots - r;
+        if (w0 + dist >= kTailSlots && dist <= best) { best = dist; t.n0 = n0; }
+      }
+      if (best > kTailNear) t.n0 = 0;
+    } else {
+      for (int n0 = d->n - 1; n0 >= 1 && t.n0 == 0; --n0) {
+        const int64_t w0 = tail_wgs(n0, ohow, tiles_n, 128), rest = w0 % kTailSlots;
+        if (w0 < kTailSlots) break;
+        if (rest <= kTailCus && rest + tail_wgs(d->n - n0, ohow, tiles_n, 64) <= kTailSlots) t.n0 = n0;
+      }
+    }
+    if (t.n0 == 0) return t;
+  }
+  t.wg0 = tail_wgs(t.n0, ohow, tiles_n, 128);
+  t.wg1 = tail_wgs(d->n - t.n0, ohow, tiles_n, 64);
+  const double round_us = kTailRoundUs0 + kTailRoundUsK * ktiles;
+  const int64_t rest_plain = t.wg_plain % kTailSlots, rest0 = t.wg0 % kTailSlots;
+  t.us_plain = round_us * ((double)(t.wg_plain / kTailSlots) + (rest_plain == 0 ? 0.0 : rest_plain <= kTailCus ? kTailLone : kTailPair));
+  const bool under = rest0 >= kTailSlots - kTailNear;
+  const double wave = ((under ? 0.0 : (double)rest0) + kTailHalf * (double)t.wg1) / kTailFill;
+  t.us_split = round_us * ((double)(t.wg0 / kTailSlots + (under ? 1 : 0)) + (wave > kTailFloor ? wave : kTailFloor));
+  t.taken = forced > 0 || (ktiles >= kTailKtMin && ktiles <= kTailKtMax && t.us_plain - t.us_split >= kTailMinGain * t.us_plain &&
+                           (!lone || kTailTakeLone));
+  return t;
+}
+static void tail_split_members(ConvParams16& p, int n0) {
+  const int64_t pix0 = (int64_t)n0 * p.OH * p.OW;
+  p.groups = 2;
+  p.small_mask = 2;
+  for (int g = 0; g < 2; ++g) {
+    p.gH[g] = p.H; p.gW[g] = p.W; p.gOH[g] = p.OH; p.gOW[g] = p.OW;
+    p.gM[g] = (int)(g == 0 ? pix0 : (int64_t)p.M - pix0);
+    p.gx[g] = p.x + (g ? pix0 * p.xs : 0);
+    p.gw[g] = p.w;
+    p.gbias[g] = p.bias;
+    p.gy[g] = (char*)p.y + (g ? pix0 * p.ys * (p.out_split ? 2 : 4) : 0);
+    p.gres[g] = p.res ? (const char*)p.res + (g ? pix0 * p.rs * 2 : 0) : nullptr;
+    p.ggn[g] = nullptr;
+  }
+  p.gn_partial = nullptr;
+  p.split_ws = nullptr;
+  p.splits = 1;
+  p.kt_per = p.ktiles;
 }
 
 static inline bool gn_of_group_needs_32(const hn_conv_group* group, int g) { return group->gn_partial[g] != nullptr; }
@@ -245,4 +332,5 @@
 
 int hn_igemm_conv16_run(const hn_conv_desc* d, const void* x16, const void* w16, const float* bias, const void* residual, void* y,
                         float* gn_partial, void* workspace, int64_t workspace_bytes, void* stream,
-                        const hn_conv_group* group = nullptr, const hn::CarryHook* carry = nullptr);
+                        const hn_conv_group* group = nullptr, const hn::CarryHook* carry = nullptr,
+                        const void* const* group_residual = nullptr);
diff --git a/handnet-pipeline_amd/csrc/hn_common.h b/handnet-pipeline_amd/csrc/hn_common.h
--- a/handnet-pipeline_amd/csrc/hn_common.h
+++ b/handnet-pipeline_amd/csrc/hn_common.h
@@ -13,11 +13,12 @@
 int* range_flag_ptr();
 struct EnvFlags {
   bool no_rs, no_rs32, split_generic, no_halo, no_thin, thin_tap, thin_flat, no_fuse_last_gn, pre_generic, no_multi,
-      halo_stamps, splitk_fill512, no_stream, no_mixed, no_deepk, no_fused_reduce, thin_nogroup;
+      halo_stamps, splitk_fill512, no_stream, no_mixed, no_deepk, no_fused_reduce, thin_nogroup, no_tail_split;
 };
 const EnvFlags& env_flags();
 struct Tuning {
   double splitk_fix = 1.0, splitk_tk = 1.0, splitk_red0 = 1.0, splitk_plane = 1.0;
+  double tail_split_n0 = 0.0;
 };
 const Tuning& tuning();
 bool conv3x3_halo_applies(const hn_conv_desc* d, bool has_gn, bool has_group, const void* residual);
@@ -38,7 +39,8 @@
 };
 int launch_conv_carry(const void* conv_params, size_t conv_params_bytes, int grid_x, int groups, int terms, int lds_bytes,
                       const void* job, hipStream_t st);
-int conv_grouped_run(const hn_conv_desc* d, const hn_conv_group* group, void* stream, const CarryHook* carry);
+int conv_grouped_run(const hn_conv_desc* d, const hn_conv_group* group, void* stream, const CarryHook* carry,
+                     const void* const* residual = nullptr);
 
 int tickets_nonzero_main(int64_t* count);
 int tickets_nonzero_multi(int64_t* count);
diff --git a/handnet-pipeline_amd/csrc/hn_common.hip b/handnet-pipeline_amd/csrc/hn_common.hip
--- a/handnet-pipeline_amd/csrc/hn_common.hip
+++ b/handnet-pipeline_amd/csrc/hn_common.hip
@@ -59,10 +59,11 @@
 }
 
 extern "C" int hn_set_tuning(const char* name, double value) {
-  HN_CHECK_ARG(name && value > 0.0, "hn_set_tuning: null name or non-positive value");
+  HN_CHECK_ARG(name && (value > 0.0 || (value == 0.0 && strcmp(name, "tail_split_n0") == 0)), "hn_set_tuning: null name or non-positive value");
   struct Entry { const char* name; double hn::Tuning::*field; };
   static const Entry table[] = {{"splitk_fix", &hn::Tuning::splitk_fix}, {"splitk_tk", &hn::Tuning::splitk_tk},
-                                {"splitk_red0", &hn::Tuning::splitk_red0}, {"splitk_plane", &hn::Tuning::splitk_plane}};
+                                {"splitk_red0", &hn::Tuning::splitk_red0}, {"splitk_plane", &hn::Tuning::splitk_plane},
+                                {"tail_split_n0", &hn::Tuning::tail_split_n0}};
   for (const Entry& e : table)
     if (strcmp(e.name, name) == 0) {
       hn::g_tuning.*(e.field) = value;
@@ -92,6 +93,7 @@
       {"conv_no_mixed", &hn::EnvFlags::no_mixed},
       {"conv_no_deepk", &hn::EnvFlags::no_deepk},
       {"conv_no_fused_reduce", &hn::EnvFlags::no_fused_reduce},
+      {"conv_no_tail_split", &hn::EnvFlags::no_tail_split},
   };
   for (const Entry& e : table)
     if (strcmp(e.name, name) == 0) {
diff --git a/handnet-pipeline_amd/hn_amd/_lib.py b/handnet-pipeline_amd/hn_amd/_lib.py
--- a/handnet-pipeline_amd/hn_amd/_lib.py
+++ b/handnet-pipeline_amd/hn_amd/_lib.py
@@ -137,6 +137,9 @@
     "hn_fcos_preprocess_f32": (C.c_int, [VP, VP] + [C.c_int] * 7 + [c_f32p, c_f32p, VP]),
     "hn_conv2d_nhwc_f16x3_ws": (C.c_int, [C.POINTER(ConvDesc)] + [VP] * 6 + [C.c_int64, VP]),
     "hn_conv2d_nhwc_f16x3_grouped": (C.c_int, [C.POINTER(ConvDesc), C.POINTER(ConvGroup), VP]),
+    "hn_conv2d_nhwc_f16x3_grouped_res": (C.c_int, [C.POINTER(ConvDesc), C.POINTER(ConvGroup), C.POINTER(VP), VP]),
+    "hn_conv2d_f16x3_tail_split": (C.c_int, [C.POINTER(ConvDesc)]),
+    "hn_conv2d_f16x3_tail_split_plan": (C.c_int, [C.POINTER(ConvDesc), C.POINTER(C.c_double)]),
     "hn_conv2d_nhwc_f16x3_gn": (C.c_int, [C.POINTER(ConvDesc)] + [VP] * 6),
     "hn_groupnorm_rows32_scratch_floats": (C.c_int64, [C.c_int64, C.c_int]),
     "hn_groupnorm_finalize_rows32": (C.c_int, [VP, VP, VP] + [C.c_int] * 4 + [C.c_float, VP, VP, VP]),
diff --git a/handnet-pipeline_amd/hn_amd/forms.py b/handnet-pipeline_amd/hn_amd/forms.py
--- a/handnet-pipeline_amd/hn_amd/forms.py
+++ b/handnet-pipeline_amd/hn_amd/forms.py
@@ -23,6 +23,7 @@
     "HN_CONV_NO_MIXED": ("conv_no_mixed", None), "HN_CONV_NO_DEEPK": ("conv_no_deepk", None),
     "HN_CONV_NO_FUSED_REDUCE": ("conv_no_fused_reduce", None), "HN_THIN_NO_GROUP": ("thin_no_group", None),
 }
+_LIB_ENV_OFF = {"HN_TAIL_SPLIT": "conv_no_tail_split"}
 
 
 def engine_forms(overrides=None) -> dict:
@@ -43,6 +44,10 @@
         if var in env:
             ops.set_form(form, True)
             done[var] = form
+    for var, form in _LIB_ENV_OFF.items():
+        if env.get(var) == "0":
+            ops.set_form(form, True)
+            done[var] = "0"
     if env.get("HN_FUSE_LAST_GN") == "0":
         ops.set_form("no_fuse_last_gn", True)
         ACTIVE["fuse_last_gn"] = False
diff --git a/handnet-pipeline_amd/hn_amd/ops.py b/handnet-pipeline_amd/hn_amd/ops.py
--- a/handnet-pipeline_amd/hn_amd/ops.py
+++ b/handnet-pipeline_amd/hn_amd/ops.py
@@ -223,6 +223,7 @@
 TILE_HALO = 0x200
 TILE_MULTI = 0x400
 TILE_STREAM = 0x800
+TILE_TAIL = 0x1000
 
 
 def tile_name(tile) -> str:
@@ -230,6 +231,8 @@
         return "halo16x16"
     if isinstance(tile, int) and tile & TILE_STREAM:
         return "stream1x1"
+    if isinstance(tile, int) and tile & TILE_TAIL:
+        return "128x128+rs|64x128"
     base = TILE_NAMES.get(tile & 0xFF, str(tile & 0xFF)) if isinstance(tile, int) else str(tile)
     return base + ("+rs" if isinstance(tile, int) and tile & TILE_RS else "") + \
         ("+multi" if isinstance(tile, int) and tile & TILE_MULTI else "")
@@ -423,7 +426,9 @@
                 flags = TILE_HALO if lib.hn_conv2d_f16x3_uses_halo(C.byref(d), 1 if residual is not None else 0) else \
                     (TILE_STREAM if lib.hn_conv2d_f16x3_uses_stream(C.byref(d)) else
                      TILE_RS if lib.hn_conv2d_f16x3_uses_rs(C.byref(d)) else 0)
-                kind = ("f16x3", lib.hn_conv2d_f16x3_pick_tile(C.byref(d)) | flags)
+                if not flags & (TILE_HALO | TILE_STREAM) and lib.hn_conv2d_f16x3_tail_split(C.byref(d)):
+                    flags = TILE_TAIL
+                kind = ("f16x3", (_lib.TILE_128x128 if flags & TILE_TAIL else lib.hn_conv2d_f16x3_pick_tile(C.byref(d))) | flags)
             else:
                 kind = ("f32", lib.hn_conv2d_pick_tile(C.byref(d)))
             return kind, n * d.oh * d.ow * cout * r * s * (algo_cin or cin), (n, h, wd, cin, cout, r, stride, dil)
@@ -508,7 +513,8 @@
 
 
 def conv2d_nhwc_grouped(xs, ws, *, pad=0, relu=False, relu_cols=None, out_split=False, tile=0, gn_partials=None,
-                        outs=None, out_channel_offsets=None, gn=None, gn_units=0, carry=None, carry_query=False):
+                        outs=None, out_channel_offsets=None, gn=None, gn_units=0, carry=None, carry_query=False,
+                        residuals=None, res_upsample=False):
     k = len(xs)
     if k != len(ws) or k == 0 or k > _lib.CONV_MAX_GROUP:
         raise ValueError(f"need 1..{_lib.CONV_MAX_GROUP} inputs and as many weight sets")
@@ -556,10 +562,26 @@
             if buf.numel() < need or buf.dtype != torch.float32 or not buf.is_cuda or uoff * 8 + cout > units * 8:
                 raise ValueError(f"member {i}: GroupNorm slab must be an fp32 GPU buffer of >= {need} floats")
             grp.gn_partial[i] = buf.data_ptr() + 16 * uoff
+    res_tab = None
+    if residuals is not None:
+        if len(residuals) != k:
+            raise ValueError("one residual per member")
+        for i, (res, (oh, ow)) in enumerate(zip(residuals, sizes)):
+            if (not res_upsample and tuple(res.shape[:3]) != (n, oh, ow)) or channels(res) != cout:
+                raise ValueError(f"member {i}: residual shape mismatch")
+            if (is_split(res), _pixel_stride(res, "residual")) != (is_split(residuals[0]), _pixel_stride(residuals[0], "residual")):
+                raise ValueError("grouped residuals must share type and pixel stride")
+        d.res_mode = 1
+        if res_upsample:
+            d.res_mode, d.res_h, d.res_w = 2, residuals[0].shape[1], residuals[0].shape[2]
+        _stamp_residual(d, residuals[0])
+        res_tab = (C.c_void_p * k)(*[r_.data_ptr() for r_ in residuals])
     if carry_query:
         return bool(lib.hn_conv2d_f16x3_grouped_carry_applies(C.byref(d), C.byref(grp)))
     timer = _profile_start()
-    if carry is not None:
+    if res_tab is not None and carry is None:
+        check(lib.hn_conv2d_nhwc_f16x3_grouped_res(C.byref(d), C.byref(grp), res_tab, _stream()), "hn_conv2d_nhwc_f16x3_grouped_res")
+    elif carry is not None:
         cxs, caff, couts, crelu = carry
         lv, cn, cc, cxstride, ca_stride, cystride, _ = _split_levels_arg(cxs, caff, couts)
         check(lib.hn_conv2d_nhwc_f16x3_grouped_carry(C.byref(d), C.byref(grp), C.byref(lv), 1 if crelu else 0, cn, cc, cxstride,
@@ -1615,6 +1637,17 @@
     check(_lib.load().hn_set_form(name.encode(), 1 if on else 0), "hn_set_form")
 
 
+def set_tuning(name: str, value: float):
+    check(_lib.load().hn_set_tuning(name.encode(), float(value)), "hn_set_tuning")
+
+
+def tail_split_plan(d) -> dict:
+    out = (C.c_double * 7)()
+    check(_lib.load().hn_conv2d_f16x3_tail_split_plan(C.byref(d), out), "hn_conv2d_f16x3_tail_split_plan")
+    return dict(n0=int(out[0]), taken=bool(out[1]), wg_plain=int(out[2]), wg0=int(out[3]), wg1=int(out[4]),
+                us_plain=out[5], us_split=out[6])
+
+
 def range_check_enable(on=True):
     check(_lib.load().hn_range_check_enable(1 if on else 0), "hn_range_check_enable")
 
diff --git a/include/handnet_hip.h b/include/handnet_hip.h
--- a/include/handnet_hip.h
+++ b/include/handnet_hip.h
@@ -119,6 +119,10 @@
   int32_t gn_units;
 } hn_conv_group;
 int hn_conv2d_nhwc_f16x3_grouped(const hn_conv_desc* desc, const hn_conv_group* group, void* stream);
+int hn_conv2d_nhwc_f16x3_grouped_res(const hn_conv_desc* desc, const hn_conv_group* group, const void* const* residual,
+                                     void* stream);
+int hn_conv2d_f16x3_tail_split(const hn_conv_desc* desc);
+int hn_conv2d_f16x3_tail_split_plan(const hn_conv_desc* desc, double* out );
 
 #define HN_CONV_MULTI_MAX 4
 typedef struct hn_conv_multi {
```

New measurement: 1179 frames/s (median of 6 runs). No clear change (+0.7%).
